# rcedgar/urmap

Measured on AMD Instinct MI355X. Metric: reads/s mapped, 150 bp SE vs hg38, at 1/2/4/8 MI355X; SAM bit-identical, higher is better.
Workload: dtype u8/u64 (fp32 DP cells as the reference)

## Files before the change

urmap_amd/csrc/kernels.h:

```cpp
#pragma once
#include <hip/hip_runtime.h>
#include <stdint.h>

#include "../../include/urmapx.h"

namespace urx {

struct DevIndex {
	const uint8_t *blob;
	const uint8_t *seq;
	const uint4 *seqp;
	uint64_t slotCount;
	uint64_t slotMagic;
	uint64_t shiftMask;
	uint32_t W;
	uint32_t maxIx;
	uint32_t seqDataSize;
	uint32_t seqCount;
	const uint32_t *seqLengths;
	const uint32_t *seqOffsets;
	const uint2 *rowinfo;
	const uint64_t *rowbase;
	const uint32_t *rows;
	const uint4 *slot16;
};

struct ProbeOut {
	uint64_t *slots;
	uint8_t *tallies;
	uint32_t *positions;
};

hipError_t launch_gather_bench(const DevIndex &X, uint32_t blocks, uint32_t iters, uint32_t *d_sink, hipStream_t s);

hipError_t launch_seed_probe(const DevIndex &X, const uint8_t *d_bases, const uint64_t *d_offs, uint32_t n,
                             uint32_t max_read_len, ProbeOut out, hipStream_t s);

struct DpJob {
	uint32_t read;
	uint32_t startdb, pk;
	int32_t maxpen;
	uint32_t combined_tlo;
	int16_t left_score, right_score;
	uint8_t nops;
	uint8_t flags;
	uint8_t vst_l, vst_r;
	uint16_t k;
	uint8_t pad[2];
};
static_assert(sizeof(DpJob) == 32, "DpJob layout");
static constexpr uint8_t DPJ_LEFT_FAIL = 1, DPJ_RIGHT_FAIL = 2, DPJ_RIGHT_SKIPPED = 4, DPJ_PATH_LONG = 8, DPJ_GATED = 16, DPJ_RIGHT_ABORTED = 32;
static constexpr int DP_ROUNDS = 4;
struct DpBounds {
	int rounds;
	uint32_t lo[DP_ROUNDS + 1];
};
inline DpBounds dp_bounds_default(bool long_reads) {
	DpBounds b;
	if (long_reads) { b.rounds = 4; b.lo[0] = 0; b.lo[1] = 2; b.lo[2] = 8; b.lo[3] = 32; b.lo[4] = 0xFFFFFFFFu; }
	else { b.rounds = 3; b.lo[0] = 0; b.lo[1] = 2; b.lo[2] = 16; b.lo[3] = 0xFFFFFFFFu; b.lo[4] = 0xFFFFFFFFu; }
	return b;
}
static constexpr int DP_TICKET_WORDS = 16;
static_assert(DP_ROUNDS <= 8, "DP_TICKET_WORDS");
static constexpr int DP_JOB_OPS = URMAPX_MAX_PATH_OPS;
static constexpr int STAGE_LAST = 3 + 4 * DP_ROUNDS;
static constexpr int STAGE_P3_MAIN = STAGE_LAST + 1, STAGE_P3_DP = STAGE_LAST + 2;
static constexpr int STAGE_EVENTS = STAGE_LAST + 3;

struct DpWork {
	DpJob *jobs = nullptr;
	uint16_t *ops = nullptr;
	uint16_t *kidx = nullptr;
	uint32_t jobs_cap = 0;
	uint32_t *tickets = nullptr;
	uint32_t *round_list = nullptr;
	uint32_t *counters = nullptr;
	uint32_t *fin_list = nullptr;
	uint32_t *state = nullptr;
	uint32_t fin_cap = 0;
};
size_t dp_state_words(bool ovf);
size_t p3_state_words(uint32_t max_read_len);

struct SearchWork {
	uint32_t *stats;
	uint8_t *scratch;
	size_t scratch_stride;
	int blocks;
	uint32_t *ticket;
	uint32_t *ticket3 = nullptr;
	int hsp_lds_cap = 0;
	uint32_t *ovf_list = nullptr;
	DpWork dp[2];
	DpWork dp3;
	uint8_t *dp_scratch = nullptr;
	size_t dp_scratch_stride = 0;
	int dp_blocks = 0;
	int fin_blocks = 0;
	DpBounds dp_bounds = dp_bounds_default(false);
	hipEvent_t *stage_events = nullptr;
};
size_t dp_scratch_stride(uint32_t max_read_len);
int dp_block_count(uint32_t max_read_len, int device);
int fin_block_count(uint32_t max_read_len, int device);
size_t search_scratch_stride(uint32_t max_read_len);
size_t search_scratch_tail(int blocks);
size_t search_pe_scratch_tail(int blocks);
int search_block_count(uint32_t max_read_len, int device);
size_t viterbi_batch_scratch_stride();

hipError_t launch_search_se(const DevIndex &X, const urmapx_params &P, const uint8_t *d_bases, const uint64_t *d_offs,
                            uint32_t n, uint32_t max_read_len, urmapx_result *d_results,
                            urmapx_path_op *d_path_ops, uint32_t *d_path_used, const SearchWork &wk, hipStream_t s);

size_t slow_scratch_stride(uint32_t qcap);
hipError_t launch_search_se_slow(const DevIndex &X, const urmapx_params &P, const uint8_t *d_bases, const uint64_t *d_offs, uint32_t n,
                                 uint32_t qcap, urmapx_result *d_results, urmapx_path_op *d_path_ops, uint32_t *d_path_used,
                                 uint32_t path_cap, uint8_t *scratch, int blocks, uint32_t *list, uint32_t *ticket, hipStream_t s);

size_t packed_seq_blocks(uint32_t seq_data_size);
hipError_t launch_pack_seq(const uint8_t *d_seq, uint32_t seq_data_size, uint4 *d_out, hipStream_t s);

size_t search_pe_scratch_stride(uint32_t max_read_len);
int search_pe_block_count(uint32_t max_read_len, int device);
hipError_t launch_search_pe(const DevIndex &X, const urmapx_params &P, const uint8_t *d_bases, const uint64_t *d_offs,
                            uint32_t npairs, uint32_t max_read_len, urmapx_result *d_results,
                            urmapx_path_op *d_path_ops, uint32_t *d_path_used, const SearchWork &wk, int veryfast,
                            urmapx_pair_info *pair_info, hipStream_t s);

size_t pe_slow_scratch_stride();
hipError_t launch_search_pe_slow(const DevIndex &X, const urmapx_params &P, const uint8_t *d_bases, const uint64_t *d_offs, uint32_t npairs,
                                 urmapx_result *d_results, urmapx_path_op *d_path_ops, uint32_t *d_path_used, uint32_t path_cap,
                                 uint8_t *scratch, int blocks, uint32_t *list, uint32_t *ticket, int veryfast, urmapx_pair_info *pair_info,
                                 int all_pairs, hipStream_t s);

hipError_t build_slot16_direct(const uint8_t *d_blob, uint64_t slot_count, uint32_t max_ix, uint4 **d_slot16, uint32_t **d_rows, uint64_t *total_rows);
hipError_t build_slot16(const uint8_t *d_blob, uint64_t slot_count, const uint2 *d_info, const uint64_t *d_base, const uint32_t *d_rows, uint4 **d_slot16);
hipError_t build_chain_rows(const uint8_t *d_blob, uint64_t slot_count, uint32_t max_ix, uint2 **d_info, uint64_t **d_base, uint32_t **d_rows,
                            uint64_t *total_rows);

hipError_t validate_index(const DevIndex &X, uint64_t out[9], float *ms);

static constexpr int UFI_STATS_COUNTERS = 17;
hipError_t ufi_stats_device(const DevIndex &X, uint64_t counters[UFI_STATS_COUNTERS], uint64_t hist[512], uint64_t *first_bad_slot, float ms[2]);
hipError_t ufi_slot_counts_device(const DevIndex &X, int minus, uint8_t *host_out);

hipError_t checksum_device(const void *d_ptr, uint64_t nbytes, uint64_t *out);

hipError_t launch_viterbi_batch(const urmapx_params &P, const uint8_t *d_a, const uint32_t *d_aoffs,
                                const uint8_t *d_b, const uint32_t *d_boffs, const uint8_t *d_flags, uint32_t n,
                                float *d_scores, uint8_t *d_status, urmapx_path_op *d_ops, uint16_t *d_nops,
                                uint8_t *d_scratch, hipStream_t s);

}
```

urmap_amd/csrc/kernels.hip:

```cpp
#include <algorithm>
#include <cstdlib>

#include "kernels.h"

#include "dev_common.h"
#include "probe_dev.h"
#include "viterbi_dev.h"

namespace urx {

template <int NCH>
__global__ __launch_bounds__(256) void seed_probe_kernel(DevIndex X, const uint8_t *__restrict__ bases,
                                                         const uint64_t *__restrict__ offs, uint32_t n, ProbeOut out) {
	const int lane = threadIdx.x & 63;
	const uint32_t r = blockIdx.x * (blockDim.x >> 6) + (threadIdx.x >> 6);
	if (r >= n) return;
	const uint64_t off = offs[r];
	const uint32_t QL = (uint32_t)(offs[r + 1] - off);
	const uint32_t W = X.W;
	if (QL < W || QL > 64u * NCH) return;
	const uint8_t *q = bases + off;
	probe_read<NCH>(X, q, QL, off, lane, out);
}


static constexpr int VB_MAXL = 448;
static constexpr int VB_WIDE_LA = 320, VB_WIDE_LB = 1800;

__global__ __launch_bounds__(64) void viterbi_batch_kernel(urmapx_params P, const uint8_t *__restrict__ a,
                                                           const uint32_t *__restrict__ aoffs,
                                                           const uint8_t *__restrict__ b,
                                                           const uint32_t *__restrict__ boffs,
                                                           const uint8_t *__restrict__ flags, uint32_t n,
                                                           float *scores, uint8_t *status_out, urmapx_path_op *ops_out,
                                                           uint16_t *nops_out, uint8_t *scratch, size_t scratch_stride) {
	__shared__ uint8_t sA[VB_MAXL];
	__shared__ uint32_t tb[(VB_MAXL / 8 + 2) * 64];
	__shared__ uint16_t rops[OPS_CAP];
	const int lane = threadIdx.x;
	const uint32_t k = blockIdx.x;
	if (k >= n) return;
	const int LA = (int)(aoffs[k + 1] - aoffs[k]), LB = (int)(boffs[k + 1] - boffs[k]);
	uint32_t status = 0;
	float score = 0.0f;
	RevOps R;
	R.ops = rops;
	R.begin();
	if (LA > VB_MAXL)
		status = URMAPX_ST_BAND_TOO_WIDE;
	else {
		for (int i = lane; i < LA; i += 64) sA[i] = a[aoffs[k] + i];
		URX_SYNC();
		WideScratch ws;
		ws.carve(scratch + (size_t)k * scratch_stride, VB_WIDE_LA, VB_WIDE_LB);
		score = viterbi_wave(VPar(P), sA, LA, b + boffs[k], LB, flags[k] & 1, (flags[k] >> 1) & 1, tb, VB_MAXL / 8 + 2, ws, R,
		                     status, lane);
	}
	int nout = R.n;
	if (nout > URMAPX_MAX_PATH_OPS) { status |= URMAPX_ST_PATH_OVERFLOW; nout = 0; }
	if (status) nout = 0;
	for (int t = lane; t < nout; t += 64) ops_out[(size_t)k * URMAPX_MAX_PATH_OPS + t] = rops[nout - 1 - t];
	if (lane == 0) { scores[k] = score; status_out[k] = (uint8_t)status; nops_out[k] = (uint16_t)nout; }
}

__global__ __launch_bounds__(64) void viterbi_batch_pair_kernel(urmapx_params P, const uint8_t *__restrict__ a,
                                                                const uint32_t *__restrict__ aoffs, const uint8_t *__restrict__ b,
                                                                const uint32_t *__restrict__ boffs, const uint8_t *__restrict__ flags,
                                                                uint32_t n, float *scores, uint8_t *status_out, urmapx_path_op *ops_out,
                                                                uint16_t *nops_out, uint8_t *scratch, size_t scratch_stride) {
	constexpr int TBR = VB_MAXL / 8 + 2;
	__shared__ uint8_t sA[2][VB_MAXL];
	__shared__ uint8_t sB[2][VB_MAXL + 96];
	__shared__ uint32_t tb[2][TBR * 64];
	__shared__ uint16_t rops[2][OPS_CAP];
	const int lane = threadIdx.x;
	const VPar VP(P);
	VFlank F[2];
	bool narrow[2] = {false, false};
	int LA[2] = {0, 0}, LB[2] = {0, 0};
	uint32_t kk[2];
	for (int h = 0; h < 2; ++h) {
		kk[h] = 2 * blockIdx.x + h;
		if (kk[h] >= n) continue;
		const uint32_t k = kk[h];
		LA[h] = (int)(aoffs[k + 1] - aoffs[k]); LB[h] = (int)(boffs[k + 1] - boffs[k]);
		if (LA[h] <= VB_MAXL)
			for (int i = lane; i < LA[h]; i += 64) sA[h][i] = a[aoffs[k] + i];
		if (LB[h] <= VB_MAXL + 64)
			for (int i = lane; i < LB[h]; i += 64) sB[h][16 + i] = b[boffs[k] + i];
	}
	URX_SYNC();
	for (int h = 0; h < 2; ++h)
		if (kk[h] < n && LA[h] <= VB_MAXL && LB[h] <= VB_MAXL + 64)
			narrow[h] = F[h].setup(VP, sA[h], LA[h], sB[h] + 16, LB[h], flags[kk[h]] & 1, (flags[kk[h]] >> 1) & 1, tb[h], TBR, -3.0e38f, false);
	if (!narrow[0]) F[0].active = false;
	if (!narrow[1]) F[1].active = false;
	viterbi_pair_rows(F[0], F[1]);
	for (int h = 0; h < 2; ++h) {
		if (kk[h] >= n) continue;
		const uint32_t k = kk[h];
		uint32_t status = 0;
		float score = 0.0f;
		RevOps R;
		R.ops = rops[h];
		R.begin();
		if (narrow[h]) score = F[h].finish(R, status);
		else if (LA[h] > VB_MAXL) status = URMAPX_ST_BAND_TOO_WIDE;
		else {
			WideScratch ws;
			ws.carve(scratch + (size_t)k * scratch_stride, VB_WIDE_LA, VB_WIDE_LB);
			score = viterbi_wave(VP, sA[h], LA[h], b + boffs[k], LB[h], flags[k] & 1, (flags[k] >> 1) & 1, tb[h], TBR, ws, R, status, lane);
		}
		int nout = R.n;
		if (nout > URMAPX_MAX_PATH_OPS) { status |= URMAPX_ST_PATH_OVERFLOW; nout = 0; }
		if (status) nout = 0;
		URX_SYNC();
		for (int t = lane; t < nout; t += 64) ops_out[(size_t)k * URMAPX_MAX_PATH_OPS + t] = rops[h][nout - 1 - t];
		if (lane == 0) { scores[k] = score; status_out[k] = (uint8_t)status; nops_out[k] = (uint16_t)nout; }
		URX_SYNC();
	}
}

static constexpr uint32_t PK_MASK = 1023u, PK_LEN_SH = 10, PK_SCORE_SH = 20, PK_ALIGNED = 1u << 30, PK_PLUS_SH = 31;
static constexpr int HSP_CAP = 256;
static constexpr int SEARCH_OVF_BLOCKS = 2048;
static constexpr int HSP_TOTAL_CAP = 8192;
static constexpr int TICKET_CHUNK = 4;
static constexpr int ROW_CAP = 32;

__host__ __device__ inline size_t search_tb_offset(int nch) {
	const int qmax = 64 * nch;
	size_t b = (size_t)2 * nch * ROW_CAP * 64 * 4 + WideScratch::bytes(qmax, qmax + 64);
	return (b + 255) & ~(size_t)255;
}
static constexpr int SE_HIT_TAIL = 64;
__host__ __device__ inline size_t search_tail_offset(int nch) {
	return (search_tb_offset(nch) + (size_t)((64 * nch - 24) / 8 + 2) * 64 * 4 + 255) & ~(size_t)255;
}
__host__ __device__ inline size_t search_scratch_bytes(int nch) { return search_tail_offset(nch) + (size_t)SE_HIT_TAIL * 4; }

__device__ __noinline__ int hsp_overflow_add(uint2 *ovf, int n, int cap, uint32_t diag, uint32_t startdb, uint32_t npk, int score) {
	const int lane = (int)__builtin_amdgcn_mbcnt_hi(~0u, __builtin_amdgcn_mbcnt_lo(~0u, 0u));
	for (int base = 0; base < n; base += 64) {
		const int i = base + lane;
		bool eq = false;
		uint2 e = make_uint2(0u, 0u);
		if (i < n) { e = ovf[i]; eq = (e.x - (e.y & PK_MASK)) == diag; }
		const uint64_t m = __ballot(eq);
		if (m) {
			const int l = __builtin_ctzll(m);
			const int old = (int)((rdlane(e.y, l) >> PK_SCORE_SH) & PK_MASK);
			if (score > old && lane == 0) ovf[base + l] = make_uint2(startdb, npk);
			URX_SYNC();
			return 0;
		}
	}
	if (n >= cap) return 2;
	if (lane == 0) ovf[n] = make_uint2(startdb, npk);
	return 1;
}

static constexpr int SE_HITW1 = 1;
template <int NCH, bool OVF, int LAYOUT = 0, int KCH = NCH>
struct SearchWave {
	static_assert(KCH >= 1 && KCH <= NCH, "k-mer chunks");
	static constexpr int QMAX = 64 * NCH;
	static constexpr int TB_ROWS8 = (QMAX - 24) / 8 + 2;
	static constexpr int WIDE_LB = QMAX + 64;
	static constexpr int NSEG = 2 * KCH;

	const DevIndex &X;
	const urmapx_params &P;
	int lane;
	const uint8_t *__restrict__ gseq;
	const uint8_t *__restrict__ gblob;
	int QL, W, nwords;
	uint8_t *sQ[2];
	uint8_t *sT;
	uint32_t *tb;
	uint16_t *ropsL, *ropsR, *cand, *top;
	uint16_t *pre;
	uint32_t *hsp_db;
	uint32_t *hsp_pk;
	uint2 *hsp_ovf;
	int hsp_lds;
	int hit_cap;
	uint32_t *rowstore;
	WideScratch ws;
	static constexpr int HITW = OVF ? 8 : SE_HITW1;
	uint32_t hit_db[HITW];
	static constexpr int TAIL = OVF ? 0 : SE_HIT_TAIL;
	uint32_t *hit_tail;
	__device__ __forceinline__ bool has_tail() const { return !OVF && hitCount > 64 * SE_HITW1; }
	int hit_wsh;
	__device__ __forceinline__ int wsh() const { return OVF ? hit_wsh : 6; }
	__device__ __forceinline__ int wl() const { return 1 << wsh(); }
	int hitCount, hspCount;
	int maxPen, best, second, bestHSP;
	bool haveTop; uint32_t top_db; bool top_plus; int top_nops;
	uint32_t status;

	__device__ SearchWave(const DevIndex &X_, const urmapx_params &P_, int lane_) : X(X_), P(P_), lane(lane_) {}

	__device__ __forceinline__ bool overlaps_hit(uint32_t db) const {
		bool eq = false;
#pragma unroll
		for (int w = 0; w < HITW; ++w) eq |= lane < wl() && (w << wsh()) + lane < hitCount && (hit_db[w] >> 6) == (db >> 6);
		if (has_tail()) eq |= lane < hitCount - 64 * SE_HITW1 && (hit_tail[lane] >> 6) == (db >> 6);
		return __ballot(eq) != 0;
	}

	__device__ __forceinline__ bool overlaps_any_hit(uint32_t db) const {
		bool ov = false;
#pragma unroll
		for (int w = 0; w < HITW; ++w)
			for (int k = 0; k < wl() && (w << wsh()) + k < hitCount; ++k) ov |= (rdlane(hit_db[w], k) >> 6) == (db >> 6);
		if (has_tail()) {
			const int nt = hitCount - 64 * SE_HITW1;
			const uint32_t t = lane < nt ? hit_tail[lane] : 0u;
			for (int k = 0; k < nt; ++k) ov |= (rdlane(t, k) >> 6) == (db >> 6);
		}
		return ov;
	}

	__device__ __forceinline__ void add_hit(uint32_t db, bool plus, int score, int cand_nops) {
		if (score < 10) return;
		const int lane = fresh_lane(this->lane);
		if (overlaps_hit(db)) return;
		int mp = (QL - score) - 2 * P.mismatch_score;
		if (mp < maxPen) maxPen = mp;
		bool newTop = false;
		if (score > best) { second = best; best = score; newTop = true; }
		else if (score == best) second = score;
		else {
			if (score < best - SECONDARY_HIT_MAX_DELTA) return;
			if (score > second) second = score;
		}
		if (hitCount >= (OVF ? HITW << wsh() : (hit_cap == 64 * SE_HITW1 ? hit_cap + TAIL : hit_cap))) { status |= URMAPX_ST_HIT_OVERFLOW; return; }
		if (!OVF && hitCount >= 64 * SE_HITW1) {
			if (lane == 0) hit_tail[hitCount - 64 * SE_HITW1] = db;
			URX_SYNC();
		} else {
#pragma unroll
			for (int w = 0; w < HITW; ++w)
				if (lane < wl() && (w << wsh()) + lane == hitCount) hit_db[w] = db;
		}
		++hitCount;
		if (newTop) {
			haveTop = true; top_db = db; top_plus = plus; top_nops = cand_nops;
			if (cand_nops) {
				for (int t = lane; t < cand_nops; t += 64) top[t] = cand[t];
				URX_SYNC();
			}
		}
	}

	__device__ __forceinline__ void add_hsp(uint32_t startq, uint32_t startdb, bool plus, uint32_t len, int score) {
		if (score < best - 4) return;
		const int lane = fresh_lane(this->lane);
		const uint32_t diag = startdb - startq;
		const uint32_t npk = startq | (len << PK_LEN_SH) | ((uint32_t)score << PK_SCORE_SH) | (plus ? 1u << PK_PLUS_SH : 0u);
		const int nlds = hspCount < hsp_lds ? hspCount : hsp_lds;
		for (int base = 0; base < nlds; base += 64) {
			const int i = base + lane;
			bool eq = false;
			if (i < nlds) eq = (hsp_db[i] - (hsp_pk[i] & PK_MASK)) == diag;
			uint64_t m = __ballot(eq);
			if (m) {
				const int k = base + __builtin_ctzll(m);
				const int old = (int)((hsp_pk[k] >> PK_SCORE_SH) & PK_MASK);
				if (score > old && lane == 0) { hsp_db[k] = startdb; hsp_pk[k] = npk; }
				URX_SYNC();
				return;
			}
		}
		if (hspCount >= hsp_lds) {
			const int rc = hsp_overflow_add(hsp_ovf, hspCount - hsp_lds, HSP_TOTAL_CAP - HSP_CAP, diag, startdb, npk, score);
			if (rc == 0) return;
			if (rc == 2) { status |= URMAPX_ST_HSP_OVERFLOW; return; }
		} else if (lane == 0) {
			hsp_db[hspCount] = startdb; hsp_pk[hspCount] = npk;
		}
		URX_SYNC();
		++hspCount;
		if (score > bestHSP) bestHSP = score;
	}

	__device__ __forceinline__ bool load_window(uint32_t tlo, int tl) {
		bool gap = false;
		for (int i = lane; i < tl; i += 64) {
			uint8_t c = gseq[tlo + i];
			sT[i] = c;
			gap |= (c == '-');
		}
		URX_SYNC();
		return __ballot(gap) != 0;
	}

	__device__ void align_hsp(int k) {
		uint32_t startdb, pk;
		if (k < hsp_lds) { startdb = hsp_db[k]; pk = hsp_pk[k]; }
		else { const uint2 e = hsp_ovf[k - hsp_lds]; startdb = e.x; pk = e.y; }
		if (pk & PK_ALIGNED) return;
		URX_SYNC();
		if (lane == 0) {
			if (k < hsp_lds) hsp_pk[k] = pk | PK_ALIGNED;
			else hsp_ovf[k - hsp_lds].y = pk | PK_ALIGNED;
		}
		const int startq = (int)(pk & PK_MASK), len = (int)((pk >> PK_LEN_SH) & PK_MASK);
		const int hscore = (int)((pk >> PK_SCORE_SH) & PK_MASK);
		const bool plus = (pk >> PK_PLUS_SH) & 1u;
		URX_SYNC();
		int totalPen = len - hscore;
		int totalScore = hscore;
		if (totalPen > maxPen) return;
		const int BR = 2 * (int)P.band_radius;
		const uint32_t TL = X.seqDataSize;
		uint32_t combinedTLo = startdb;
		const uint8_t *Q = plus ? sQ[0] : sQ[1];
		RevOps RL, RR;
		RL.ops = ropsL; RR.ops = ropsR;
		RL.begin(); RR.begin();
		int rtrim = 0;
		const VPar VP(P);
		const WideScratch wsv = ws;
		uint32_t vst = 0;

		const int rightQLo = startq + len;
#pragma unroll 1
		for (int side = 0; side < 2; ++side) {
			const bool left = side == 0;
			int fql;
			uint32_t tlo, tl;
			const uint8_t *fq;
			if (left) {
				if (startq <= 0) continue;
				if (startdb < (uint32_t)startq) return;
				fql = startq;
				const uint32_t leftTHi = startdb - 1;
				tl = (uint32_t)(fql + BR);
				if (tl >= leftTHi) return;
				tlo = leftTHi - tl + 1;
				fq = Q;
			} else {
				if (rightQLo >= QL) continue;
				fql = QL - rightQLo;
				tlo = startdb + (uint32_t)len;
				uint32_t thi = tlo + (uint32_t)fql + (uint32_t)BR;
				if (thi >= TL) thi = TL - 1;
				tl = thi - tlo + 1;
				fq = Q + rightQLo;
			}
			if (load_window(tlo, (int)tl)) return;
			const int allGap = P.gap_open_score + (fql - 1) * P.gap_ext_score;
			const int need = fql - (maxPen - totalPen);
			bool aborted = false;
			RevOps R;
			R.ops = left ? ropsL : ropsR;
			int score = (int)viterbi_wave<true>(VP, fq, fql, sT, (int)tl, left, !left, tb, TB_ROWS8, wsv, R, vst, lane, (float)need,
			                                    allGap < need ? &aborted : nullptr);
			if (aborted) return;
			status |= vst;
			if (left) {
				RL.n = R.n;
				int nTrimI = 0;
				if (RL.n > 0) {
					uint32_t lastop = ropsL[RL.n - 1];
					if ((lastop & 3u) == OP_I) { nTrimI = (int)(lastop >> 2); --RL.n; }
				}
				combinedTLo = tlo + (uint32_t)nTrimI;
			} else {
				RR.n = R.n;
				if (RR.n > 1 && (ropsR[0] & 3u) == OP_I) rtrim = 1;
			}
			if (allGap > score) score = allGap;
			totalScore += score;
			totalPen += fql - score;
			if (totalPen > maxPen) return;
		}
		if (vst & (URMAPX_ST_BAND_TOO_WIDE | URMAPX_ST_PATH_OVERFLOW)) return;
		int nc = 0, cop = -1, clen = 0;
		bool ovf = false;
		auto put = [&](int op, int l) {
			if (l <= 0) return;
			if (op == cop) { clen += l; return; }
			if (clen) { if (nc < URMAPX_MAX_PATH_OPS) { if (lane == 0) cand[nc] = (uint16_t)((clen << 2) | cop); ++nc; } else ovf = true; }
			cop = op; clen = l;
		};
		for (int t = RL.n - 1; t >= 0; --t) { uint32_t o = ropsL[t]; put((int)(o & 3u), (int)(o >> 2)); }
		put(OP_M, len);
		for (int t = RR.n - 1; t >= rtrim; --t) { uint32_t o = ropsR[t]; put((int)(o & 3u), (int)(o >> 2)); }
		put(-2, 1);
		if (ovf) { status |= URMAPX_ST_PATH_OVERFLOW; return; }
		URX_SYNC();
		add_hit(combinedTLo, plus, totalScore, nc);
	}

	static constexpr int STATE_WORDS = HITW * 64 + TAIL + 16 + URMAPX_MAX_PATH_OPS / 2;

	__device__ __forceinline__ bool hsp_get(int k, uint32_t &startdb, uint32_t &pk) const {
		startdb = 0; pk = 0;
		if (k >= hspCount) return false;
		if (k < hsp_lds) { startdb = hsp_db[k]; pk = hsp_pk[k]; }
		else { const uint2 e = hsp_ovf[k - hsp_lds]; startdb = e.x; pk = e.y; }
		return true;
	}
	__device__ __forceinline__ bool hsp_wants_dp(int k, uint32_t &startdb, uint32_t &pk) const {
		if (!hsp_get(k, startdb, pk)) return false;
		if (pk & PK_ALIGNED) return false;
		const int len = (int)((pk >> PK_LEN_SH) & PK_MASK), hscore = (int)((pk >> PK_SCORE_SH) & PK_MASK);
		return len - hscore <= maxPen;
	}

	static constexpr int P3_HSP = 128;
	static constexpr int P3_WORDS = STATE_WORDS + 2 * P3_HSP + 3 * NSEG * 64 + 2 * NSEG;

	template <bool P3 = false>
	__device__ int park_for_dp(const DpWork &dp, uint32_t r, int phase) {
		const int lane = fresh_lane(this->lane);
		int njobs = 0;
		bool clipped = false;
		for (int base = 0; base < hspCount; base += 64) {
			uint32_t sdb, pk;
			const bool want = hsp_wants_dp(base + lane, sdb, pk);
			njobs += __builtin_popcountll(__ballot(want));
			clipped |= want && (uint64_t)(sdb - (pk & PK_MASK)) + (uint64_t)QL + 2ull * P.band_radius >= (uint64_t)X.seqDataSize;
		}
		(void)clipped;
		if (njobs == 0) return 0;
		if (P3 && (hspCount > hsp_lds || hspCount > P3_HSP)) return -1;
		uint32_t jb = 0, slot = 0;
		if (lane == 0) jb = atomicAdd(dp.counters, (uint32_t)njobs);
		jb = uni(jb);
		bool room = jb < dp.jobs_cap && (uint32_t)njobs <= dp.jobs_cap - jb;
		if (room) {
			if (lane == 0) slot = atomicAdd(dp.counters + 1, 1u);
			slot = uni(slot);
			room = slot < dp.fin_cap;
		}
		if (!room) {
			for (uint32_t i = jb + lane; i < dp.jobs_cap && i - jb < (uint32_t)njobs; i += 64) { dp.jobs[i].read = 0xFFFFFFFFu; dp.kidx[i] = 0xFFFFu; }
			return -1;
		}
		int w = 0;
		for (int base = 0; base < hspCount; base += 64) {
			uint32_t sdb, pk;
			const bool ok = hsp_wants_dp(base + lane, sdb, pk);
			const uint64_t m = __ballot(ok);
			if (ok) {
				const uint32_t rank = __builtin_amdgcn_mbcnt_hi((uint32_t)(m >> 32), __builtin_amdgcn_mbcnt_lo((uint32_t)m, 0u));
				DpJob J;
				J.read = r; J.startdb = sdb; J.pk = pk; J.maxpen = maxPen;
				J.combined_tlo = 0; J.left_score = 0; J.right_score = 0; J.nops = 0; J.flags = 0; J.vst_l = 0; J.vst_r = 0;
				J.k = (uint16_t)((uint32_t)w + rank); J.pad[0] = J.pad[1] = 0;
				dp.jobs[jb + (uint32_t)w + rank] = J;
				dp.kidx[jb + (uint32_t)w + rank] = J.k;
			}
			w += __builtin_popcountll(m);
		}
		if (njobs > 0xFFFF) status |= URMAPX_ST_HSP_OVERFLOW;
		if (lane == 0) *reinterpret_cast<uint4 *>(dp.fin_list + 4 * (size_t)slot) = make_uint4(r, jb, (uint32_t)njobs, (uint32_t)QL);
		uint32_t *const st = dp.state + (size_t)slot * (P3 ? P3_WORDS : STATE_WORDS);
		park_state(st, phase);
		if constexpr (P3) {
			uint32_t *const hx = st + STATE_WORDS;
			for (int i = lane; i < hspCount; i += 64) { hx[i] = hsp_db[i]; hx[P3_HSP + i] = hsp_pk[i] | PK_ALIGNED; }
			uint32_t *const px = hx + 2 * P3_HSP;
#pragma unroll
			for (int g = 0; g < NSEG; ++g)
				if (64 * (g % KCH) < nwords) {
					px[g * 64 + lane] = pr_lo[g * 64 + lane];
					px[(NSEG + g) * 64 + lane] = pr_hi[g * 64 + lane];
					px[(2 * NSEG + g) * 64 + lane] = pr_sl[g * 64 + lane];
				}
			if (lane < NSEG) reinterpret_cast<uint64_t *>(px + 3 * NSEG * 64)[lane] = pr_hb[lane];
		}
		return 1;
	}

	__device__ __forceinline__ void mark_all_aligned() {
		const int nl = hspCount < hsp_lds ? hspCount : hsp_lds;
		for (int i = lane; i < nl; i += 64) hsp_pk[i] |= PK_ALIGNED;
		for (int i = hsp_lds + lane; i < hspCount; i += 64) hsp_ovf[i - hsp_lds].y |= PK_ALIGNED;
		URX_SYNC();
	}

	__device__ int resume3(uint32_t *st) {
		const int lane = fresh_lane(this->lane);
		const uint32_t *const hx = st + STATE_WORDS;
		const uint32_t *const px = hx + 2 * P3_HSP;
		wait_lgkm0();
#pragma unroll
		for (int g = 0; g < NSEG; ++g)
			if (64 * (g % KCH) < nwords) {
				glds_dword(px + g * 64 + lane, lds_addr(pr_lo + g * 64));
				glds_dword(px + (NSEG + g) * 64 + lane, lds_addr(pr_hi + g * 64));
				glds_dword(px + (2 * NSEG + g) * 64 + lane, lds_addr(pr_sl + g * 64));
			}
		uint64_t hb = 0;
		if (lane < NSEG) hb = reinterpret_cast<const uint64_t *>(px + 3 * NSEG * 64)[lane];
		const int phase = restore_state(st);
		for (int i = lane; i < hspCount; i += 64) { hsp_db[i] = hx[i]; hsp_pk[i] = hx[P3_HSP + i]; }
		if (lane < NSEG) pr_hb[lane] = hb;
		wait_vm0();
		URX_SYNC();
		return phase;
	}

	__device__ void park_state(uint32_t *st, int phase) {
#pragma unroll
		for (int wd = 0; wd < HITW; ++wd) st[wd * 64 + lane] = hit_db[wd];
		if (has_tail() && hit_tail != st + HITW * 64 && lane < hitCount - 64 * SE_HITW1) st[HITW * 64 + lane] = hit_tail[lane];
		uint32_t *sc = st + HITW * 64 + TAIL;
		if (lane == 0) {
			sc[0] = (uint32_t)hitCount; sc[1] = (uint32_t)maxPen; sc[2] = (uint32_t)best; sc[3] = (uint32_t)second;
			sc[4] = top_db; sc[5] = (haveTop ? 1u : 0u) | (top_plus ? 2u : 0u) | ((uint32_t)phase << 8);
			sc[6] = (uint32_t)top_nops; sc[7] = status; sc[8] = (uint32_t)hspCount;
		}
		uint16_t *tops = reinterpret_cast<uint16_t *>(sc + 16);
		for (int t = lane; t < top_nops; t += 64) tops[t] = top[t];
	}

	__device__ int restore_state(uint32_t *st) {
#pragma unroll
		for (int wd = 0; wd < HITW; ++wd) hit_db[wd] = st[wd * 64 + lane];
		hit_tail = st + HITW * 64;
		const uint32_t *sc = st + HITW * 64 + TAIL;
		static_assert(URMAPX_MAX_PATH_OPS <= 128, "two path ops per lane");
		const uint16_t *tops = reinterpret_cast<const uint16_t *>(sc + 16);
		const uint16_t t0 = tops[lane];
		const uint16_t t1 = lane + 64 < URMAPX_MAX_PATH_OPS ? tops[lane + 64] : (uint16_t)0;
		hitCount = (int)uni(sc[0]); maxPen = (int)uni(sc[1]); best = (int)uni(sc[2]); second = (int)uni(sc[3]);
		top_db = uni(sc[4]);
		const uint32_t f = uni(sc[5]);
		haveTop = (f & 1u) != 0; top_plus = (f & 2u) != 0;
		top_nops = (int)uni(sc[6]); status = uni(sc[7]); hspCount = (int)uni(sc[8]); bestHSP = 0;
		top[lane] = t0;
		if (lane + 64 < URMAPX_MAX_PATH_OPS) top[lane + 64] = t1;
		URX_SYNC();
		return (int)(f >> 8);
	}

	__device__ bool consume_job(const DpJob &J, const uint16_t *jops) {
		const uint32_t pk = J.pk;
		const int startq = (int)(pk & PK_MASK), len = (int)((pk >> PK_LEN_SH) & PK_MASK);
		const int hscore = (int)((pk >> PK_SCORE_SH) & PK_MASK);
		const bool plus = (pk >> PK_PLUS_SH) & 1u;
		int totalPen = len - hscore;
		int totalScore = hscore;
		if (totalPen > maxPen) return false;
		if (J.flags & DPJ_GATED) { status |= URMAPX_ST_BAND_TOO_WIDE; return false; }
		uint32_t vst = 0;
		if (startq > 0) {
			if (J.flags & DPJ_LEFT_FAIL) return true;
			vst |= J.vst_l;
			status |= J.vst_l;
			totalScore += J.left_score;
			totalPen += startq - J.left_score;
			if (totalPen > maxPen) return true;
		}
		const int rightQLo = startq + len;
		if (rightQLo < QL) {
			if (J.flags & (DPJ_RIGHT_FAIL | DPJ_RIGHT_SKIPPED)) return true;
			vst |= J.vst_r;
			status |= J.vst_r;
			totalScore += J.right_score;
			totalPen += (QL - rightQLo) - J.right_score;
			if (totalPen > maxPen) return true;
		}
		if (vst & (URMAPX_ST_BAND_TOO_WIDE | URMAPX_ST_PATH_OVERFLOW)) return true;
		if (J.flags & DPJ_PATH_LONG) { status |= URMAPX_ST_PATH_OVERFLOW; return true; }
		const int nc = (int)J.nops;
		URX_SYNC();
		for (int t = lane; t < nc; t += 64) cand[t] = jops[t];
		URX_SYNC();
		add_hit(J.combined_tlo, plus, totalScore, nc);
		return true;
	}

	__device__ void fill_result(urmapx_result &res, int phase, urmapx_path_op *__restrict__ path_ops, uint32_t *path_used) {
		const int lane = fresh_lane(this->lane);
		if (fill_result_core(res, phase)) {
			uint32_t po = 0;
			if (lane == 0) po = atomicAdd(path_used, (uint32_t)top_nops);
			po = uni(po);
			for (int t = lane; t < top_nops; t += 64) path_ops[po + t] = top[t];
			res.path_off = po; res.path_nops = (uint16_t)top_nops;
		}
	}
	__device__ bool fill_result_core(urmapx_result &res, int phase) {
		res.mapq = (uint8_t)calc_mapq();
		res.score = (int16_t)best; res.second = (int16_t)second;
		res.hit_count = (uint16_t)hitCount; res.exit_phase = (uint8_t)phase; res.status = (uint8_t)status;
		if (haveTop) {
			uint32_t lo = 0, hi = X.seqCount - 1;
			uint32_t found = 0xFFFFFFFFu, coord = 0xFFFFFFFFu, tl = 0;
			if (X.seqCount <= 64u) {
				const int lane = fresh_lane(this->lane);
				const bool mine = (uint32_t)lane < X.seqCount;
				const uint32_t o = mine ? X.seqOffsets[lane] : 0u, sl = mine ? X.seqLengths[lane] : 0u;
				const uint64_t m = __ballot(mine && top_db >= o && top_db < o + sl);
				if (m) {
					const int k = __builtin_ctzll(m);
					found = (uint32_t)k; coord = top_db - rdlane(o, k); tl = rdlane(sl, k);
				}
				hi = 0xFFFFFFFFu;
			}
			while (lo <= hi && hi != 0xFFFFFFFFu) {
				uint32_t k = (lo + hi) / 2;
				uint32_t o = X.seqOffsets[k], sl = X.seqLengths[k];
				if (top_db >= o && top_db < o + sl) { found = k; coord = top_db - o; tl = sl; break; }
				if (top_db > o) lo = k + 1;
				else hi = k - 1;
			}
			if (found != 0xFFFFFFFFu && coord + (uint32_t)QL <= tl) {
				res.dbpos = top_db; res.seq_index = found; res.coord = coord; res.plus = top_plus ? 1 : 0;
				return top_nops > 0;
			}
		}
		return false;
	}

	__device__ __forceinline__ uint32_t calc_mapq() const {
		if (hitCount == 0) return 0;
		if (best <= 0) return 0;
		double bp = (double)QL;
		double sec = (double)second;
		if (sec < bp / 2.0) {
			sec = bp / 2.0;
			if ((double)best <= sec) return 0;
		}
		double fract = (double)best / bp;
		double drop = (double)best - sec;
		if (drop > 40) drop = 40;
		double x = drop * fract;
		x = x * fract;
		uint32_t mapq = (uint32_t)x;
		if (mapq > 40) mapq = 40;
		return mapq;
	}

	uint32_t *pr_lo, *pr_hi, *pr_sl;
	uint64_t *pr_hb;
	uint32_t reserved = 0;
	__device__ __forceinline__ void probe_get(int s, int q, uint32_t &tally, uint32_t &pos) const {
		const int e = s * KCH * 64 + (s ? nwords - 1 - q : q);
		if constexpr (LAYOUT == 1) {
			pos = pr_lo[e];
			tally = pr_hi[e] & 0xFFu;
			return;
		}
		const uint32_t lo = pr_lo[e], hi = pr_hi[e], sl = pr_sl[e];
		const uint64_t v = (((uint64_t)hi << 32) | lo) >> (8u * (sl & 3u));
		tally = (uint32_t)(v & 0xFFu);
		pos = (uint32_t)(v >> 8);
	}

	__device__ __forceinline__ void probe_hash(const uint8_t *nq, int QLn, uint32_t *stage_sl, uint64_t *stage_b) {
		const int lane = fresh_lane(this->lane);
		QLn = fresh_uniform(QLn);
		const uint32_t nwn = (uint32_t)(QLn - (W - 1));
		auto planes = [&](int c, uint64_t &lo, uint64_t &hi, uint64_t &inv, uint64_t &invm) {
			const int p = 64 * c + lane;
			const uint32_t ch = p < QLn ? nq[p] : 0u;
			const uint32_t L = p < QLn ? letter_of(ch) : 4u;
			lo = __ballot(L & 1u);
			hi = __ballot((L >> 1) & 1u);
			inv = __ballot(L > 3u);
			invm = __ballot(L > 3u || ch == 'u');
		};
		uint64_t lo0, hi0, inv0, invm0;
		planes(0, lo0, hi0, inv0, invm0);
#pragma unroll
		for (int c = 0; c < KCH; ++c) {
			if (64u * c < nwn) {
				uint64_t lo1 = 0, hi1 = 0, inv1 = ~0ull, invm1 = ~0ull;
				if (c + 1 < NCH && 64 * (c + 1) < QLn) planes(c + 1, lo1, hi1, inv1, invm1);
				uint64_t sp, sm;
				bool vp, vm;
				kmer_slots(X, lo0, hi0, inv0, invm0, lo1, hi1, inv1, invm1, lane, 64u * c + lane, nwn, sp, sm, vp, vm);
				stage_sl[c * 64 + lane] = (uint32_t)sp;
				stage_sl[(KCH + c) * 64 + lane] = (uint32_t)sm;
				const uint64_t hbp = __ballot(vp && ((sp >> 32) & 1ull)), hbm = __ballot(vm && ((sm >> 32) & 1ull));
				const uint64_t okp = __ballot(vp), okm = __ballot(vm);
				if (lane == 0) {
					stage_b[2 * c] = hbp; stage_b[2 * c + 1] = okp;
					stage_b[2 * (KCH + c)] = hbm; stage_b[2 * (KCH + c) + 1] = okm;
				}
				lo0 = lo1; hi0 = hi1; inv0 = inv1; invm0 = invm1;
			}
		}
	}
	__device__ __forceinline__ void probe_gather(int QLn, const uint32_t *stage_sl, const uint64_t *stage_b) {
		const int lane = fresh_lane(this->lane);
		QLn = fresh_uniform(QLn);
		const uint32_t nwn = (uint32_t)(QLn - (W - 1));
		wait_lgkm0();
#pragma unroll
		for (int g = 0; g < NSEG; ++g) {
			if (64u * (g % KCH) < nwn) {
				const uint64_t hb = stage_b[2 * g], ok = stage_b[2 * g + 1];
				const bool v = (ok >> lane) & 1ull;
				const uint32_t sl = stage_sl[g * 64 + lane];
				if constexpr (LAYOUT == 1) {
					const uint64_t slot16 = (uint64_t)sl | (((hb >> lane) & 1ull) << 32);
					const uint8_t *ap = v ? reinterpret_cast<const uint8_t *>(X.slot16) + 16ull * slot16 : reinterpret_cast<const uint8_t *>(g_zero16);
					glds_dword(ap, lds_addr(pr_lo + g * 64));
					glds_dword(ap + 4, lds_addr(pr_hi + g * 64));
					glds_dword(ap + 8, lds_addr(pr_sl + g * 64));
					continue;
				}
#ifdef URX_FAULT_SLOT32
				const uint64_t slot = (uint64_t)sl; (void)hb;
#else
				const uint64_t slot = (uint64_t)sl | (((hb >> lane) & 1ull) << 32);
#endif
				pr_sl[g * 64 + lane] = v ? sl : 0u;
				if (lane == 0) pr_hb[g] = hb;
				const uint8_t *ap = v ? gblob + ((5ull * slot) & ~3ull) : reinterpret_cast<const uint8_t *>(g_zero16);
				glds_dword(ap, lds_addr(pr_lo + g * 64));
				glds_dword(ap + 4, lds_addr(pr_hi + g * 64));
			}
		}
	}

	__device__ __forceinline__ void walk_heads(uint64_t (&sl)[NSEG], uint32_t (&T)[NSEG], uint32_t (&ps)[NSEG], bool (&act)[NSEG]) const {
		const int lane = fresh_lane(this->lane);
#pragma unroll
		for (int g = 0; g < NSEG; ++g) {
			const int s2 = g / KCH, c = g % KCH;
			const int p = 64 * c + lane;
			T[g] = 0; ps[g] = 0; sl[g] = 0;
			if constexpr (LAYOUT == 1) {
				if (p < nwords) {
					const int e = s2 * KCH * 64 + (s2 ? nwords - 1 - p : p);
					const uint32_t hi = pr_hi[e];
					ps[g] = pr_lo[e];
					T[g] = hi & 0xFFu;
					sl[g] = (uint64_t)((hi >> 8) & 0xFFu) | ((uint64_t)pr_sl[e] << 32);
				}
				act[g] = (T[g] & TALLY_MY_BIT) != 0 && T[g] != TALLY_BOTH1;
				continue;
			}
			if (p < nwords) probe_get(s2, p, T[g], ps[g]);
			act[g] = (T[g] & TALLY_MY_BIT) != 0 && T[g] != TALLY_BOTH1;
			if (act[g]) {
				const int i = s2 ? nwords - 1 - p : p;
				sl[g] = (uint64_t)pr_sl[s2 * KCH * 64 + i] | (((pr_hb[s2 * KCH + (i >> 6)] >> (i & 63)) & 1ull) << 32);
			}
		}
	}
	__device__ __forceinline__ void walk_run(uint64_t (&sl)[NSEG], uint32_t (&T)[NSEG], uint32_t (&ps)[NSEG], bool (&act)[NSEG], int (&rl)[NSEG]) {
		const uint64_t N = X.slotCount;
		const int maxIx = (int)X.maxIx;
		bool any = false;
#pragma unroll
		for (int g = 0; g < NSEG; ++g) { rl[g] = 0; any |= act[g]; }
		while (any) {
			const int lane = fresh_lane(this->lane);
#pragma unroll
			for (int g = 0; g < NSEG; ++g) {
				if (!act[g]) continue;
				uint32_t *rs = rowstore + (size_t)g * ROW_CAP * 64 + lane;
				rs[rl[g] * 64] = ps[g];
				++rl[g];
				const uint32_t t = T[g];
				if (rl[g] == maxIx || rl[g] >= ROW_CAP) act[g] = false;
				else if (t == TALLY_PLUS1 || t == TALLY_BOTH1) { rl[g] = 1; act[g] = false; }
				else if (t == TALLY_END) act[g] = false;
				else if (t == TALLY_LONG_MINE || t == TALLY_LONG_OTHER) {
					const uint64_t slotA = addmod(sl[g], ps[g] & 0xFFFFu, N);
					sl[g] = addmod(slotA, ps[g] >> 16, N);
					uint32_t tA, pA;
					load_slot(gblob, slotA, tA, pA);
					rs[(rl[g] - 1) * 64] = pA;
				} else
					sl[g] = addmod(sl[g], t & TALLY_NEXT_MASK, N);
			}
			any = false;
#pragma unroll
			for (int g = 0; g < NSEG; ++g) {
				if (act[g]) load_slot(gblob, sl[g], T[g], ps[g]);
				any |= act[g];
			}
		}
	}

	__device__ __forceinline__ void rows_fetch(uint64_t (&sl)[NSEG], uint32_t (&T)[NSEG], uint32_t (&ps)[NSEG], bool (&act)[NSEG], int (&rl)[NSEG]) {
		const int lane = fresh_lane(this->lane);
		if constexpr (LAYOUT == 1) {
#pragma unroll
			for (int g = 0; g < NSEG; ++g) {
				rl[g] = act[g] ? (int)(sl[g] & 0xFFu) : 0;
				if (act[g]) {
					rowstore[(size_t)g * 64 + lane] = (uint32_t)(sl[g] >> 32);
					rowstore[(size_t)(NSEG + g) * 64 + lane] = ps[g];
				}
			}
			return;
		}
		uint2 info[NSEG];
		bool longhead = false;
#pragma unroll
		for (int g = 0; g < NSEG; ++g) {
			info[g] = make_uint2(0u, 0u);
			if (act[g] && T[g] != TALLY_PLUS1) info[g] = X.rowinfo[sl[g]];
			longhead |= act[g] && T[g] == TALLY_LONG_MINE;
		}
		const bool any_long = __ballot(longhead) != 0;
#pragma unroll
		for (int g = 0; g < NSEG; ++g) {
			rl[g] = 0;
			if (act[g]) {
				uint32_t p0 = ps[g];
				if (T[g] == TALLY_PLUS1) rl[g] = 1;
				else {
					rl[g] = (int)(info[g].x & 0xFFu);
					uint32_t at = 0;
					if (rl[g] > 2 || (any_long && T[g] == TALLY_LONG_MINE)) at = (uint32_t)(X.rowbase[sl[g] >> 10] + (info[g].x >> 8));
					if (any_long && T[g] == TALLY_LONG_MINE) p0 = X.rows[at];
					rowstore[(size_t)g * 64 + lane] = at;
					rowstore[(size_t)(2 * NSEG + g) * 64 + lane] = info[g].y;
				}
				rowstore[(size_t)(NSEG + g) * 64 + lane] = p0;
			}
		}
	}
	__device__ __forceinline__ uint32_t row_entry(int seg, int k, int l, bool short_row) const {
		if constexpr (LAYOUT == 1) {
			if (k == 0) return rowstore[(size_t)(NSEG + seg) * 64 + l];
			const uint32_t x = rowstore[(size_t)seg * 64 + l];
			return short_row ? x : X.rows[(size_t)x + (uint32_t)k];
		}
		if (k < 2) return rowstore[(size_t)((k + 1) * NSEG + seg) * 64 + l];
		return X.rows[(size_t)rowstore[(size_t)seg * 64 + l] + (uint32_t)k];
	}

	template <int NS>
	__device__ __forceinline__ int scan_counts(const int (&cnt)[NS]) {
		int carry = 0;
#pragma unroll
		for (int sgm = 0; sgm < NS; ++sgm) {
			int inc = wave_prefix_sum(cnt[sgm]);
			pre[sgm * 64 + lane] = (uint16_t)(carry + inc - cnt[sgm]);
			carry += rdlane(inc, 63);
		}
		if (lane == 0) pre[NS * 64] = (uint16_t)carry;
		if (carry > 0xFFFF) status |= URMAPX_ST_HSP_OVERFLOW;
		URX_SYNC();
		return carry;
	}

	__device__ __forceinline__ void locate(int g, int nrows, int &r, int &k) const {
		int lo = 0, hi = nrows;
		while (lo < hi) {
			int mid = (lo + hi + 1) >> 1;
			if ((int)pre[mid] <= g) lo = mid;
			else hi = mid - 1;
		}
		r = lo;
		k = g - (int)pre[lo];
	}
};

#define SEARCH_WAVES_PER_EU(NCH) ((NCH) <= 3 ? 4 : (NCH) == 4 ? 3 : (NCH) == 5 ? 2 : 1)
template <int NCH, bool OVF, bool DBG, int ROWS = 0, int PART = 0, int KCH = NCH>
__global__ __launch_bounds__(64, SEARCH_WAVES_PER_EU(NCH)) void search_se_kernel(DevIndex X, urmapx_params P, const uint8_t *__restrict__ bases,
                                                       const uint64_t *__restrict__ offs, uint32_t n,
                                                       urmapx_result *__restrict__ results,
                                                       urmapx_path_op *__restrict__ path_ops, uint32_t *path_used,
                                                       uint32_t *stats, uint8_t *scratch, size_t scratch_stride,
                                                       const uint8_t *__restrict__ g_seq, const uint8_t *__restrict__ g_blob,
                                                       const uint4 *__restrict__ g_seqp,
                                                       uint32_t *ticket, int hsp_lds_cap, uint32_t *ovf_list, uint2 *hsp_ovf_base,
                                                       DpWork dp, DpWork dp3) {
	static_assert(PART == 0 || (!OVF && !DBG && ROWS == 1), "phase 3 is parked by the production first pass only");
	static_assert(KCH == NCH || (ROWS == 2 && PART == 0 && !OVF && !DBG), "fewer k-mer chunks: the production first pass on the slot16 layout");
// ... 157 lines not shown
					if (64 * c < QL) {
						const int p = 64 * c + lane;
						uint64_t b0, b1, b2 = 0, b3 = 0;
						if (acgt) {
							const uint32_t code = p < QL ? seq_code_acgt(sQ2[s * SW::QMAX + p]) : 0u;
							b0 = __ballot(code & 1u); b1 = __ballot(code & 2u);
						} else {
							const uint32_t code = p < QL ? seq_code(sQ2[s * SW::QMAX + p], SEQ_CODE_QOTHER) : 0u;
							b0 = __ballot(code & 1u); b1 = __ballot(code & 2u); b2 = __ballot(code & 4u); b3 = __ballot(code & 8u);
							oth |= __ballot(code == SEQ_CODE_QOTHER);
						}
						if (lane < 2) {
							const int shh = 32 * lane;
							qpl[s * 2 * NCH + 2 * c + lane] = make_uint4((uint32_t)(b0 >> shh), (uint32_t)(b1 >> shh), (uint32_t)(b2 >> shh), (uint32_t)(b3 >> shh));
						}
					}
				}
			}
			q_other = oth != 0;
			URX_SYNC();
			if (next_ok) { wait_lgkm0(); fetch_bytes(noff, nQL); fetched = true; }
			lapc(0);
		}
		int nwords = QL - (W - 1);
		if constexpr (PART == 2) {
			if (cur_ok) {
				phase = S.resume3(dp3.state + (size_t)p3_e * SW::P3_WORDS);
				for (uint32_t k0 = 0; k0 < p3_nj; k0 += 64) {
					const uint32_t k = k0 + (uint32_t)lane;
					uint32_t jpk = 0;
					uint4 jw = make_uint4(0u, 0u, 0u, 0u);
					if (k < p3_nj) {
						const uint32_t *jp = reinterpret_cast<const uint32_t *>(dp3.jobs + p3_jb + k);
						jpk = jp[2];
						jw = *reinterpret_cast<const uint4 *>(jp + 4);
					}
					const int nt = (int)(p3_nj - k0 < 64u ? p3_nj - k0 : 64u);
					for (int t = 0; t < nt; ++t) {
						DpJob J;
						J.read = r; J.startdb = 0; J.maxpen = 0; J.k = 0; J.pad[0] = J.pad[1] = 0;
						J.pk = rdlane(jpk, t);
						J.combined_tlo = rdlane(jw.x, t);
						const uint32_t sc = rdlane(jw.y, t), fl = rdlane(jw.z, t);
						J.left_score = (int16_t)(sc & 0xFFFFu); J.right_score = (int16_t)(sc >> 16);
						J.nops = (uint8_t)(fl & 0xFFu); J.flags = (uint8_t)((fl >> 8) & 0xFFu); J.vst_l = (uint8_t)((fl >> 16) & 0xFFu); J.vst_r = (uint8_t)(fl >> 24);
						S.consume_job(J, dp3.ops + (size_t)(p3_jb + k0 + (uint32_t)t) * DP_JOB_OPS);
					}
				}
				if (S.best >= QL + P.xphase1 * P.mismatch_score) done = true;
			}
		}
		const int minScore1 = QL + P.xphase1 * P.mismatch_score;
		const int minScore3 = QL + P.xphase3 * P.mismatch_score;
		const int minScore4 = QL + P.xphase4 * P.mismatch_score;
		const int termHSP3 = (QL * P.term_hsp_score_pct_phase3) / 100;
		const int minhsp = (int)((uint32_t)P.min_hsp_score_pct * (uint32_t)(QL > 0 ? QL : 0) / 100.0);

		int rl[SW::NSEG];
#pragma unroll
		for (int g = 0; g < SW::NSEG; ++g) rl[g] = 0;
		for (int step = (cur_ok && PART != 2) ? 1 : 5;;) {
			QL = fresh_uniform(QL);
			S.QL = QL; nwords = QL - (W - 1); S.nwords = nwords;
			lane = fresh_lane(lane); S.lane = lane;
			if (DBG && dbg_stop && step != 5 && (dbg_stop == 100 || (dbg_stop < 100 && step > dbg_stop))) {
				done = true;
				if (step == 4 || step == 6) break;
				step = 5;
			}
			if (step == 5) {
				const bool go = !done;
				uint64_t wsl[SW::NSEG];
				uint32_t wT[SW::NSEG], wps[SW::NSEG];
				bool wact[SW::NSEG];
				if (PART != 2 && next_ok) {
					if (!fetched) fetch_bytes(noff, nQL);
					wait_vm0();
					URX_SYNC();
					S.probe_hash(nextQ + nmis, nQL, stage_sl, stage_b);
					URX_SYNC();
				}
				if (go) S.walk_heads(wsl, wT, wps, wact);
				if (PART != 2 && next_ok) S.probe_gather(nQL, stage_sl, stage_b);
				if (PART == 2 && next_ok && !fetched) { fetch_bytes(noff, nQL); fetched = true; }
				if (!go) break;
				if constexpr (ROWS != 0) S.rows_fetch(wsl, wT, wps, wact, rl);
				else S.walk_run(wsl, wT, wps, wact, rl);
				URX_SYNC();
				lapc(3);
				if (DBG && dbg_stop == 104) { done = true; break; }
				step = 4;
				continue;
			}
			phase = step;
			if (step == 3 || step == 6) {
				if constexpr (PART != 0) {
					if (S.status & (URMAPX_ST_HSP_OVERFLOW | URMAPX_ST_HIT_OVERFLOW)) {
						if (step == 6) break;
						done = true;
					} else if (step == 6) {
						const int rc = S.template park_for_dp<false>(dp, r, 6);
						if (rc > 0) parked = true;
						else if (rc < 0) S.status |= URMAPX_ST_HSP_OVERFLOW;
						break;
					} else if (S.bestHSP > termHSP3) {
						const int rc = S.template park_for_dp<true>(dp3, r, 3);
						if (rc > 0) { parked = true; done = true; }
						else if (rc < 0) { S.status |= URMAPX_ST_HSP_OVERFLOW; done = true; }
						else S.mark_all_aligned();
					}
					step = 5;
					continue;
				} else {
				if (step == 6 && !OVF && (S.status & (URMAPX_ST_HSP_OVERFLOW | URMAPX_ST_HIT_OVERFLOW))) break;
				if (step == 6 && dp.jobs != nullptr && S.park_for_dp(dp, r, 6) > 0) { parked = true; break; }
				if (step == 6 || S.bestHSP > termHSP3) {
					for (int k = 0; k < S.hspCount; ++k) S.align_hsp(k);
					if (step == 3 && S.best >= minScore1) done = true;
				}
				lapc(step == 3 ? 2 : 6);
				if (step == 6) break;
				step = 5;
				continue;
				}
			}
			int cnt[2 * SW::NSEG];
#pragma unroll
			for (int g = 0; g < 2 * SW::NSEG; ++g) cnt[g] = 0;
			if (step == 1) {
#pragma unroll
				for (int c = 0; c < KCH; ++c) {
					const int p = 64 * c + lane;
					int nb1 = 0;
					if (p < nwords) {
						uint32_t t0, p0, t1, p1;
						S.probe_get(0, p, t0, p0);
						S.probe_get(1, p, t1, p1);
						nb1 = (t0 == TALLY_BOTH1 ? 1 : 0) + (t1 == TALLY_BOTH1 ? 1 : 0);
					}
					const bool onStride = (p % W) == 0;
					cnt[c] = onStride ? nb1 : 0;
					cnt[KCH + c] = onStride ? 0 : nb1;
				}
			} else {
#pragma unroll
				for (int g = 0; g < SW::NSEG; ++g) {
					cnt[g] = rl[g] <= 2 ? rl[g] : 0;
					cnt[SW::NSEG + g] = rl[g] > 2 ? rl[g] : 0;
				}
			}
			const int used = 2 * SW::NSEG;
			const int total = S.template scan_counts<2 * SW::NSEG>(cnt);
			const int totalFirst = (int)S.pre[(step == 1 ? KCH : SW::NSEG) * 64];
			bool crossed = false;
			int scanned = 0, qhead = 0, qcount = 0;
			while (!done && (scanned < total || qcount > 0)) {
				QL = fresh_uniform(QL);
				S.QL = QL; nwords = QL - (W - 1); S.nwords = nwords;
				lane = fresh_lane(lane); S.lane = lane;
				uint64_t tsub = timing ? __builtin_amdgcn_s_memtime() : 0;
				auto laps = [&](int slot) {
					if (!timing) return;
					uint64_t now = __builtin_amdgcn_s_memtime();
					if (lane == 0) atomicAdd(reinterpret_cast<unsigned long long *>(stats) + 1 + slot, (unsigned long long)(now - tsub));
					tsub = now;
				};
				while (qcount < 64 && scanned < total) {
					const int g = scanned + lane;
					uint32_t s_qpos = 0, s_db = 0;
					bool s_plus = true, ok = false;
					if (g < total) {
						int row, k;
						S.locate(g, used * 64, row, k);
						if (step == 1) {
							if (row >= KCH * 64) row -= KCH * 64;
							s_qpos = (uint32_t)row;
							uint32_t tp, pp, tm, pm;
							S.probe_get(0, row, tp, pp);
							S.probe_get(1, row, tm, pm);
							if (k == 0 && tp == TALLY_BOTH1) { s_plus = true; s_db = pp; }
							else { s_plus = false; s_db = pm; }
						} else {
							int seg = row >> 6;
							const int l = row & 63;
							const bool short_row = seg < SW::NSEG;
							if (seg >= SW::NSEG) seg -= SW::NSEG;
							s_plus = seg < KCH;
							s_qpos = (uint32_t)((seg - (s_plus ? 0 : KCH)) * 64 + l);
							if constexpr (ROWS != 0) s_db = S.row_entry(seg, k, l, short_row);
							else s_db = S.rowstore[((size_t)seg * ROW_CAP + k) * 64 + l];
						}
						ok = s_db >= s_qpos;
					}
					ok = ok && !S.overlaps_any_hit(s_db - s_qpos);
					const uint64_t m = __ballot(ok);
					if (ok) {
						const int pos = (qhead + qcount + (int)__builtin_amdgcn_mbcnt_hi((uint32_t)(m >> 32), __builtin_amdgcn_mbcnt_lo((uint32_t)m, 0u))) & 127;
						cq_db[pos] = s_db;
						cq_qp[pos] = (uint16_t)(s_qpos | (s_plus ? 0x4000u : 0u) | (g >= totalFirst ? 0x8000u : 0u));
					}
					qcount += __builtin_popcountll(m);
					scanned += 64;
				}
				URX_SYNC();
				const int nb = qcount < 64 ? qcount : 64;
				if (nb == 0) break;
				uint32_t c_qpos = 0, c_db = 0;
				bool c_plus = true, c_second = false;
				const bool c_ok = lane < nb;
				if (c_ok) {
					const int pos = (qhead + lane) & 127;
					c_db = cq_db[pos];
					const uint32_t qp = cq_qp[pos];
					c_qpos = qp & 0x3FFFu; c_plus = (qp & 0x4000u) != 0; c_second = (qp & 0x8000u) != 0;
				}
				qhead = (qhead + nb) & 127; qcount -= nb;
				URX_SYNC();
				bool c_live = c_ok;
				laps(8);
				uint64_t mm[NCH];
#pragma unroll
				for (int c = 0; c < NCH; ++c) mm[c] = 0;
				if (q_other) {
					if (c_live) lane_mismatch_mask<NCH>(g_seq, c_db - c_qpos, sQ2 + (c_plus ? 0 : SW::QMAX), QL, mm);
				} else {
					if (c_live) lane_mismatch_planes<NCH>(g_seqp, c_db - c_qpos, qpl + (c_plus ? 0 : 2 * NCH), QL, mm);
				}
				laps(9);
				int e_kind = 0, e_bst = 0, e_start = 0, e_end = 0, e_pen = 0;
				bool worth = false;
				if (c_live) {
					const int nmis = mismatches_outside_seed<NCH>(mm, (int)c_qpos, W);
					const int floor2 = minhsp > S.best - 4 ? minhsp : S.best - 4;
					worth = -P.mismatch_score * nmis <= S.maxPen || QL - nmis >= floor2;
				}
				if (worth) {
					xdrop_walk_lane<NCH>(mm, (int)c_qpos, W, QL, P.mismatch_score, P.xdrop, S.maxPen, e_bst, e_start, e_end, e_pen);
					if (e_start == 0 && e_end == QL - 1) e_kind = 1;
					else if (e_bst >= minhsp) e_kind = 2;
				}
				laps(10);
				const uint32_t my_dblo = c_db - c_qpos;
				uint64_t todo = __ballot(e_kind != 0 && e_pen <= S.maxPen && !(e_kind == 2 && e_bst < S.best - 4) &&
				                         !S.overlaps_any_hit(my_dblo));
				while (todo) {
					lane = fresh_lane(lane); S.lane = lane;
					const int t = __builtin_ctzll(todo);
					todo &= todo - 1;
					if (rdlane((uint32_t)c_second, t) != 0 && !crossed) {
						crossed = true;
						if (step == 4 && S.best >= minScore3) { done = true; break; }
					}
					const uint32_t dblo = rdlane(my_dblo, t);
					if (S.overlaps_hit(dblo)) continue;
					if (rdlane(e_pen, t) > S.maxPen) continue;
					const bool pl = rdlane((uint32_t)c_plus, t) != 0;
					const int bst = rdlane(e_bst, t);
					const int hc0 = S.hitCount, mp0 = S.maxPen, b0 = S.best;
					if (rdlane(e_kind, t) == 1) {
						S.add_hit(dblo, pl, bst, 0);
						if (step == 1 && bst >= minScore1) { done = true; phase = crossed ? 2 : 1; break; }
					} else {
						const int sp = rdlane(e_start, t), ep = rdlane(e_end, t);
						S.add_hsp((uint32_t)sp, dblo + (uint32_t)sp, pl, (uint32_t)(ep - sp + 1), bst);
						todo &= ~__ballot(e_kind == 2 && my_dblo == dblo && e_bst <= bst);
					}
					if (S.hitCount != hc0 || S.maxPen != mp0 || S.best != b0)
						todo &= __ballot(e_pen <= S.maxPen && !(e_kind == 2 && e_bst < S.best - 4) &&
						                 !(S.hitCount != hc0 && (my_dblo >> 6) == (dblo >> 6)));
				}
				laps(11);
			}

			if (step == 1) {
				lapc(1);
				if (!done) phase = 2;
				step = done ? 5 : 3;
				continue;
			}
			lapc(4);
			if (!done && !crossed && S.best >= minScore3) done = true;
			if (!done) { phase = 5; if (S.best >= minScore4) done = true; }
			if (done) break;
			step = 6;
		}
		lapc(6);
		if (cur_ok && !parked) S.fill_result(res, phase, path_ops, path_used);
		lapc(7);
		if (have_cur && !parked) {
			if constexpr (!OVF) {
				if (res.status & (URMAPX_ST_HSP_OVERFLOW | URMAPX_ST_HIT_OVERFLOW)) {
					if (lane == 0) ovf_list[1 + atomicAdd(ovf_list, 1u)] = r;
				}
			}
			if (lane == 0) results[r] = res;
			if (timing && lane == 0) stats[64 + r] = (uint32_t)((__builtin_amdgcn_s_memtime() - t_read0) >> 4);
		}
		if (!have_next) break;
		have_cur = true; r = rn; off = noff; QL = nQL;
		p3_e = n_e; p3_jb = n_jb; p3_nj = n_nj;
	}
}

__global__ __launch_bounds__(256) void dp_round_lists_kernel(DpWork dp, DpBounds bounds) {
	const uint32_t *const DP_ROUND_LO = bounds.lo;
	constexpr int PER = 16;
	__shared__ uint32_t cnt[DP_ROUNDS], base[DP_ROUNDS];
	const uint32_t made = dp.counters[0];
	const uint32_t njobs = made < dp.jobs_cap ? made : dp.jobs_cap;
	for (uint32_t c0 = blockIdx.x * 256u * PER; c0 < njobs; c0 += gridDim.x * 256u * PER) {
		if (threadIdx.x < DP_ROUNDS) cnt[threadIdx.x] = 0;
		__syncthreads();
		const uint32_t j0 = c0 + threadIdx.x * PER;
		uint16_t kk[PER];
		if (j0 + PER <= njobs) {
			const uint4 a = *reinterpret_cast<const uint4 *>(dp.kidx + j0), b = *reinterpret_cast<const uint4 *>(dp.kidx + j0 + 8);
			const uint32_t w[8] = {a.x, a.y, a.z, a.w, b.x, b.y, b.z, b.w};
#pragma unroll
			for (int i = 0; i < PER; ++i) kk[i] = (uint16_t)(w[i >> 1] >> (16 * (i & 1)));
		} else {
#pragma unroll
			for (int i = 0; i < PER; ++i) kk[i] = j0 + i < njobs ? dp.kidx[j0 + i] : (uint16_t)0xFFFFu;
		}
		uint32_t my[DP_ROUNDS], pos[DP_ROUNDS];
#pragma unroll
		for (int rd = 0; rd < DP_ROUNDS; ++rd) {
			my[rd] = 0;
#pragma unroll
			for (int i = 0; i < PER; ++i) my[rd] += (kk[i] != 0xFFFFu && kk[i] >= DP_ROUND_LO[rd] && kk[i] < DP_ROUND_LO[rd + 1]) ? 1u : 0u;
			pos[rd] = my[rd] ? atomicAdd(&cnt[rd], my[rd]) : 0u;
		}
		__syncthreads();
		if (threadIdx.x < DP_ROUNDS) base[threadIdx.x] = cnt[threadIdx.x] ? atomicAdd(dp.tickets + 8 + threadIdx.x, cnt[threadIdx.x]) : 0u;
		__syncthreads();
#pragma unroll
		for (int rd = 0; rd < DP_ROUNDS; ++rd) {
			uint32_t *out = dp.round_list + (size_t)rd * dp.jobs_cap + base[rd] + pos[rd];
#pragma unroll
			for (int i = 0; i < PER; ++i)
				if (kk[i] != 0xFFFFu && kk[i] >= DP_ROUND_LO[rd] && kk[i] < DP_ROUND_LO[rd + 1]) *out++ = j0 + (uint32_t)i;
		}
		__syncthreads();
	}
}

template <int NCH>
__global__ __launch_bounds__(64) void dp_kernel(DevIndex X, urmapx_params P, const uint8_t *__restrict__ bases,
                                                const uint64_t *__restrict__ offs, DpWork dp, uint8_t *scratch,
                                                size_t scratch_stride, const uint8_t *__restrict__ g_seq, uint32_t klo, uint32_t khi,
                                                uint32_t *ticket, const uint32_t *__restrict__ list, const uint32_t *list_count) {
	constexpr int QMAX = 64 * NCH;
	constexpr int TB_ROWS8 = (QMAX - 24) / 8 + 2;
	__shared__ __attribute__((aligned(16))) uint8_t sQT[QMAX + QMAX + 64];
	uint8_t *const sQ = sQT, *const sT = sQT + QMAX;
	static_assert(QMAX >= 64, "the window lies band_radius + 1 bytes or more inside sQT (viterbi_dev.h: B_LDS)");
	uint32_t *const tb = reinterpret_cast<uint32_t *>(scratch + (size_t)blockIdx.x * scratch_stride +
	                                                  ((WideScratch::bytes(QMAX, QMAX + 64) + 255) & ~(size_t)255));
	__shared__ uint32_t wlds[3 * QMAX];
	__shared__ uint16_t ropsL[OPS_CAP], ropsR[OPS_CAP], cand[URMAPX_MAX_PATH_OPS];
	const int lane = threadIdx.x;
	WideScratch ws;
	ws.carve(scratch + (size_t)blockIdx.x * scratch_stride, QMAX, QMAX + 64);
	const VPar VP(P);
	const int BR = 2 * (int)P.band_radius;
	const uint32_t made = dp.counters[0];
	const uint32_t njobs = made < dp.jobs_cap ? made : dp.jobs_cap;
	auto load_window = [&](uint32_t tlo, int tl) {
		bool gap = false;
		for (int i = lane; i < tl; i += 64) {
			const uint8_t c = g_seq[tlo + i];
			sT[i] = c;
			gap |= (c == '-');
		}
		URX_SYNC();
		return __ballot(gap) != 0;
	};
	uint32_t n_gated = 0;
	uint32_t q_read = 0xFFFFFFFFu;
	bool q_plus = false;
	uint64_t q_off = 0;
	int q_len = 0;
	constexpr uint32_t DP_TILE = 16;
	(void)klo; (void)khi; (void)njobs;
	const uint32_t nlist = *list_count < dp.jobs_cap ? *list_count : dp.jobs_cap;
	uint32_t tile = blockIdx.x * DP_TILE;
	for (bool first = true;; first = false) {
	if (!first) {
		if (tile + DP_TILE >= nlist && tile >= gridDim.x * DP_TILE) break;
		uint32_t t0 = 0;
		if (lane == 0) t0 = atomicAdd(ticket, DP_TILE);
		tile = gridDim.x * DP_TILE + (uint32_t)__builtin_amdgcn_readfirstlane((int)t0);
	}
	if (tile >= nlist) break;
	uint32_t jl = 0xFFFFFFFFu;
	if (lane < (int)DP_TILE && tile + lane < nlist) jl = list ? list[tile + lane] : tile + (uint32_t)lane;
	uint64_t todo = __ballot(jl != 0xFFFFFFFFu);
	while (todo) {
		const uint32_t j = rdlane(jl, __builtin_ctzll(todo));
		todo &= todo - 1;
		const DpJob J = dp.jobs[j];
		if (J.read == 0xFFFFFFFFu) continue;
		{
			const int glen = (int)((J.pk >> PK_LEN_SH) & PK_MASK), gscore = (int)((J.pk >> PK_SCORE_SH) & PK_MASK);
			if (glen - gscore > J.maxpen) {
				if (lane == 0) dp.jobs[j].flags = DPJ_GATED;
				++n_gated;
				continue;
			}
		}
		const uint32_t pk = J.pk, startdb = J.startdb;
		const int startq = (int)(pk & PK_MASK), len = (int)((pk >> PK_LEN_SH) & PK_MASK), hscore = (int)((pk >> PK_SCORE_SH) & PK_MASK);
		const bool plus = (pk >> PK_PLUS_SH) & 1u;
		URX_SYNC();
		if (J.read != q_read || plus != q_plus) {
			if (J.read != q_read) {
				q_off = offs[J.read];
				q_len = (int)(offs[J.read + 1] - q_off);
			}
			const uint8_t *q = bases + q_off;
#pragma unroll
			for (int c = 0; c < NCH; ++c) {
				const int p = 64 * c + lane;
				if (p < q_len) sQ[p] = plus ? q[p] : (uint8_t)comp_char(q[q_len - 1 - p]);
			}
			q_read = J.read; q_plus = plus;
			URX_SYNC();
		}
		const int QL = q_len;
		uint32_t flags = 0, vst_l = 0, vst_r = 0, combinedTLo = startdb;
		int leftScore = 0, rightScore = 0, rtrim = 0;
		int totalPen = len - hscore;
		RevOps RL, RR;
		RL.ops = ropsL; RR.ops = ropsR;
		RL.begin(); RR.begin();
		if (startq > 0) {
			const int leftQL = startq;
			const uint32_t leftTHi = startdb - 1;
			const uint32_t leftTL = (uint32_t)(leftQL + BR);
			if (startdb < (uint32_t)startq || leftTL >= leftTHi) flags |= DPJ_LEFT_FAIL;
			else {
				const uint32_t leftTLo = leftTHi - leftTL + 1;
				if (load_window(leftTLo, (int)leftTL)) flags |= DPJ_LEFT_FAIL;
				else {
					const int allGap = P.gap_open_score + (leftQL - 1) * P.gap_ext_score;
					const int need = leftQL - (J.maxpen - totalPen);
					bool aborted = false;
					leftScore = (int)viterbi_wave<true>(VP, sQ, leftQL, sT, (int)leftTL, true, false, tb, TB_ROWS8, ws, RL, vst_l, lane,
					                                    (float)need, allGap < need ? &aborted : nullptr, wlds, 3 * QMAX);
					if (aborted) { leftScore = need - 1; RL.begin(); vst_l = 0; }
					int nTrimI = 0;
					if (RL.n > 0) {
						const uint32_t lastop = ropsL[RL.n - 1];
						if ((lastop & 3u) == OP_I) { nTrimI = (int)(lastop >> 2); --RL.n; }
					}
					combinedTLo = leftTLo + (uint32_t)nTrimI;
					if (allGap > leftScore) leftScore = allGap;
					totalPen += leftQL - leftScore;
				}
			}
		}
		const int rightQLo = startq + len;
		if (!(flags & DPJ_LEFT_FAIL) && rightQLo < QL) {
			if (totalPen > J.maxpen) flags |= DPJ_RIGHT_SKIPPED;
			else {
				const int rightQL = QL - rightQLo;
				const uint32_t rightTLo = startdb + (uint32_t)len;
				uint32_t rightTHi = rightTLo + (uint32_t)rightQL + (uint32_t)BR;
				if (rightTHi >= X.seqDataSize) rightTHi = X.seqDataSize - 1;
				const uint32_t rightTL = rightTHi - rightTLo + 1;
				if (load_window(rightTLo, (int)rightTL)) flags |= DPJ_RIGHT_FAIL;
				else {
					const int allGap = P.gap_open_score + (rightQL - 1) * P.gap_ext_score;
					const int need = rightQL - (J.maxpen - totalPen);
					bool aborted = false;
					rightScore = (int)viterbi_wave<true>(VP, sQ + rightQLo, rightQL, sT, (int)rightTL, false, true, tb, TB_ROWS8, ws, RR, vst_r, lane,
					                                     (float)need, allGap < need ? &aborted : nullptr, wlds, 3 * QMAX);
					if (aborted) { rightScore = need - 1; RR.begin(); vst_r = 0; flags |= DPJ_RIGHT_ABORTED; }
					if (RR.n > 1 && (ropsR[0] & 3u) == OP_I) rtrim = 1;
					if (allGap > rightScore) rightScore = allGap;
				}
			}
		}
		int nc = 0;
		if (!(flags & (DPJ_LEFT_FAIL | DPJ_RIGHT_FAIL | DPJ_RIGHT_SKIPPED | DPJ_RIGHT_ABORTED))) {
			int cop = -1, clen = 0;
			bool ovf = false;
			auto put = [&](int op, int l) {
				if (l <= 0) return;
				if (op == cop) { clen += l; return; }
				if (clen) { if (nc < URMAPX_MAX_PATH_OPS) { if (lane == 0) cand[nc] = (uint16_t)((clen << 2) | cop); ++nc; } else ovf = true; }
				cop = op; clen = l;
			};
			for (int t = RL.n - 1; t >= 0; --t) { const uint32_t o = ropsL[t]; put((int)(o & 3u), (int)(o >> 2)); }
			put(OP_M, len);
			for (int t = RR.n - 1; t >= rtrim; --t) { const uint32_t o = ropsR[t]; put((int)(o & 3u), (int)(o >> 2)); }
			put(-2, 1);
			if (ovf) { flags |= DPJ_PATH_LONG; nc = 0; }
			URX_SYNC();
			uint16_t *out = dp.ops + (size_t)j * DP_JOB_OPS;
			for (int t = lane; t < nc; t += 64) out[t] = cand[t];
		}
		if (lane == 0) {
			DpJob *o = dp.jobs + j;
			o->combined_tlo = combinedTLo;
			o->left_score = (int16_t)leftScore; o->right_score = (int16_t)rightScore;
			o->nops = (uint8_t)nc; o->flags = (uint8_t)flags; o->vst_l = (uint8_t)vst_l; o->vst_r = (uint8_t)vst_r;
		}
	}
	}
	if (lane == 0 && n_gated) atomicAdd(dp.counters + 3, n_gated);
}

template <int NCH, bool OVF>
__global__ __launch_bounds__(64) __attribute__((amdgpu_waves_per_eu(8, 8))) void finalize_se_kernel(DevIndex X, urmapx_params P, const uint64_t *__restrict__ offs, DpWork dp,
                                                         urmapx_result *__restrict__ results, urmapx_path_op *__restrict__ path_ops,
                                                         uint32_t *path_used, int hsp_lds_cap, uint32_t *ovf_list, uint32_t klo,
                                                         uint32_t khi) {
	using SW = SearchWave<NCH, OVF>;
	__shared__ uint16_t top[URMAPX_MAX_PATH_OPS], cand[URMAPX_MAX_PATH_OPS];
	constexpr int PBUF_OPS = 1024, PEND = 64;
	__shared__ uint16_t pbuf[PBUF_OPS];
	__shared__ uint32_t pend_r[PEND];
	__shared__ urmapx_result pend_res[PEND];
	int pb_used = 0, pb_n = 0;
	const int lane = threadIdx.x;
	auto flush_paths = [&]() {
		if (pb_n == 0) return;
		URX_SYNC();
		uint32_t po = 0;
		if (lane == 0) po = atomicAdd(path_used, (uint32_t)pb_used);
		po = uni(po);
		for (int t = lane; t < pb_used; t += 64) path_ops[po + t] = pbuf[t];
		if (lane < pb_n) {
			urmapx_result rr = pend_res[lane];
			rr.path_off += po;
			results[pend_r[lane]] = rr;
		}
		URX_SYNC();
		pb_used = 0; pb_n = 0;
	};
	SW S(X, P, lane);
	S.W = (int)X.W;
	S.top = top; S.cand = cand;
	S.hsp_lds = (hsp_lds_cap >= 64 && hsp_lds_cap <= HSP_CAP) ? (hsp_lds_cap & ~63) : HSP_CAP;
	S.hit_cap = (hsp_lds_cap >= 64 && hsp_lds_cap <= HSP_CAP) ? S.hsp_lds / 4 : 64 * SE_HITW1;
	S.hit_wsh = (hsp_lds_cap >= 64 && hsp_lds_cap <= HSP_CAP) ? 4 : 6;
	const uint32_t parked = dp.counters[1] < dp.fin_cap ? dp.counters[1] : dp.fin_cap;
	const uint4 *const fin = reinterpret_cast<const uint4 *>(dp.fin_list);
	uint32_t used_block = 0;
	uint4 ent = make_uint4(0u, 0u, 0u, 0u);
	if (blockIdx.x < parked) ent = fin[blockIdx.x];
	for (uint32_t e = blockIdx.x; e < parked; e += gridDim.x) {
		const uint32_t r = uni(ent.x), jb = uni(ent.y), nj = uni(ent.z);
		S.QL = (int)uni(ent.w);
		if (e + gridDim.x < parked) ent = fin[e + gridDim.x];
		if (nj <= klo) continue;
		S.nwords = S.QL - (S.W - 1);
		const uint32_t kend = nj < khi ? nj : khi;
		uint32_t jpk0 = 0;
		uint4 jw0 = make_uint4(0u, 0u, 0u, 0u);
		if (klo + (uint32_t)lane < kend) {
			const uint32_t *jp = reinterpret_cast<const uint32_t *>(dp.jobs + jb + klo + (uint32_t)lane);
			jpk0 = jp[2];
			jw0 = *reinterpret_cast<const uint4 *>(jp + 4);
		}
		URX_SYNC();
		uint32_t *const st = dp.state + (size_t)e * SW::STATE_WORDS;
		const int phase = S.restore_state(st);
		uint32_t used = 0;
		for (uint32_t k0 = klo; k0 < kend; k0 += 64) {
			const uint32_t k = k0 + (uint32_t)lane;
			const uint32_t jpk = jpk0;
			const uint4 jw = jw0;
			jpk0 = 0; jw0 = make_uint4(0u, 0u, 0u, 0u);
			if (k + 64u < kend) {
				const uint32_t *jp = reinterpret_cast<const uint32_t *>(dp.jobs + jb + k + 64u);
				jpk0 = jp[2];
				jw0 = *reinterpret_cast<const uint4 *>(jp + 4);
			}
			const int jstartq = (int)(jpk & PK_MASK), jlen = (int)((jpk >> PK_LEN_SH) & PK_MASK), jhs = (int)((jpk >> PK_SCORE_SH) & PK_MASK);
			const int jpen = jlen - jhs;
			const int jls = (int)(int16_t)(jw.y & 0xFFFFu), jrs = (int)(int16_t)(jw.y >> 16);
			const uint32_t jfl = (jw.z >> 8) & 0xFFu;
			const bool has_l = jstartq > 0, has_r = jstartq + jlen < S.QL;
			const bool raises = (jw.z >> 16) != 0u || (jfl & (DPJ_GATED | DPJ_PATH_LONG)) != 0u;
			const bool dead = (has_l && (jfl & DPJ_LEFT_FAIL)) || (has_r && (jfl & (DPJ_RIGHT_FAIL | DPJ_RIGHT_SKIPPED)));
			const int pen1 = jpen + (has_l ? jstartq - jls : 0);
			const int pen2 = pen1 + (has_r ? (S.QL - (jstartq + jlen)) - jrs : 0);
			const int jscore = jhs + (has_l ? jls : 0) + (has_r ? jrs : 0);
			auto viable = [&]() {
				return k < kend && jpen <= S.maxPen && (raises || (!dead && pen1 <= S.maxPen && pen2 <= S.maxPen && jscore >= S.best - SECONDARY_HIT_MAX_DELTA && jscore >= 10));
			};
			used += (uint32_t)__builtin_popcountll(__ballot(k < kend && jpen <= S.maxPen));
			uint64_t todo = __ballot(viable());
			while (todo) {
				const int t = __builtin_ctzll(todo);
				todo &= todo - 1;
				DpJob J;
				J.read = r; J.startdb = 0; J.maxpen = 0; J.k = 0; J.pad[0] = J.pad[1] = 0;
				J.pk = rdlane(jpk, t);
				J.combined_tlo = rdlane(jw.x, t);
				const uint32_t sc = rdlane(jw.y, t), fl = rdlane(jw.z, t);
				J.left_score = (int16_t)(sc & 0xFFFFu); J.right_score = (int16_t)(sc >> 16);
				J.nops = (uint8_t)(fl & 0xFFu); J.flags = (uint8_t)((fl >> 8) & 0xFFu); J.vst_l = (uint8_t)((fl >> 16) & 0xFFu); J.vst_r = (uint8_t)(fl >> 24);
				const int mp0 = S.maxPen, b0 = S.best;
				S.consume_job(J, dp.ops + (size_t)(jb + k0 + (uint32_t)t) * DP_JOB_OPS);
				if (S.maxPen != mp0 || S.best != b0) todo &= __ballot(viable());
			}
		}
		used_block += used;
		if (nj > khi) {
			URX_SYNC();
			S.park_state(st, phase);
			for (uint32_t k = khi + lane; k < nj; k += 64) dp.jobs[jb + k].maxpen = S.maxPen;
			continue;
		}
		urmapx_result res;
		res.dbpos = 0xFFFFFFFFu; res.seq_index = 0xFFFFFFFFu; res.coord = 0xFFFFFFFFu;
		res.score = 0; res.second = 0; res.mapq = 0; res.plus = 0; res.exit_phase = 0; res.status = 0;
		res.hit_count = 0; res.path_nops = 0; res.path_off = 0;
		if (S.fill_result_core(res, phase)) {
			if (pb_used + S.top_nops > PBUF_OPS || pb_n == PEND) flush_paths();
			URX_SYNC();
			for (int t = lane; t < S.top_nops; t += 64) pbuf[pb_used + t] = top[t];
			res.path_nops = (uint16_t)S.top_nops;
			res.path_off = (uint32_t)pb_used;
			if (lane == 0) { pend_r[pb_n] = r; pend_res[pb_n] = res; }
			pb_used += S.top_nops; ++pb_n;
		} else if (lane == 0) results[r] = res;
		if constexpr (!OVF) {
			if (res.status & (URMAPX_ST_HSP_OVERFLOW | URMAPX_ST_HIT_OVERFLOW)) {
				if (lane == 0) ovf_list[1 + atomicAdd(ovf_list, 1u)] = r;
			}
		}
	}
	flush_paths();
	if (lane == 0 && used_block) atomicAdd(dp.counters + 2, used_block);
}

size_t dp_state_words(bool ovf) { return ovf ? (size_t)SearchWave<3, true>::STATE_WORDS : (size_t)SearchWave<3, false>::STATE_WORDS; }
size_t p3_state_words(uint32_t max_read_len) {
	return max_read_len <= 128 ? (size_t)SearchWave<2, false>::P3_WORDS : max_read_len <= 192 ? (size_t)SearchWave<3, false>::P3_WORDS :
	       max_read_len <= 256 ? (size_t)SearchWave<4, false>::P3_WORDS : max_read_len <= 320 ? (size_t)SearchWave<5, false>::P3_WORDS : 0;
}
size_t dp_scratch_stride(uint32_t max_read_len) {
	const int qmax = 64 * (max_read_len <= 128 ? 2 : max_read_len <= 192 ? 3 : max_read_len <= 256 ? 4 : max_read_len <= 320 ? 5 : max_read_len <= 512 ? 8 : 16);
	return ((WideScratch::bytes(qmax, qmax + 64) + 255) & ~(size_t)255) + (size_t)((qmax - 24) / 8 + 2) * 256;
}

static int nch_for(uint32_t max_read_len) {
	if (max_read_len <= 128) return 2;
	if (max_read_len <= 192) return 3;
	if (max_read_len <= 256) return 4;
	if (max_read_len <= 320) return 5;
	if (max_read_len <= 512) return 8;
	if (max_read_len <= 1024) return 16;
	return 0;
}

size_t search_scratch_stride(uint32_t max_read_len) {
	const int nch = nch_for(max_read_len);
	return (search_scratch_bytes(nch) + 255) & ~(size_t)255;
}
size_t search_scratch_tail(int blocks) {
	return (size_t)(blocks > SEARCH_OVF_BLOCKS ? blocks : SEARCH_OVF_BLOCKS) * (HSP_TOTAL_CAP - HSP_CAP) * sizeof(uint2);
}

int search_block_count(uint32_t max_read_len, int device) {
	hipDeviceProp_t prop;
	if (hipGetDeviceProperties(&prop, device) != hipSuccess) return 0;
	int per_cu = 0;
	const int nchq = nch_for(max_read_len);
	hipError_t e = nchq == 2   ? hipOccupancyMaxActiveBlocksPerMultiprocessor(&per_cu, search_se_kernel<2, false, false, true>, 64, 0)
	               : nchq == 3 ? hipOccupancyMaxActiveBlocksPerMultiprocessor(&per_cu, search_se_kernel<3, false, false, true>, 64, 0)
	               : nchq == 4 ? hipOccupancyMaxActiveBlocksPerMultiprocessor(&per_cu, search_se_kernel<4, false, false, true>, 64, 0)
	               : nchq == 5 ? hipOccupancyMaxActiveBlocksPerMultiprocessor(&per_cu, search_se_kernel<5, false, false, true>, 64, 0)
	               : nchq == 8 ? hipOccupancyMaxActiveBlocksPerMultiprocessor(&per_cu, search_se_kernel<8, false, false>, 64, 0)
	                           : hipOccupancyMaxActiveBlocksPerMultiprocessor(&per_cu, search_se_kernel<16, false, false>, 64, 0);
	if (e != hipSuccess || per_cu < 1) per_cu = 8;
	if (const char *t = getenv("URMAPX_TEST_BLOCKS_PER_CU")) { const int v = atoi(t); if (v >= 1 && v < per_cu) per_cu = v; }
	if (const char *t = getenv("URMAPX_BLOCKS_PER_CU")) { const int v = atoi(t); if (v >= 1 && v < per_cu) per_cu = v; }
	return per_cu * prop.multiProcessorCount;
}

__global__ __launch_bounds__(256) void pack_seq_kernel(const uint8_t *__restrict__ seq, uint64_t nbytes, uint4 *__restrict__ out,
                                                       uint64_t nblocks) {
	const int lane = threadIdx.x & 63;
	const uint64_t wave = (uint64_t)blockIdx.x * (blockDim.x >> 6) + (threadIdx.x >> 6);
	const uint64_t nwaves = (uint64_t)gridDim.x * (blockDim.x >> 6);
	uint32_t *o32 = reinterpret_cast<uint32_t *>(out);
	for (uint64_t w = wave; 2 * w < nblocks; w += nwaves) {
		const uint64_t i = 64 * w + lane;
		const uint32_t code = i < nbytes ? seq_code(seq[i], SEQ_CODE_TOTHER) : SEQ_CODE_TOTHER;
		const uint64_t b0 = __ballot(code & 1u), b1 = __ballot(code & 2u), b2 = __ballot(code & 4u), b3 = __ballot(code & 8u);
		if (lane < 8 && 2 * w + (lane >> 2) < nblocks) {
			const int k = lane & 3;
			const uint64_t b = k == 0 ? b0 : k == 1 ? b1 : k == 2 ? b2 : b3;
			o32[8 * w + lane] = (uint32_t)(b >> (32 * (lane >> 2)));
		}
	}
}

size_t packed_seq_blocks(uint32_t seq_data_size) { return ((size_t)seq_data_size + 4096 + 31) / 32 + 40; }

hipError_t launch_pack_seq(const uint8_t *d_seq, uint32_t seq_data_size, uint4 *d_out, hipStream_t s) {
	const uint64_t nblocks = packed_seq_blocks(seq_data_size);
	hipLaunchKernelGGL(pack_seq_kernel, dim3(8192), dim3(256), 0, s, d_seq, (uint64_t)seq_data_size, d_out, nblocks);
	return hipGetLastError();
}

template <int MODE>
__global__ __launch_bounds__(256) void gather_bench_kernel(const uint8_t *__restrict__ blob, uint64_t slot_count,
                                                           uint64_t magic, uint32_t iters, uint32_t *sink) {
	__shared__ uint32_t dst[MODE == 2 ? 4 * 8 * 2 * 64 : (MODE == 3 ? 4 * 8 * 3 * 64 : 1)];
	uint64_t x = murmur64(((uint64_t)blockIdx.x << 20) + threadIdx.x + 1);
	uint32_t acc = 0;
	const int wv = threadIdx.x >> 6;
	for (uint32_t i = 0; i < iters; ++i) {
		if constexpr (MODE == 0) {
			uint32_t t[8], p[8];
#pragma unroll
			for (int u = 0; u < 8; ++u) {
				x = murmur64(x + 0x9E3779B97F4A7C15ull);
				load_slot(blob, mod_slots(x, slot_count, magic), t[u], p[u]);
			}
#pragma unroll
			for (int u = 0; u < 8; ++u) acc += t[u] ^ p[u];
		} else if constexpr (MODE == 1) {
			uint32_t lo[8], hi[8];
			const uint32_t *a[8];
#pragma unroll
			for (int u = 0; u < 8; ++u) {
				x = murmur64(x + 0x9E3779B97F4A7C15ull);
				a[u] = reinterpret_cast<const uint32_t *>(blob + ((5ull * mod_slots(x, slot_count, magic)) & ~3ull));
			}
#pragma unroll
			for (int u = 0; u < 8; ++u) {
				asm volatile("global_load_dword %0, %2, off\n\tglobal_load_dword %1, %2, off offset:4" : "=&v"(lo[u]), "=&v"(hi[u]) : "v"(a[u]) : "memory");
			}
			asm volatile("s_waitcnt vmcnt(0)" : "+v"(lo[0]), "+v"(lo[1]), "+v"(lo[2]), "+v"(lo[3]), "+v"(lo[4]), "+v"(lo[5]), "+v"(lo[6]), "+v"(lo[7]),
			             "+v"(hi[0]), "+v"(hi[1]), "+v"(hi[2]), "+v"(hi[3]), "+v"(hi[4]), "+v"(hi[5]), "+v"(hi[6]), "+v"(hi[7])::"memory");
#pragma unroll
			for (int u = 0; u < 8; ++u) acc += lo[u] ^ hi[u];
		} else if constexpr (MODE == 2 || MODE == 3) {
			constexpr int PER = MODE == 2 ? 2 : 3;
#pragma unroll
			for (int u = 0; u < 8; ++u) {
				x = murmur64(x + 0x9E3779B97F4A7C15ull);
				const uint8_t *a = blob + ((5ull * mod_slots(x, slot_count, magic)) & ~3ull);
				if constexpr (MODE == 2) {
					glds_dword(a, lds_addr(dst + ((wv * 8 + u) * PER + 0) * 64));
					glds_dword(a + 4, lds_addr(dst + ((wv * 8 + u) * PER + 1) * 64));
				} else {
					unsigned keep;
					asm volatile("s_mov_b32 %0, m0\n\ts_mov_b32 m0, %2\n\ts_nop 0\n\tglobal_load_lds_dwordx3 %1, off\n\ts_mov_b32 m0, %0"
					             : "=&s"(keep) : "v"(a), "s"(lds_addr(dst + (wv * 8 + u) * PER * 64)) : "memory");
				}
			}
			wait_vm0();
			acc += dst[(wv * 8 * PER) * 64 + (threadIdx.x & 63) + (i & 7) * 64];
		} else {
			uint4 v[8];
#pragma unroll
			for (int u = 0; u < 8; ++u) {
				x = murmur64(x + 0x9E3779B97F4A7C15ull);
				v[u] = *reinterpret_cast<const uint4 *>(blob + ((5ull * mod_slots(x, slot_count, magic)) & ~15ull));
			}
#pragma unroll
			for (int u = 0; u < 8; ++u) acc += v[u].x ^ v[u].w;
		}
	}
	if (acc == 0x12345678u) *sink = acc;
}

hipError_t launch_gather_bench(const DevIndex &X, uint32_t blocks, uint32_t iters, uint32_t *d_sink, hipStream_t s) {
	const char *e = getenv("URMAPX_GATHER_MODE");
	const int mode = e ? atoi(e) : 0;
	if (mode == 1) hipLaunchKernelGGL(gather_bench_kernel<1>, dim3(blocks), dim3(256), 0, s, X.blob, X.slotCount, X.slotMagic, iters, d_sink);
	else if (mode == 2) hipLaunchKernelGGL(gather_bench_kernel<2>, dim3(blocks), dim3(256), 0, s, X.blob, X.slotCount, X.slotMagic, iters, d_sink);
	else if (mode == 3) hipLaunchKernelGGL(gather_bench_kernel<3>, dim3(blocks), dim3(256), 0, s, X.blob, X.slotCount, X.slotMagic, iters, d_sink);
	else if (mode == 4) hipLaunchKernelGGL(gather_bench_kernel<4>, dim3(blocks), dim3(256), 0, s, X.blob, X.slotCount, X.slotMagic, iters, d_sink);
	else hipLaunchKernelGGL(gather_bench_kernel<0>, dim3(blocks), dim3(256), 0, s, X.blob, X.slotCount, X.slotMagic, iters, d_sink);
	return hipGetLastError();
}

size_t viterbi_batch_scratch_stride() { return (WideScratch::bytes(VB_WIDE_LA, VB_WIDE_LB) + 255) & ~(size_t)255; }

hipError_t launch_seed_probe(const DevIndex &X, const uint8_t *d_bases, const uint64_t *d_offs, uint32_t n,
                             uint32_t max_read_len, ProbeOut out, hipStream_t s) {
	if (n == 0) return hipSuccess;
	const int nch = nch_for(max_read_len);
	dim3 block(256), grid((n + 3) / 4);
	if (nch == 2) hipLaunchKernelGGL(seed_probe_kernel<2>, grid, block, 0, s, X, d_bases, d_offs, n, out);
	else if (nch == 3) hipLaunchKernelGGL(seed_probe_kernel<3>, grid, block, 0, s, X, d_bases, d_offs, n, out);
	else if (nch == 4) hipLaunchKernelGGL(seed_probe_kernel<4>, grid, block, 0, s, X, d_bases, d_offs, n, out);
	else if (nch == 5) hipLaunchKernelGGL(seed_probe_kernel<5>, grid, block, 0, s, X, d_bases, d_offs, n, out);
	else if (nch == 8) hipLaunchKernelGGL(seed_probe_kernel<8>, grid, block, 0, s, X, d_bases, d_offs, n, out);
	else hipLaunchKernelGGL(seed_probe_kernel<16>, grid, block, 0, s, X, d_bases, d_offs, n, out);
	return hipGetLastError();
}

hipError_t launch_search_se(const DevIndex &X, const urmapx_params &P, const uint8_t *d_bases, const uint64_t *d_offs,
                            uint32_t n, uint32_t max_read_len, urmapx_result *d_results,
                            urmapx_path_op *d_path_ops, uint32_t *d_path_used, const SearchWork &wk, hipStream_t s) {
	if (n == 0) return hipSuccess;
	const int nch = nch_for(max_read_len);
	{
		hipError_t e = hipMemsetAsync(wk.ticket, 0, 8, s);
		if (e == hipSuccess && wk.ticket3) e = hipMemsetAsync(wk.ticket3, 0, 4, s);
		if (e != hipSuccess) return e;
	}
	if (wk.stats) {
		hipError_t e = hipMemsetAsync(wk.stats + 2, 0, 184, s);
		if (e != hipSuccess) return e;
	}
	{
		hipError_t e = hipMemsetAsync(wk.ovf_list, 0, 4, s);
		if (e != hipSuccess) return e;
	}
	dim3 block(64), grid((unsigned)wk.blocks);
	uint2 *const no_ovf = reinterpret_cast<uint2 *>(wk.scratch + (size_t)wk.blocks * wk.scratch_stride);
	const DpWork no_dp;
	auto stamp = [&](int i) { if (wk.stage_events) (void)hipEventRecord(wk.stage_events[i], s); };
	if (wk.dp[0].jobs && wk.dp[1].jobs && wk.dp[1].counters == wk.dp[0].counters + 4 && wk.dp[0].tickets == wk.dp[0].counters + 16 &&
	    wk.dp[1].tickets == wk.dp[0].tickets + DP_TICKET_WORDS) {
		const bool with3 = wk.dp3.jobs && wk.dp3.counters == wk.dp[0].counters + 8 && wk.dp3.tickets == wk.dp[0].tickets + 2 * DP_TICKET_WORDS;
		hipError_t e = hipMemsetAsync(wk.dp[0].counters, 0, 64 + (with3 ? 3 : 2) * 4 * DP_TICKET_WORDS, s);
		if (e == hipSuccess && wk.dp3.jobs && !with3) {
			e = hipMemsetAsync(wk.dp3.counters, 0, 16, s);
			if (e == hipSuccess) e = hipMemsetAsync(wk.dp3.tickets, 0, 4 * DP_TICKET_WORDS, s);
		}
		if (e != hipSuccess) return e;
	} else
		for (int pass = 0; pass < 2; ++pass)
			if (wk.dp[pass].jobs) {
				hipError_t e = hipMemsetAsync(wk.dp[pass].counters, 0, 16, s);
				if (e == hipSuccess) e = hipMemsetAsync(wk.dp[pass].tickets, 0, 4 * DP_TICKET_WORDS, s);
				if (e != hipSuccess) return e;
			}
#define URX_LAUNCH_SE(NCH_, OVF_, DBG_, GRID_, STATS_, OVFBASE_, DP_)                                                             \
	hipLaunchKernelGGL((search_se_kernel<NCH_, OVF_, DBG_>), GRID_, block, 0, s, X, P, d_bases, d_offs, n, d_results,                \
	                   d_path_ops, d_path_used, STATS_, wk.scratch, wk.scratch_stride, X.seq, X.blob, X.seqp,                    \
	                   wk.ticket + ((OVF_) ? 1 : 0), wk.hsp_lds_cap, wk.ovf_list, OVFBASE_, DP_, no_dp)
#define URX_LAUNCH_SE_ROWS(NCH_, GRID_, STATS_, OVFBASE_, DP_)                                                                      \
	hipLaunchKernelGGL((search_se_kernel<NCH_, false, false, true>), GRID_, block, 0, s, X, P, d_bases, d_offs, n, d_results,          \
	                   d_path_ops, d_path_used, STATS_, wk.scratch, wk.scratch_stride, X.seq, X.blob, X.seqp, wk.ticket,         \
	                   wk.hsp_lds_cap, wk.ovf_list, OVFBASE_, DP_, no_dp)
#define URX_LAUNCH_SE_S16(NCH_, GRID_, OVFBASE_, DP_)                                                                               \
	hipLaunchKernelGGL((search_se_kernel<NCH_, false, false, 2>), GRID_, block, 0, s, X, P, d_bases, d_offs, n, d_results,            \
	                   d_path_ops, d_path_used, no_stats3, wk.scratch, wk.scratch_stride, X.seq, X.blob, X.seqp, wk.ticket,          \
	                   wk.hsp_lds_cap, wk.ovf_list, OVFBASE_, DP_, no_dp)
#define URX_LAUNCH_SE_S16K(NCH_, KCH_, GRID_, OVFBASE_, DP_)                                                                        \
	hipLaunchKernelGGL((search_se_kernel<NCH_, false, false, 2, 0, KCH_>), GRID_, block, 0, s, X, P, d_bases, d_offs, n, d_results,   \
	                   d_path_ops, d_path_used, no_stats3, wk.scratch, wk.scratch_stride, X.seq, X.blob, X.seqp, wk.ticket,          \
	                   wk.hsp_lds_cap, wk.ovf_list, OVFBASE_, DP_, no_dp)
#define URX_LAUNCH_SE_P3(NCH_)                                                                                                      \
	do {                                                                                                                            \
	hipLaunchKernelGGL((search_se_kernel<NCH_, false, false, true, 1>), grid, block, 0, s, X, P, d_bases, d_offs, n, d_results,       \
	                   d_path_ops, d_path_used, no_stats3, wk.scratch, wk.scratch_stride, X.seq, X.blob, X.seqp, wk.ticket,          \
	                   wk.hsp_lds_cap, wk.ovf_list, no_ovf, wk.dp[0], wk.dp3);                                                       \
	stamp(STAGE_P3_MAIN);                                                                                                           \
	hipLaunchKernelGGL((dp_kernel<NCH_>), dim3((unsigned)wk.dp_blocks), block, 0, s, X, P, d_bases, d_offs, wk.dp3,                   \
	                   wk.dp_scratch, wk.dp_scratch_stride, X.seq, 0u, 0xFFFFFFFFu, wk.dp3.tickets, (const uint32_t *)nullptr,       \
	                   wk.dp3.counters);                                                                                             \
	stamp(STAGE_P3_DP);                                                                                                             \
	hipLaunchKernelGGL((search_se_kernel<NCH_, false, false, true, 2>), grid, block, 0, s, X, P, d_bases, d_offs, n, d_results,       \
	                   d_path_ops, d_path_used, no_stats3, wk.scratch, wk.scratch_stride, X.seq, X.blob, X.seqp, wk.ticket3,         \
	                   wk.hsp_lds_cap, wk.ovf_list, no_ovf, wk.dp[0], wk.dp3);                                                       \
	} while (0)
#define URX_LAUNCH_DP(NCH_, OVF_, PASS_)                                                                                          \
	do {  \
	const unsigned dpg = (unsigned)wk.dp_blocks;                                                                                  \
	const unsigned fing = (unsigned)(wk.fin_blocks > 0 ? wk.fin_blocks : wk.blocks), fing2 = PASS_ && fing > 1024u ? 1024u : fing;  \
	const uint32_t *const DP_ROUND_LO = wk.dp_bounds.lo;                                                                          \
	hipLaunchKernelGGL(dp_round_lists_kernel, dim3(PASS_ ? 128 : 2048), dim3(256), 0, s, wk.dp[PASS_], wk.dp_bounds);             \
	for (int rd = 0; rd < DP_ROUNDS; ++rd) {                                                                                      \
		if (rd >= wk.dp_bounds.rounds) { stamp(2 + (2 * DP_ROUNDS + 1) * PASS_ + 2 * rd); stamp(3 + (2 * DP_ROUNDS + 1) * PASS_ + 2 * rd); continue; } \
		hipLaunchKernelGGL((dp_kernel<NCH_>), dim3(dpg), block, 0, s, X, P, d_bases, d_offs, wk.dp[PASS_],                        \
		                   wk.dp_scratch, wk.dp_scratch_stride, X.seq, DP_ROUND_LO[rd], DP_ROUND_LO[rd + 1],                      \
		                   wk.dp[PASS_].tickets + rd, wk.dp[PASS_].round_list + (size_t)rd * wk.dp[PASS_].jobs_cap,               \
		                   wk.dp[PASS_].tickets + 8 + rd);                                                                       \
		stamp(2 + (2 * DP_ROUNDS + 1) * PASS_ + 2 * rd);                                                                            \
		hipLaunchKernelGGL((finalize_se_kernel<NCH_, OVF_>), dim3(fing2), block,                                                  \
		                   0, s, X, P, d_offs, wk.dp[PASS_], d_results, d_path_ops, d_path_used, wk.hsp_lds_cap, wk.ovf_list,        \
		                   DP_ROUND_LO[rd], DP_ROUND_LO[rd + 1]);                                                                  \
		stamp(3 + (2 * DP_ROUNDS + 1) * PASS_ + 2 * rd);                                                                            \
	} } while (0)
	stamp(0);
	const bool diag = wk.stats != nullptr && (nch == 3 || nch == 4);
	uint32_t *const no_stats3 = nullptr;
	const bool k2 = getenv("URMAPX_NO_K2") == nullptr && max_read_len >= X.W && max_read_len - (X.W - 1) <= 128u;
	const bool p3 = !diag && wk.dp3.jobs && wk.dp[0].jobs && wk.dp_blocks > 0 && X.rowinfo && nch <= 5 && wk.stats == nullptr;
	if (p3 && nch == 2) URX_LAUNCH_SE_P3(2);
	else if (p3 && nch == 3) URX_LAUNCH_SE_P3(3);
	else if (p3 && nch == 4) URX_LAUNCH_SE_P3(4);
	else if (p3) URX_LAUNCH_SE_P3(5);
	else if (!diag && X.slot16 && wk.stats == nullptr && nch == 2) URX_LAUNCH_SE_S16(2, grid, no_ovf, wk.dp[0]);
	else if (!diag && X.slot16 && wk.stats == nullptr && nch == 3 && k2) URX_LAUNCH_SE_S16K(3, 2, grid, no_ovf, wk.dp[0]);
	else if (!diag && X.slot16 && wk.stats == nullptr && nch == 3) URX_LAUNCH_SE_S16(3, grid, no_ovf, wk.dp[0]);
	else if (!diag && X.slot16 && wk.stats == nullptr && nch == 4) URX_LAUNCH_SE_S16(4, grid, no_ovf, wk.dp[0]);
	else if (!diag && X.slot16 && wk.stats == nullptr && nch == 5) URX_LAUNCH_SE_S16(5, grid, no_ovf, wk.dp[0]);
	else if (!diag && X.slot16 && wk.stats == nullptr && nch == 8) URX_LAUNCH_SE_S16(8, grid, no_ovf, wk.dp[0]);
	else if (!diag && X.slot16 && wk.stats == nullptr && nch == 16) URX_LAUNCH_SE_S16(16, grid, no_ovf, wk.dp[0]);
	else if (diag && nch == 3) URX_LAUNCH_SE(3, false, true, grid, wk.stats, no_ovf, no_dp);
	else if (diag) URX_LAUNCH_SE(4, false, true, grid, wk.stats, no_ovf, no_dp);
	else if (nch == 2 && X.rowinfo) URX_LAUNCH_SE_ROWS(2, grid, wk.stats, no_ovf, wk.dp[0]);
	else if (nch == 3 && X.rowinfo) URX_LAUNCH_SE_ROWS(3, grid, wk.stats, no_ovf, wk.dp[0]);
	else if (nch == 4 && X.rowinfo) URX_LAUNCH_SE_ROWS(4, grid, wk.stats, no_ovf, wk.dp[0]);
	else if (nch == 5 && X.rowinfo) URX_LAUNCH_SE_ROWS(5, grid, wk.stats, no_ovf, wk.dp[0]);
	else if (nch == 8 && X.rowinfo) URX_LAUNCH_SE_ROWS(8, grid, wk.stats, no_ovf, wk.dp[0]);
	else if (nch == 16 && X.rowinfo) URX_LAUNCH_SE_ROWS(16, grid, wk.stats, no_ovf, wk.dp[0]);
	else if (nch == 2) URX_LAUNCH_SE(2, false, false, grid, wk.stats, no_ovf, wk.dp[0]);
	else if (nch == 3) URX_LAUNCH_SE(3, false, false, grid, wk.stats, no_ovf, wk.dp[0]);
	else if (nch == 4) URX_LAUNCH_SE(4, false, false, grid, wk.stats, no_ovf, wk.dp[0]);
	else if (nch == 5) URX_LAUNCH_SE(5, false, false, grid, wk.stats, no_ovf, wk.dp[0]);
	else if (nch == 8) URX_LAUNCH_SE(8, false, false, grid, wk.stats, no_ovf, wk.dp[0]);
	else URX_LAUNCH_SE(16, false, false, grid, wk.stats, no_ovf, wk.dp[0]);
	if (!p3) { stamp(STAGE_P3_MAIN); stamp(STAGE_P3_DP); }
	stamp(1);
	if (wk.dp[0].jobs && !diag) {
		if (nch == 2) URX_LAUNCH_DP(2, false, 0);
		else if (nch == 3) URX_LAUNCH_DP(3, false, 0);
		else if (nch == 4) URX_LAUNCH_DP(4, false, 0);
		else if (nch == 5) URX_LAUNCH_DP(5, false, 0);
		else if (nch == 8) URX_LAUNCH_DP(8, false, 0);
		else URX_LAUNCH_DP(16, false, 0);
	} else
		for (int i = 0; i < 2 * DP_ROUNDS; ++i) stamp(2 + i);
	{
		hipError_t e = hipGetLastError();
		if (e != hipSuccess) return e;
	}
	dim3 grid2((unsigned)(wk.blocks < SEARCH_OVF_BLOCKS ? wk.blocks : SEARCH_OVF_BLOCKS));
	uint2 *ovf_base = reinterpret_cast<uint2 *>(wk.scratch + (size_t)wk.blocks * wk.scratch_stride);
	uint32_t *const no_stats = nullptr;
	if (nch == 2) URX_LAUNCH_SE(2, true, false, grid2, no_stats, ovf_base, wk.dp[1]);
	else if (nch == 3) URX_LAUNCH_SE(3, true, false, grid2, no_stats, ovf_base, wk.dp[1]);
	else if (nch == 4) URX_LAUNCH_SE(4, true, false, grid2, no_stats, ovf_base, wk.dp[1]);
	else if (nch == 5) URX_LAUNCH_SE(5, true, false, grid2, no_stats, ovf_base, wk.dp[1]);
	else if (nch == 8) URX_LAUNCH_SE(8, true, false, grid2, no_stats, ovf_base, wk.dp[1]);
	else URX_LAUNCH_SE(16, true, false, grid2, no_stats, ovf_base, wk.dp[1]);
	stamp(2 + 2 * DP_ROUNDS);
	if (wk.dp[1].jobs) {
		if (nch == 2) URX_LAUNCH_DP(2, true, 1);
		else if (nch == 3) URX_LAUNCH_DP(3, true, 1);
		else if (nch == 4) URX_LAUNCH_DP(4, true, 1);
		else if (nch == 5) URX_LAUNCH_DP(5, true, 1);
		else if (nch == 8) URX_LAUNCH_DP(8, true, 1);
		else URX_LAUNCH_DP(16, true, 1);
	} else
		for (int i = 0; i < 2 * DP_ROUNDS; ++i) stamp(3 + 2 * DP_ROUNDS + i);
#undef URX_LAUNCH_SE
#undef URX_LAUNCH_SE_ROWS
#undef URX_LAUNCH_SE_P3
#undef URX_LAUNCH_SE_S16
#undef URX_LAUNCH_SE_S16K
#undef URX_LAUNCH_DP
	return hipGetLastError();
}

int dp_block_count(uint32_t max_read_len, int device) {
	hipDeviceProp_t prop;
	if (hipGetDeviceProperties(&prop, device) != hipSuccess) return 0;
	int per_cu = 0;
	const int nchq = nch_for(max_read_len);
	hipError_t e = nchq == 2   ? hipOccupancyMaxActiveBlocksPerMultiprocessor(&per_cu, dp_kernel<2>, 64, 0)
	               : nchq == 3 ? hipOccupancyMaxActiveBlocksPerMultiprocessor(&per_cu, dp_kernel<3>, 64, 0)
	               : nchq == 4 ? hipOccupancyMaxActiveBlocksPerMultiprocessor(&per_cu, dp_kernel<4>, 64, 0)
	               : nchq == 5 ? hipOccupancyMaxActiveBlocksPerMultiprocessor(&per_cu, dp_kernel<5>, 64, 0)
	               : nchq == 8 ? hipOccupancyMaxActiveBlocksPerMultiprocessor(&per_cu, dp_kernel<8>, 64, 0)
	                           : hipOccupancyMaxActiveBlocksPerMultiprocessor(&per_cu, dp_kernel<16>, 64, 0);
	if (e != hipSuccess || per_cu < 1) per_cu = 8;
	return per_cu * prop.multiProcessorCount;
}

int fin_block_count(uint32_t max_read_len, int device) {
	hipDeviceProp_t prop;
	if (hipGetDeviceProperties(&prop, device) != hipSuccess) return 0;
	int per_cu = 0;
	const int nchq = nch_for(max_read_len);
	hipError_t e = nchq == 2   ? hipOccupancyMaxActiveBlocksPerMultiprocessor(&per_cu, finalize_se_kernel<2, false>, 64, 0)
	               : nchq == 3 ? hipOccupancyMaxActiveBlocksPerMultiprocessor(&per_cu, finalize_se_kernel<3, false>, 64, 0)
	               : nchq == 4 ? hipOccupancyMaxActiveBlocksPerMultiprocessor(&per_cu, finalize_se_kernel<4, false>, 64, 0)
	               : nchq == 5 ? hipOccupancyMaxActiveBlocksPerMultiprocessor(&per_cu, finalize_se_kernel<5, false>, 64, 0)
	               : nchq == 8 ? hipOccupancyMaxActiveBlocksPerMultiprocessor(&per_cu, finalize_se_kernel<8, false>, 64, 0)
	                           : hipOccupancyMaxActiveBlocksPerMultiprocessor(&per_cu, finalize_se_kernel<16, false>, 64, 0);
	if (e != hipSuccess || per_cu < 1) per_cu = 16;
	return per_cu * prop.multiProcessorCount;
}

hipError_t launch_viterbi_batch(const urmapx_params &P, const uint8_t *d_a, const uint32_t *d_aoffs,
                                const uint8_t *d_b, const uint32_t *d_boffs, const uint8_t *d_flags, uint32_t n,
                                float *d_scores, uint8_t *d_status, urmapx_path_op *d_ops, uint16_t *d_nops,
                                uint8_t *d_scratch, hipStream_t s) {
	if (n == 0) return hipSuccess;
	const long worst = (long)VB_MAXL * std::max(std::max(std::labs((long)P.mismatch_score), std::labs((long)P.gap_ext_score)), 1L) + std::labs((long)P.gap_open_score);
	if (getenv("URMAPX_VITERBI_PAIR") && worst < 16000)
		hipLaunchKernelGGL(viterbi_batch_pair_kernel, dim3((n + 1) / 2), dim3(64), 0, s, P, d_a, d_aoffs, d_b, d_boffs, d_flags, n, d_scores,
		                   d_status, d_ops, d_nops, d_scratch, viterbi_batch_scratch_stride());
	else
		hipLaunchKernelGGL(viterbi_batch_kernel, dim3(n), dim3(64), 0, s, P, d_a, d_aoffs, d_b, d_boffs, d_flags, n, d_scores,
		                   d_status, d_ops, d_nops, d_scratch, viterbi_batch_scratch_stride());
	return hipGetLastError();
}

}
```

urmap_amd/csrc/urmapx.hip:

```cpp
#include <fcntl.h>
#include <unistd.h>

#include <algorithm>
#include <atomic>
#include <cstdio>
#include <cstdlib>
#include <cstring>
#include <string>
#include <thread>
#include <vector>

#include "internal.h"
#include "kernels.h"

using namespace urx;

namespace {

const uint32_t MAGIC1 = ('U' << 24) | ('F' << 16) | ('I' << 8) | '1';
const uint32_t MAGIC2 = ('U' << 24) | ('F' << 16) | ('I' << 8) | '2';
const uint32_t MAGIC3 = ('U' << 24) | ('F' << 16) | ('I' << 8) | '3';
const uint32_t MAGIC5 = ('U' << 24) | ('F' << 16) | ('I' << 8) | '5';
const size_t SEQ_TAIL_PAD = 4096;
const size_t BLOB_TAIL_PAD = 8;

bool rd(FILE *f, void *p, size_t n) { return fread(p, 1, n, f) == n; }

}

struct urmapx_index {
	uint32_t W = 0, maxIx = 0, seqDataSize = 0;
	uint64_t slotCount = 0;
	std::vector<std::string> labels;
	std::vector<uint32_t> seqLengths, seqOffsets;
	const uint8_t *h_blob = nullptr, *h_seq = nullptr;
	uint8_t *own_blob = nullptr, *own_seq = nullptr;
	int device = -1;
	const uint8_t *d_blob = nullptr, *d_seq = nullptr;
	uint4 *d_seqp = nullptr;
	uint2 *d_rowinfo = nullptr;
	uint32_t *d_rows = nullptr;
	uint4 *d_slot16 = nullptr;
	uint64_t *d_rowbase = nullptr;
	uint64_t n_rows = 0;
	bool own_dev = false;
	uint32_t *d_seqLengths = nullptr, *d_seqOffsets = nullptr;

	DevIndex view() const {
		DevIndex X;
		X.blob = d_blob; X.seq = d_seq; X.seqp = d_seqp; X.slotCount = slotCount;
		X.slotMagic = (uint64_t)((((unsigned __int128)1) << 64) / slotCount);
		X.shiftMask = (W >= 32) ? ~0ull : ((1ull << (2 * W)) - 1ull);
		X.W = W; X.maxIx = maxIx; X.seqDataSize = seqDataSize; X.seqCount = (uint32_t)labels.size();
		X.seqLengths = d_seqLengths; X.seqOffsets = d_seqOffsets;
		X.rowinfo = d_rowinfo; X.rowbase = d_rowbase; X.rows = d_rows; X.slot16 = d_slot16;
		return X;
	}
};

struct urmapx_ctx {
	const urmapx_index *index = nullptr;
	int device = -1;
	hipStream_t stream = nullptr;
	urmapx_params params;
	DevIndex X;
	char arch[64];
	hipEvent_t ev[3] = {nullptr, nullptr, nullptr};
	bool ev_valid = false;
	DevBuf<uint8_t> bases, tallies, vflags, vstatus, va, vb;
	DevBuf<uint64_t> offs, slots;
	DevBuf<uint32_t> positions, used, vaoffs, vboffs;
	DevBuf<urmapx_result> results;
	DevBuf<urmapx_path_op> pathops, vops;
	DevBuf<float> vscores;
	DevBuf<uint16_t> vnops;
	DevBuf<uint8_t> scratch, vscratch;
	DevBuf<uint32_t> statsbuf;
	DevBuf<uint8_t> pe_scratch;
	int pe_veryfast = 0;
	int dp_rounds_used = 3;
	uint32_t dp_bounds_used[DP_ROUNDS + 1] = {0, 2, 16, 0xFFFFFFFFu, 0xFFFFFFFFu};
	int pair_info_on = 0;
	DevBuf<urmapx_pair_info> pairinfo;
	DevBuf<uint32_t> ovflist;
	DevBuf<uint8_t> dpbuf, dpscratch;
	DevBuf<uint8_t> slowscratch;
	DevBuf<uint32_t> slowlist;
	int dp_blocks[6] = {0, 0, 0, 0, 0, 0};
	int fin_blocks[6] = {0, 0, 0, 0, 0, 0};
	hipEvent_t stage_ev[STAGE_EVENTS] = {};
	bool stage_valid = false;
	bool p3_parked = false;
	uint32_t pairinfo_n = 0;
	uint32_t stats_reads = 0;
	int pe_blocks[4] = {0, 0, 0, 0};
	int blocks[6] = {0, 0, 0, 0, 0, 0};
};

namespace urx {
AllocClock &alloc_clock() { static AllocClock c{}; return c; }

__attribute__((constructor)) static void urx_more_hw_queues() { setenv("GPU_MAX_HW_QUEUES", "16", 0); }
hipStream_t ctx_stream(urmapx_ctx *C) { return C->stream; }
int ctx_device(const urmapx_ctx *C) { return C->device; }
const urmapx_index *ctx_index(const urmapx_ctx *C) { return C->index; }
}

extern "C" {

const char *urmapx_strerror(int code) {
	switch (code) {
	case URMAPX_OK: return "ok";
	case URMAPX_E_IO: return "I/O error";
	case URMAPX_E_FORMAT: return "bad .ufi format";
	case URMAPX_E_NOMEM: return "out of memory";
	case URMAPX_E_NODEVICE: return "no usable HIP device / HIP runtime error";
	case URMAPX_E_ARG: return "invalid argument";
	case URMAPX_E_UNSUPPORTED: return "input outside the device path's domain";
	default: return "unknown error";
	}
}

int urmapx_params_for_method(unsigned method, urmapx_params *p) {
	if (!p) return URMAPX_E_ARG;
	if (method == 6 || method == 8) { *p = urmapx_params{-3, -5, -1, 20, 60, 9, 100, 1, 1, 1, 12}; return URMAPX_OK; }
	if (method == 7) { *p = urmapx_params{-4, -6, -2, 35, 35, 12, 75, 8, 6, 5, 8}; return URMAPX_OK; }
	return URMAPX_E_ARG;
}

static int set_directory(urmapx_index *I, uint32_t seq_count, const uint32_t *seq_lengths, const uint32_t *offsets,
                         const char *labels) {
	const char *p = labels;
	for (uint32_t i = 0; i < seq_count; ++i) {
		I->seqLengths.push_back(seq_lengths[i]);
		I->seqOffsets.push_back(offsets[i]);
		I->labels.push_back(std::string(p));
		p += strlen(p) + 1;
	}
	return URMAPX_OK;
}

int urmapx_index_open(const char *path, urmapx_index **out) {
	if (!path || !out) return URMAPX_E_ARG;
	*out = nullptr;
	FILE *f = fopen(path, "rb");
	if (!f) return URMAPX_E_IO;
	urmapx_index *I = new urmapx_index;
	uint32_t u = 0, seqCount = 0;
	bool ok = rd(f, &u, 4) && u == MAGIC1 && rd(f, &I->W, 4) && rd(f, &I->maxIx, 4) && rd(f, &I->seqDataSize, 4) &&
	          rd(f, &I->slotCount, 8) && rd(f, &seqCount, 4);
	for (uint32_t i = 0; ok && i < seqCount; ++i) {
		uint32_t L, off, n;
		ok = rd(f, &L, 4) && rd(f, &off, 4) && rd(f, &n, 4) && n < (1u << 20);
		if (!ok) break;
		std::string s(n, '\0');
		ok = rd(f, &s[0], n);
		I->seqLengths.push_back(L);
		I->seqOffsets.push_back(off);
		I->labels.push_back(std::string(s.c_str()));
	}
	ok = ok && rd(f, &u, 4) && u == MAGIC2 && I->slotCount > 0 && I->W >= 1 && I->W <= 32;
	if (!ok) { fclose(f); delete I; return URMAPX_E_FORMAT; }
	I->own_blob = (uint8_t *)malloc(5 * I->slotCount + BLOB_TAIL_PAD);
	I->own_seq = (uint8_t *)calloc((size_t)I->seqDataSize + SEQ_TAIL_PAD, 1);
	if (!I->own_blob || !I->own_seq) { fclose(f); urmapx_index_close(I); return URMAPX_E_NOMEM; }
	memset(I->own_blob + 5 * I->slotCount, 0, BLOB_TAIL_PAD);
	ok = rd(f, I->own_blob, 5 * I->slotCount) && rd(f, &u, 4) && u == MAGIC3 && rd(f, I->own_seq, I->seqDataSize) &&
	     rd(f, &u, 4) && u == MAGIC5;
	fclose(f);
	if (!ok) { urmapx_index_close(I); return URMAPX_E_FORMAT; }
	I->h_blob = I->own_blob;
	I->h_seq = I->own_seq;
	*out = I;
	return URMAPX_OK;
}

static int upload_directory(urmapx_index *I);

extern "C++" {
int urx::stream_to_device(int fd, uint64_t file_off, size_t nbytes, uint8_t *dev, int threads) {
	constexpr size_t PIECE = 128u << 20;
	constexpr int NS = 3;
	char *stage[NS] = {nullptr, nullptr, nullptr};
	hipEvent_t ev[NS] = {};
	hipStream_t st = nullptr;
	int rc = URMAPX_OK;
	auto cleanup = [&]() {
		if (st) { (void)hipStreamSynchronize(st); (void)hipStreamDestroy(st); }
		for (int k = 0; k < NS; ++k) {
			if (stage[k]) (void)hipHostFree(stage[k]);
			if (ev[k]) (void)hipEventDestroy(ev[k]);
		}
	};
	if (hipStreamCreateWithFlags(&st, hipStreamNonBlocking) != hipSuccess) { st = nullptr; cleanup(); return URMAPX_E_NODEVICE; }
	const size_t stage_bytes = std::min(PIECE, std::max<size_t>(nbytes, 1));
	for (int k = 0; k < NS; ++k)
		if (hipHostMalloc((void **)&stage[k], stage_bytes, hipHostMallocDefault) != hipSuccess ||
		    hipEventCreateWithFlags(&ev[k], hipEventDisableTiming) != hipSuccess) { (void)hipGetLastError(); cleanup(); return URMAPX_E_NOMEM; }
	if (threads < 1) threads = 1;
	size_t piece = 0;
	for (size_t off = 0; off < nbytes && rc == URMAPX_OK; off += PIECE, ++piece) {
		const int k = (int)(piece % NS);
		const size_t n = std::min(PIECE, nbytes - off);
		if (piece >= (size_t)NS && hipEventSynchronize(ev[k]) != hipSuccess) { rc = URMAPX_E_NODEVICE; break; }
		std::atomic<bool> ok{true};
		std::vector<std::thread> th;
		const int T = (int)std::min<size_t>((size_t)threads, (n + (4u << 20) - 1) / (4u << 20));
		for (int t = 0; t < T; ++t)
			th.emplace_back([&, t] {
				const size_t lo = n * (size_t)t / (size_t)T, hi = n * (size_t)(t + 1) / (size_t)T;
				size_t got = lo;
				while (got < hi) {
					const ssize_t r = pread(fd, stage[k] + got, hi - got, (off_t)(file_off + off + got));
					if (r <= 0) { ok.store(false); return; }
					got += (size_t)r;
				}
			});
		for (auto &x : th) x.join();
		if (!ok.load()) { rc = URMAPX_E_FORMAT; break; }
		if (hipMemcpyAsync(dev + off, stage[k], n, hipMemcpyHostToDevice, st) != hipSuccess || hipEventRecord(ev[k], st) != hipSuccess) rc = URMAPX_E_NODEVICE;
	}
	if (st && hipStreamSynchronize(st) != hipSuccess && rc == URMAPX_OK) rc = URMAPX_E_NODEVICE;
	cleanup();
	return rc;
}
}

int urmapx_index_open_device(const char *path, int device, urmapx_index **out) {
	if (!path || !out) return URMAPX_E_ARG;
	*out = nullptr;
	FILE *f = fopen(path, "rb");
	if (!f) return URMAPX_E_IO;
	urmapx_index *I = new urmapx_index;
	uint32_t u = 0, seqCount = 0;
	bool ok = rd(f, &u, 4) && u == MAGIC1 && rd(f, &I->W, 4) && rd(f, &I->maxIx, 4) && rd(f, &I->seqDataSize, 4) &&
	          rd(f, &I->slotCount, 8) && rd(f, &seqCount, 4);
	for (uint32_t i = 0; ok && i < seqCount; ++i) {
		uint32_t L, off, n;
		ok = rd(f, &L, 4) && rd(f, &off, 4) && rd(f, &n, 4) && n < (1u << 20);
		if (!ok) break;
		std::string s(n, '\0');
		ok = rd(f, &s[0], n);
		I->seqLengths.push_back(L);
		I->seqOffsets.push_back(off);
		I->labels.push_back(std::string(s.c_str()));
	}
	ok = ok && rd(f, &u, 4) && u == MAGIC2 && I->slotCount > 0 && I->W >= 1 && I->W <= 32;
	if (!ok) { fclose(f); delete I; return URMAPX_E_FORMAT; }
	const uint64_t blob_off = (uint64_t)ftello(f);
	const size_t nb = 5 * I->slotCount;
	const uint64_t seq_off = blob_off + nb + 4;
	uint32_t m3 = 0, m5 = 0;
	const int fd = fileno(f);
	ok = pread(fd, &m3, 4, (off_t)(blob_off + nb)) == 4 && m3 == MAGIC3 && pread(fd, &m5, 4, (off_t)(seq_off + I->seqDataSize)) == 4 && m5 == MAGIC5;
	if (!ok) { fclose(f); delete I; return URMAPX_E_FORMAT; }
	hipError_t e = hipSetDevice(device);
	uint8_t *db = nullptr, *ds = nullptr;
	if (e == hipSuccess) e = hipMalloc((void **)&db, nb + BLOB_TAIL_PAD);
	if (e == hipSuccess) e = hipMalloc((void **)&ds, (size_t)I->seqDataSize + SEQ_TAIL_PAD);
	if (e != hipSuccess) { (void)hipGetLastError(); if (db) (void)hipFree(db); fclose(f); delete I; return hip_rc(e); }
	I->d_blob = db; I->d_seq = ds; I->own_dev = true; I->device = device;
	int rc = URMAPX_OK;
	if (hipMemset(db + nb, 0, BLOB_TAIL_PAD) != hipSuccess || hipMemset(ds + I->seqDataSize, 0, SEQ_TAIL_PAD) != hipSuccess) rc = URMAPX_E_NODEVICE;
	int threads = (int)std::min(16u, std::max(1u, std::thread::hardware_concurrency()));
	if (const char *e = getenv("URMAPX_LOAD_THREADS")) threads = std::max(1, std::min(256, atoi(e)));
	const auto t0 = std::chrono::steady_clock::now();
	if (!rc) rc = stream_to_device(fd, blob_off, nb, db, threads);
	if (!rc) rc = stream_to_device(fd, seq_off, I->seqDataSize, ds, threads);
	fclose(f);
	const auto t1 = std::chrono::steady_clock::now();
	if (!rc) rc = upload_directory(I);
	if (getenv("URMAPX_VERBOSE"))
		fprintf(stderr, "urmapx: index streamed to device %d: %.2f GB in %.2f s (%d reader threads), resident layouts built in %.2f s\n", device,
		        (double)(nb + I->seqDataSize) / 1e9, std::chrono::duration<double>(t1 - t0).count(), threads,
		        std::chrono::duration<double>(std::chrono::steady_clock::now() - t1).count());
	if (rc) { urmapx_index_close(I); return rc; }
	*out = I;
	return URMAPX_OK;
}

int urmapx_index_wrap_host(uint32_t W, uint32_t max_ix, uint64_t slot_count, const uint8_t *blob, const uint8_t *seqdata,
                           uint32_t seqdata_size, uint32_t seq_count, const uint32_t *seq_lengths,
                           const uint32_t *offsets, const char *labels, urmapx_index **out) {
	if (!out || !blob || !seqdata || slot_count == 0 || W < 1 || W > 32) return URMAPX_E_ARG;
	urmapx_index *I = new urmapx_index;
	I->W = W; I->maxIx = max_ix; I->slotCount = slot_count; I->seqDataSize = seqdata_size;
	I->h_blob = blob; I->h_seq = seqdata;
	set_directory(I, seq_count, seq_lengths, offsets, labels);
	*out = I;
	return URMAPX_OK;
}

static int build_packed_seq(urmapx_index *I) {
	HIP_TRY(hipMalloc((void **)&I->d_seqp, packed_seq_blocks(I->seqDataSize) * sizeof(uint4)));
	HIP_TRY(launch_pack_seq(I->d_seq, I->seqDataSize, I->d_seqp, nullptr));
	HIP_TRY(hipDeviceSynchronize());
	return URMAPX_OK;
}

static int upload_directory(urmapx_index *I) {
	int rc = build_packed_seq(I);
	if (rc) return rc;
	if (!getenv("URMAPX_NO_CHAIN_ROWS") && !getenv("URMAPX_NO_SLOT16") && !getenv("URMAPX_PARK_PHASE3") && !getenv("URMAPX_KEEP_ROWINFO") && !getenv("URMAPX_TWO_STEP_LAYOUT")) {
		const hipError_t e = build_slot16_direct(I->d_blob, I->slotCount, I->maxIx, &I->d_slot16, &I->d_rows, &I->n_rows);
		if (getenv("URMAPX_VERBOSE"))
			fprintf(stderr, "urmapx: slot16 + rows %s in one build: %llu positions in rows, %.2f GB (hip: %s)\n", I->d_slot16 ? "built" : "NOT built",
			        (unsigned long long)I->n_rows, I->d_slot16 ? (16.0 * (double)I->slotCount + 4.0 * (double)I->n_rows) / 1e9 : 0.0, hipGetErrorString(e));
		HIP_TRY(e);
	}
	if (!I->d_slot16 && !getenv("URMAPX_NO_CHAIN_ROWS")) {
		const hipError_t e = build_chain_rows(I->d_blob, I->slotCount, I->maxIx, &I->d_rowinfo, &I->d_rowbase, &I->d_rows, &I->n_rows);
		if (getenv("URMAPX_VERBOSE"))
			fprintf(stderr, "urmapx: chain rows %s: %llu positions in rows, %.2f GB (hip: %s)\n", I->d_rows ? "built" : "NOT built",
			        (unsigned long long)I->n_rows, I->d_rowinfo ? (8.0 * (double)I->slotCount + 4.0 * (double)I->n_rows) / 1e9 : 0.0, hipGetErrorString(e));
		HIP_TRY(e);
		if (I->d_rowinfo && !getenv("URMAPX_NO_SLOT16")) {
			const hipError_t e2 = build_slot16(I->d_blob, I->slotCount, I->d_rowinfo, I->d_rowbase, I->d_rows, &I->d_slot16);
			if (getenv("URMAPX_VERBOSE")) fprintf(stderr, "urmapx: slot16 table %s (%.2f GB)\n", I->d_slot16 ? "built" : "NOT built", 16.0 * (double)I->slotCount / 1e9);
			HIP_TRY(e2);
			if (I->d_slot16 && !getenv("URMAPX_PARK_PHASE3") && !getenv("URMAPX_KEEP_ROWINFO")) {
				(void)hipFree(I->d_rowinfo); I->d_rowinfo = nullptr;
				(void)hipFree(I->d_rowbase); I->d_rowbase = nullptr;
			}
		}
		static bool warned = false;
		if (!I->d_rowinfo && !I->d_slot16 && !warned) {
			warned = true;
			fprintf(stderr, "urmapx: the chain-row layout of the index was not built on device %d (no room for it, or MaxIx over 32): "
			                "collision chains are walked link by link\n", I->device);
		}
	}
	size_t n = I->labels.size();
	HIP_TRY(hipMalloc((void **)&I->d_seqLengths, (n + 1) * 4));
	HIP_TRY(hipMalloc((void **)&I->d_seqOffsets, (n + 1) * 4));
	HIP_TRY(hipMemcpy(I->d_seqLengths, I->seqLengths.data(), n * 4, hipMemcpyHostToDevice));
	HIP_TRY(hipMemcpy(I->d_seqOffsets, I->seqOffsets.data(), n * 4, hipMemcpyHostToDevice));
	return URMAPX_OK;
}

int urmapx_index_wrap_device(int device, uint32_t W, uint32_t max_ix, uint64_t slot_count, const void *d_blob,
                             const void *d_seqdata, uint32_t seqdata_size, uint32_t seq_count,
                             const uint32_t *seq_lengths, const uint32_t *offsets, const char *labels,
                             urmapx_index **out) {
	if (!out || !d_blob || !d_seqdata || slot_count == 0 || W < 1 || W > 32) return URMAPX_E_ARG;
	HIP_TRY(hipSetDevice(device));
	urmapx_index *I = new urmapx_index;
	I->W = W; I->maxIx = max_ix; I->slotCount = slot_count; I->seqDataSize = seqdata_size;
	I->device = device; I->d_blob = (const uint8_t *)d_blob; I->d_seq = (const uint8_t *)d_seqdata; I->own_dev = false;
	set_directory(I, seq_count, seq_lengths, offsets, labels);
	int rc = upload_directory(I);
	if (rc) { urmapx_index_close(I); return rc; }
	*out = I;
	return URMAPX_OK;
}

int urmapx_index_upload(urmapx_index *I, int device) {
	if (!I) return URMAPX_E_ARG;
	if (I->d_blob && I->device == device) return URMAPX_OK;
	if (I->d_blob) return URMAPX_E_ARG;
	if (!I->h_blob || !I->h_seq) return URMAPX_E_ARG;
	HIP_TRY(hipSetDevice(device));
	uint8_t *db = nullptr, *ds = nullptr;
	const size_t nb = 5 * I->slotCount;
	HIP_TRY(hipMalloc((void **)&db, nb + BLOB_TAIL_PAD));
	hipError_t e = hipMalloc((void **)&ds, (size_t)I->seqDataSize + SEQ_TAIL_PAD);
	if (e != hipSuccess) { (void)hipFree(db); return hip_rc(e); }
	I->d_blob = db; I->d_seq = ds; I->own_dev = true; I->device = device;
	HIP_TRY(hipMemset(db + nb, 0, BLOB_TAIL_PAD));
	HIP_TRY(hipMemset(ds + I->seqDataSize, 0, SEQ_TAIL_PAD));
	HIP_TRY(hipMemcpy(db, I->h_blob, nb, hipMemcpyHostToDevice));
	HIP_TRY(hipMemcpy(ds, I->h_seq, I->seqDataSize, hipMemcpyHostToDevice));
	return upload_directory(I);
}

int urmapx_index_replicate(const urmapx_index *src, int device, urmapx_index **out) {
	if (!src || !out || ((!src->h_blob || !src->h_seq) && (!src->d_blob || !src->d_seq))) return URMAPX_E_ARG;
	*out = nullptr;
	urmapx_index *I = new urmapx_index;
	I->W = src->W; I->maxIx = src->maxIx; I->seqDataSize = src->seqDataSize; I->slotCount = src->slotCount;
	I->labels = src->labels; I->seqLengths = src->seqLengths; I->seqOffsets = src->seqOffsets;
	int rc;
	if (src->h_blob && src->h_seq) {
		I->h_blob = src->h_blob; I->h_seq = src->h_seq;
		rc = urmapx_index_upload(I, device);
	} else {
		const size_t nb = 5 * I->slotCount;
		uint8_t *db = nullptr, *ds = nullptr;
		hipError_t e = hipSetDevice(device);
		if (e == hipSuccess) e = hipMalloc((void **)&db, nb + BLOB_TAIL_PAD);
		if (e == hipSuccess) e = hipMalloc((void **)&ds, (size_t)I->seqDataSize + SEQ_TAIL_PAD);
		if (e != hipSuccess) { (void)hipGetLastError(); if (db) (void)hipFree(db); delete I; return hip_rc(e); }
		I->d_blob = db; I->d_seq = ds; I->own_dev = true; I->device = device;
// ... 7 lines not shown
	return URMAPX_OK;
}

void urmapx_index_close(urmapx_index *I) {
	if (!I) return;
	lane_pool_purge(I);
	if (I->own_dev) { (void)hipFree((void *)I->d_blob); (void)hipFree((void *)I->d_seq); }
	if (I->d_seqp) (void)hipFree(I->d_seqp);
	if (I->d_slot16) (void)hipFree(I->d_slot16);
	if (I->d_rowinfo) (void)hipFree(I->d_rowinfo);
	if (I->d_rowbase) (void)hipFree(I->d_rowbase);
	if (I->d_rows) (void)hipFree(I->d_rows);
	if (I->d_seqLengths) (void)hipFree(I->d_seqLengths);
	if (I->d_seqOffsets) (void)hipFree(I->d_seqOffsets);
	free(I->own_blob);
	free(I->own_seq);
	delete I;
}

uint64_t urmapx_index_chain_row_bytes(const urmapx_index *I) {
	if (!I) return 0ull;
	return (I->d_rowinfo ? 8ull * I->slotCount + 8ull * ((I->slotCount + 1023) / 1024) : 0ull) + (I->d_rows ? 4ull * (I->n_rows + 64) : 0ull) +
	       (I->d_slot16 ? 16ull * (I->slotCount + 1) : 0ull);
}
int urmapx_index_validate(const urmapx_index *I, urmapx_validate_report *out) {
	if (!I || !out) return URMAPX_E_ARG;
	memset(out, 0, sizeof *out);
	out->first_bad_slot = ~0ull;
	if (!I->d_blob || !I->d_seq || I->device < 0) return URMAPX_E_ARG;
	HIP_TRY(hipSetDevice(I->device));
	uint64_t v[9];
	float ms = 0.f;
	HIP_TRY(validate_index(I->view(), v, &ms));
	out->slots = I->slotCount;
	out->heads = v[0]; out->positions = v[1]; out->used = v[2]; out->reached = v[3];
	out->bad_hash = v[4]; out->bad_pos = v[5]; out->bad_link = v[6]; out->bad_len = v[7]; out->first_bad_slot = v[8];
	out->seconds = ms * 1e-3;
	const bool ok = !v[4] && !v[5] && !v[6] && !v[7] && v[2] == v[3];
	return ok ? URMAPX_OK : URMAPX_E_FORMAT;
}
int urmapx_index_stats(const urmapx_index *I, urmapx_ufi_stats *out) {
	if (!I || !out) return URMAPX_E_ARG;
	memset(out, 0, sizeof *out);
	out->first_bad_slot = ~0ull;
	if (!I->d_blob || !I->d_seq || I->device < 0) return URMAPX_E_ARG;
	if (I->W < 1 || I->W > 32) return URMAPX_E_UNSUPPORTED;
	HIP_TRY(hipSetDevice(I->device));
	uint64_t c[UFI_STATS_COUNTERS], hist[512], first_bad = ~0ull;
	float ms[2] = {0.f, 0.f};
	HIP_TRY(ufi_stats_device(I->view(), c, hist, &first_bad, ms));
	out->word_length = I->W; out->max_ix = I->maxIx; out->seqdata_size = I->seqDataSize; out->slots = I->slotCount;
	out->indexed = c[0]; out->not_indexed = c[1]; out->wildcard = c[2];
	out->indexed2 = c[3]; out->free = c[4]; out->collision = c[5]; out->single_both = c[6]; out->single_plus = c[7]; out->end = c[8];
	out->mine = c[9]; out->other = c[10]; out->trunc = c[11]; out->trunc2 = c[12]; out->long_mine = c[13]; out->long_other = c[14];
	out->total = c[15]; out->bad_rows = c[16]; out->first_bad_slot = first_bad;
	memcpy(out->count_hist, hist, sizeof out->count_hist);
	memcpy(out->trunc_hist, hist + 256, sizeof out->trunc_hist);
	out->position_seconds = ms[0] * 1e-3;
	out->slot_seconds = ms[1] * 1e-3;
	return out->bad_rows ? URMAPX_E_FORMAT : URMAPX_OK;
}
int urmapx_index_slot_counts(const urmapx_index *I, int minus, uint8_t *host_out, uint64_t n) {
	if (!I || !host_out || n != I->slotCount) return URMAPX_E_ARG;
	if (!I->d_blob || !I->d_seq || I->device < 0) return URMAPX_E_ARG;
	if (I->W < 1 || I->W > 32) return URMAPX_E_UNSUPPORTED;
	HIP_TRY(hipSetDevice(I->device));
	HIP_TRY(ufi_slot_counts_device(I->view(), minus, host_out));
	return URMAPX_OK;
}
int urmapx_ufi_info(const char *path, uint32_t *word_length, uint32_t *max_ix, uint32_t *seqdata_size, uint64_t *slot_count) {
	if (!path) return URMAPX_E_ARG;
	FILE *f = fopen(path, "rb");
	if (!f) return URMAPX_E_IO;
	uint32_t u = 0, w = 0, m = 0, sd = 0;
	uint64_t sc = 0;
	const bool got = rd(f, &u, 4) && (u != MAGIC1 || (rd(f, &w, 4) && rd(f, &m, 4) && rd(f, &sd, 4) && rd(f, &sc, 8)));
	fclose(f);
	if (!got) return URMAPX_E_IO;
	if (u != MAGIC1) return URMAPX_E_FORMAT;
	if (word_length) *word_length = w;
	if (max_ix) *max_ix = m;
	if (seqdata_size) *seqdata_size = sd;
	if (slot_count) *slot_count = sc;
	return URMAPX_OK;
}
int urmapx_checksum_device(int device, const void *d_ptr, uint64_t nbytes, uint64_t *out) {
	if (!d_ptr || !out || ((uintptr_t)d_ptr & 7)) return URMAPX_E_ARG;
	HIP_TRY(hipSetDevice(device));
	HIP_TRY(checksum_device(d_ptr, nbytes, out));
	return URMAPX_OK;
}
int urmapx_index_checksum(const urmapx_index *I, uint64_t out[2]) {
	if (!I || !out) return URMAPX_E_ARG;
	if (!I->d_blob || !I->d_seq || I->device < 0) return URMAPX_E_ARG;
	HIP_TRY(hipSetDevice(I->device));
	HIP_TRY(checksum_device(I->d_blob, 5ull * I->slotCount, &out[0]));
	HIP_TRY(checksum_device(I->d_seq, I->seqDataSize, &out[1]));
	return URMAPX_OK;
}
int urmapx_index_layout_checksum(const urmapx_index *I, uint64_t out[2]) {
	if (!I || !out) return URMAPX_E_ARG;
	if (!I->d_blob || I->device < 0) return URMAPX_E_ARG;
	out[0] = out[1] = 0;
	HIP_TRY(hipSetDevice(I->device));
	if (I->d_slot16) HIP_TRY(checksum_device(I->d_slot16, 16ull * I->slotCount, &out[0]));
	if (I->d_rows) HIP_TRY(checksum_device(I->d_rows, 4ull * I->n_rows, &out[1]));
	return URMAPX_OK;
}
uint32_t urmapx_index_word_length(const urmapx_index *I) { return I->W; }
uint32_t urmapx_index_max_ix(const urmapx_index *I) { return I->maxIx; }
uint64_t urmapx_index_slot_count(const urmapx_index *I) { return I->slotCount; }
uint32_t urmapx_index_seqdata_size(const urmapx_index *I) { return I->seqDataSize; }
uint32_t urmapx_index_seq_count(const urmapx_index *I) { return (uint32_t)I->labels.size(); }
const char *urmapx_index_label(const urmapx_index *I, uint32_t i) { return i < I->labels.size() ? I->labels[i].c_str() : nullptr; }
uint32_t urmapx_index_seq_length(const urmapx_index *I, uint32_t i) { return i < I->seqLengths.size() ? I->seqLengths[i] : 0; }
uint32_t urmapx_index_seq_offset(const urmapx_index *I, uint32_t i) { return i < I->seqOffsets.size() ? I->seqOffsets[i] : 0; }

int urmapx_ctx_create(const urmapx_index *I, int device, const urmapx_params *P, urmapx_ctx **out) {
	if (!I || !P || !out) return URMAPX_E_ARG;
	*out = nullptr;
	if (!I->d_blob || I->device != device) return URMAPX_E_ARG;
	HIP_TRY(hipSetDevice(device));
	urmapx_ctx *C = new urmapx_ctx;
	C->index = I; C->device = device; C->params = *P; C->X = I->view();
	hipDeviceProp_t prop;
	hipError_t e = hipGetDeviceProperties(&prop, device);
	if (e != hipSuccess) { delete C; return hip_rc(e); }
	snprintf(C->arch, sizeof C->arch, "%s", prop.gcnArchName);
	if (char *colon = strchr(C->arch, ':')) *colon = 0;
	e = hipStreamCreateWithFlags(&C->stream, hipStreamNonBlocking);
	if (e != hipSuccess) { delete C; return hip_rc(e); }
	for (int i = 0; i < 3; ++i) {
		e = hipEventCreate(&C->ev[i]);
		if (e != hipSuccess) { urmapx_ctx_destroy(C); return hip_rc(e); }
	}
	for (int i = 0; i < STAGE_EVENTS; ++i) {
		e = hipEventCreate(&C->stage_ev[i]);
		if (e != hipSuccess) { urmapx_ctx_destroy(C); return hip_rc(e); }
	}
	*out = C;
	return URMAPX_OK;
}

void urmapx_ctx_destroy(urmapx_ctx *C) {
	if (!C) return;
	(void)hipSetDevice(C->device);
	if (C->stream) (void)hipStreamSynchronize(C->stream);
	C->bases.release(); C->tallies.release(); C->vflags.release(); C->vstatus.release(); C->va.release(); C->vb.release();
	C->offs.release(); C->slots.release(); C->positions.release(); C->used.release(); C->vaoffs.release(); C->vboffs.release();
	C->results.release(); C->pathops.release(); C->vops.release(); C->vscores.release(); C->vnops.release();
	C->dpbuf.release(); C->dpscratch.release(); C->slowscratch.release(); C->slowlist.release();
	for (int i = 0; i < STAGE_EVENTS; ++i)
		if (C->stage_ev[i]) (void)hipEventDestroy(C->stage_ev[i]);
	C->scratch.release(); C->vscratch.release(); C->statsbuf.release(); C->pe_scratch.release(); C->pairinfo.release(); C->ovflist.release();
	for (int i = 0; i < 3; ++i)
		if (C->ev[i]) (void)hipEventDestroy(C->ev[i]);
	if (C->stream) (void)hipStreamDestroy(C->stream);
	delete C;
}

const char *urmapx_device_arch(urmapx_ctx *C) { return C ? C->arch : nullptr; }

int urmapx_ctx_phase_cycles(urmapx_ctx *C, uint64_t out[12]) {
	if (!C || !out || !C->statsbuf.p) return URMAPX_E_ARG;
	HIP_TRY(hipStreamSynchronize(C->stream));
	uint64_t buf[13];
	HIP_TRY(hipMemcpy(buf, C->statsbuf.p, sizeof buf, hipMemcpyDeviceToHost));
	for (int i = 0; i < 12; ++i) out[i] = buf[i + 1];
	return URMAPX_OK;
}

int urmapx_ctx_stage_ms(urmapx_ctx *C, float ms[7]) {
	if (!C || !ms) return URMAPX_E_ARG;
	if (!C->stage_valid) { for (int i = 0; i < 7; ++i) ms[i] = 0; return URMAPX_OK; }
	HIP_TRY(hipEventSynchronize(C->stage_ev[STAGE_LAST]));
	auto span = [&](int a, int b, float &out) -> hipError_t { float t = 0; hipError_t e = hipEventElapsedTime(&t, C->stage_ev[a], C->stage_ev[b]); out += t; return e; };
	for (int i = 0; i < 7; ++i) ms[i] = 0;
	HIP_TRY(span(0, 1, ms[0]));
	for (int p = 0; p < 2; ++p) {
		const int b = 1 + (2 * DP_ROUNDS + 1) * p;
		for (int rd = 0; rd < DP_ROUNDS; ++rd) {
			HIP_TRY(span(b + 2 * rd, b + 2 * rd + 1, ms[1 + 3 * p]));
			HIP_TRY(span(b + 2 * rd + 1, b + 2 * rd + 2, ms[2 + 3 * p]));
		}
	}
	HIP_TRY(span(1 + 2 * DP_ROUNDS, 2 + 2 * DP_ROUNDS, ms[3]));
	HIP_TRY(span(STAGE_LAST - 1, STAGE_LAST, ms[6]));
	return URMAPX_OK;
}

int urmapx_ctx_phase3(urmapx_ctx *C, float ms[3], uint32_t stats[2]) {
	if (!C || !ms || !stats) return URMAPX_E_ARG;
	ms[0] = ms[1] = ms[2] = 0; stats[0] = stats[1] = 0;
	if (!C->stage_valid || !C->dpbuf.p || !C->p3_parked) return URMAPX_OK;
	HIP_TRY(hipEventSynchronize(C->stage_ev[STAGE_LAST]));
	HIP_TRY(hipEventElapsedTime(&ms[0], C->stage_ev[0], C->stage_ev[STAGE_P3_MAIN]));
	HIP_TRY(hipEventElapsedTime(&ms[1], C->stage_ev[STAGE_P3_MAIN], C->stage_ev[STAGE_P3_DP]));
	HIP_TRY(hipEventElapsedTime(&ms[2], C->stage_ev[STAGE_P3_DP], C->stage_ev[1]));
	uint32_t buf[2];
	HIP_TRY(hipMemcpy(buf, C->dpbuf.p + 32, sizeof buf, hipMemcpyDeviceToHost));
	stats[0] = buf[0]; stats[1] = buf[1];
	return URMAPX_OK;
}

int urmapx_ctx_round_ms(urmapx_ctx *C, float ms[16], int *rounds) {
	if (!C || !ms || !rounds) return URMAPX_E_ARG;
	static_assert(2 * DP_ROUNDS <= 16, "ms[16]");
	for (int i = 0; i < 16; ++i) ms[i] = 0;
	*rounds = C->dp_rounds_used;
	if (!C->stage_valid) return URMAPX_OK;
	HIP_TRY(hipEventSynchronize(C->stage_ev[STAGE_LAST]));
	for (int i = 0; i < 2 * C->dp_rounds_used; ++i) HIP_TRY(hipEventElapsedTime(&ms[i], C->stage_ev[1 + i], C->stage_ev[2 + i]));
	return URMAPX_OK;
}

int urmapx_ctx_dp_rounds(urmapx_ctx *C, uint32_t lo[8], int *rounds) {
	if (!C || !lo || !rounds) return URMAPX_E_ARG;
	*rounds = C->dp_rounds_used;
	for (int i = 0; i < 8; ++i) lo[i] = i <= DP_ROUNDS ? C->dp_bounds_used[i] : 0xFFFFFFFFu;
	return URMAPX_OK;
}

int urmapx_ctx_dp_stats(urmapx_ctx *C, uint32_t out[8]) {
	if (!C || !out || !C->dpbuf.p) return URMAPX_E_ARG;
	HIP_TRY(hipStreamSynchronize(C->stream));
	uint32_t buf[8];
	HIP_TRY(hipMemcpy(buf, C->dpbuf.p, sizeof buf, hipMemcpyDeviceToHost));
	for (int p = 0; p < 2; ++p)
		for (int i = 0; i < 4; ++i) out[4 * p + i] = buf[4 * p + i];
	return URMAPX_OK;
}

int urmapx_ctx_read_cycles(urmapx_ctx *C, uint32_t *out, uint32_t n) {
	if (!C || !out || !C->statsbuf.p || n > C->stats_reads) return URMAPX_E_ARG;
	HIP_TRY(hipStreamSynchronize(C->stream));
	HIP_TRY(hipMemcpy(out, C->statsbuf.p + 64, (size_t)n * 4, hipMemcpyDeviceToHost));
	return URMAPX_OK;
}

int urmapx_ctx_sync(urmapx_ctx *C) {
	if (!C) return URMAPX_E_ARG;
	HIP_TRY(hipStreamSynchronize(C->stream));
	return URMAPX_OK;
}

int urmapx_ctx_last_kernel_ms(urmapx_ctx *C, float ms[2]) {
	if (!C || !ms || !C->ev_valid) return URMAPX_E_ARG;
	HIP_TRY(hipEventSynchronize(C->ev[2]));
	HIP_TRY(hipEventElapsedTime(&ms[0], C->ev[0], C->ev[1]));
	HIP_TRY(hipEventElapsedTime(&ms[1], C->ev[1], C->ev[2]));
	return URMAPX_OK;
}

static constexpr int PE_SLOW_BLOCKS = 32;

static int ensure_probe(urmapx_ctx *C, uint64_t total_bases) {
	int rc;
	if ((rc = C->slots.ensure(2 * total_bases + 64))) return rc;
	if ((rc = C->tallies.ensure(2 * total_bases + 64))) return rc;
	if ((rc = C->positions.ensure(2 * total_bases + 64))) return rc;
	return URMAPX_OK;
}

int urmapx_map_se_device(urmapx_ctx *C, const void *d_bases, const void *d_offs, uint32_t n, uint64_t total_bases,
                         uint32_t max_read_len, void *d_results, void *d_path_ops, void *d_path_used) {
	if (!C || (n && (!d_bases || !d_offs || !d_results || !d_path_ops || !d_path_used))) return URMAPX_E_ARG;
	if (max_read_len > URMAPX_MAX_QL_SLOW) return URMAPX_E_UNSUPPORTED;
	HIP_TRY(hipSetDevice(C->device));
	(void)total_bases;
	int rc;
	const uint32_t slow_qcap = max_read_len < URMAPX_MAX_QL ? URMAPX_MAX_QL : max_read_len;
	if (max_read_len > URMAPX_MAX_QL) max_read_len = URMAPX_MAX_QL;
	const int cls = max_read_len <= 128 ? 3 : max_read_len <= 192 ? 0 : max_read_len <= 256 ? 2 : max_read_len <= 320 ? 1 : max_read_len <= 512 ? 4 : 5;
	if (C->blocks[cls] == 0) {
		C->blocks[cls] = search_block_count(max_read_len, C->device);
		if (getenv("URMAPX_VERBOSE")) fprintf(stderr, "urmapx: search_se_kernel grid = %d persistent blocks (read class %d)\n", C->blocks[cls], cls);
	}
	if (C->blocks[cls] <= 0) return URMAPX_E_NODEVICE;
	SearchWork wk;
	wk.blocks = C->blocks[cls];
	wk.scratch_stride = search_scratch_stride(max_read_len);
	if ((rc = C->scratch.ensure(wk.scratch_stride * (size_t)wk.blocks + search_scratch_tail(wk.blocks)))) return rc;
	if ((rc = C->ovflist.ensure((size_t)n + 1))) return rc;
	wk.ovf_list = C->ovflist.p;
	const char *ds = getenv("URMAPX_DEBUG_STOP");
	const bool diag = getenv("URMAPX_PHASE_STATS") || ds;
	if ((rc = C->statsbuf.ensure(64 + (diag ? (size_t)n : 0)))) return rc;
	C->stats_reads = diag ? n : 0;
	wk.scratch = C->scratch.p;
	wk.ticket = C->statsbuf.p + 62;
	wk.ticket3 = C->statsbuf.p + 58;
	if (const char *e = getenv("URMAPX_TEST_HSP_LDS_CAP")) wk.hsp_lds_cap = atoi(e);
	wk.stats = diag ? C->statsbuf.p : nullptr;
	if (wk.stats) {
		const uint32_t ctl[2] = {ds ? (uint32_t)atoi(ds) : 0u, getenv("URMAPX_PHASE_STATS") ? 0u : 1u};
		HIP_TRY(hipMemcpyAsync(C->statsbuf.p, ctl, 8, hipMemcpyHostToDevice, C->stream));
	}
	if (!getenv("URMAPX_INLINE_PHASE6")) {
		if (C->dp_blocks[cls] == 0) C->dp_blocks[cls] = dp_block_count(max_read_len, C->device);
		if (C->dp_blocks[cls] <= 0) return URMAPX_E_NODEVICE;
		wk.dp_blocks = C->dp_blocks[cls];
		if (C->fin_blocks[cls] == 0) C->fin_blocks[cls] = fin_block_count(max_read_len, C->device);
		wk.fin_blocks = C->fin_blocks[cls] > 0 ? C->fin_blocks[cls] : 0;
		wk.dp_scratch_stride = dp_scratch_stride(max_read_len);
		wk.dp_bounds = dp_bounds_default(max_read_len > 192);
		if (const char *e = getenv("URMAPX_DP_BOUNDS")) {
			DpBounds b;
			b.rounds = 0;
			for (const char *c = e; *c && b.rounds < DP_ROUNDS;) {
				char *end;
				const unsigned long v = strtoul(c, &end, 10);
				if (end == c) break;
				b.lo[b.rounds++] = (uint32_t)v;
				c = *end == ',' ? end + 1 : end;
			}
			bool ok = b.rounds >= 1 && b.lo[0] == 0;
			for (int i = 1; i < b.rounds; ++i) ok = ok && b.lo[i] > b.lo[i - 1];
			if (ok) {
				for (int i = b.rounds; i <= DP_ROUNDS; ++i) b.lo[i] = 0xFFFFFFFFu;
				wk.dp_bounds = b;
			}
		}
		C->dp_rounds_used = wk.dp_bounds.rounds;
		for (int i = 0; i <= DP_ROUNDS; ++i) C->dp_bounds_used[i] = wk.dp_bounds.lo[i];
		if ((rc = C->dpscratch.ensure(wk.dp_scratch_stride * (size_t)wk.dp_blocks))) return rc;
		wk.dp_scratch = C->dpscratch.p;
		const uint64_t jc = (uint64_t)n * 16u;
		const uint32_t jobs_cap[2] = {(uint32_t)(jc < (1ull << 30) ? jc : (1ull << 30)) + 4096u,
		                              (uint32_t)(jc < (1ull << 30) ? jc : (1ull << 30)) + 65536u};
		const uint32_t fin_cap[2] = {n, n / 8u + 1024u};
		size_t need = 256, at[2][7];
		for (int p = 0; p < 2; ++p) {
			at[p][5] = need; need += (((size_t)jobs_cap[p] * 2) + 63) & ~(size_t)63;
			at[p][0] = need; need += (size_t)jobs_cap[p] * sizeof(DpJob);
			at[p][1] = need; need += (((size_t)jobs_cap[p] * DP_JOB_OPS * 2) + 63) & ~(size_t)63;
			at[p][2] = need; need += (((size_t)fin_cap[p] * 16) + 63) & ~(size_t)63;
			at[p][3] = need; need += (size_t)fin_cap[p] * dp_state_words(p == 1) * 4;
			at[p][4] = 16 * (size_t)p;
			at[p][6] = need; need += (((size_t)jobs_cap[p] * 4 * DP_ROUNDS) + 63) & ~(size_t)63;
		}
		const char *park3 = getenv("URMAPX_PARK_PHASE3");
		size_t p3w = (park3 && atoi(park3) > 0) ? p3_state_words(max_read_len) : 0;
		if (p3w && !C->X.rowinfo) {
			static std::atomic<bool> said{false};
			if (!said.exchange(true)) fprintf(stderr, "urmapx: URMAPX_PARK_PHASE3 is set but the index was uploaded without it (its row layout is gone): phase 3 stays inline\n");
			p3w = 0;
		}
		uint32_t jobs_cap3 = (uint32_t)((uint64_t)n * 2u < (1ull << 30) ? (uint64_t)n * 2u : (1ull << 30)) + 4096u;
		uint32_t fin_cap3 = n;
		if (const char *e = getenv("URMAPX_TEST_P3_JOBS_CAP")) jobs_cap3 = (uint32_t)atoi(e) + 1u;
		if (const char *e = getenv("URMAPX_TEST_P3_FIN_CAP")) fin_cap3 = std::min<uint32_t>(n, (uint32_t)atoi(e));
		size_t at3[5] = {0, 0, 0, 0, 0};
		if (p3w) {
			at3[4] = need; need += (((size_t)jobs_cap3 * 2) + 63) & ~(size_t)63;
			at3[0] = need; need += (size_t)jobs_cap3 * sizeof(DpJob);
			at3[1] = need; need += (((size_t)jobs_cap3 * DP_JOB_OPS * 2) + 63) & ~(size_t)63;
			at3[2] = need; need += (((size_t)fin_cap3 * 16) + 63) & ~(size_t)63;
			at3[3] = need; need += (size_t)fin_cap3 * p3w * 4;
		}
		if ((rc = C->dpbuf.ensure(need))) return rc;
		C->p3_parked = p3w != 0;
		if (p3w) {
			DpWork &d = wk.dp3;
			d.jobs = reinterpret_cast<DpJob *>(C->dpbuf.p + at3[0]);
			d.ops = reinterpret_cast<uint16_t *>(C->dpbuf.p + at3[1]);
			d.kidx = reinterpret_cast<uint16_t *>(C->dpbuf.p + at3[4]);
			d.fin_list = reinterpret_cast<uint32_t *>(C->dpbuf.p + at3[2]);
			d.state = reinterpret_cast<uint32_t *>(C->dpbuf.p + at3[3]);
			d.counters = reinterpret_cast<uint32_t *>(C->dpbuf.p + 32);
			d.tickets = reinterpret_cast<uint32_t *>(C->dpbuf.p + 64 + 4 * DP_TICKET_WORDS * (size_t)2);
			d.jobs_cap = jobs_cap3; d.fin_cap = fin_cap3;
		}
		for (int p = 0; p < 2; ++p) {
			DpWork &d = wk.dp[p];
			d.jobs = reinterpret_cast<DpJob *>(C->dpbuf.p + at[p][0]);
			d.ops = reinterpret_cast<uint16_t *>(C->dpbuf.p + at[p][1]);
			d.kidx = reinterpret_cast<uint16_t *>(C->dpbuf.p + at[p][5]);
			d.round_list = reinterpret_cast<uint32_t *>(C->dpbuf.p + at[p][6]);
			d.fin_list = reinterpret_cast<uint32_t *>(C->dpbuf.p + at[p][2]);
			d.state = reinterpret_cast<uint32_t *>(C->dpbuf.p + at[p][3]);
			d.counters = reinterpret_cast<uint32_t *>(C->dpbuf.p + at[p][4]);
			d.tickets = reinterpret_cast<uint32_t *>(C->dpbuf.p + 64 + 4 * DP_TICKET_WORDS * (size_t)p);
			d.jobs_cap = jobs_cap[p]; d.fin_cap = fin_cap[p];
		}
	}
	const bool stamps = getenv("URMAPX_NO_STAGE_STAMPS") == nullptr;
	wk.stage_events = stamps ? C->stage_ev : nullptr;
	HIP_TRY(hipMemsetAsync(d_path_used, 0, 4, C->stream));
	HIP_TRY(hipEventRecord(C->ev[0], C->stream));
	HIP_TRY(hipEventRecord(C->ev[1], C->stream));
	C->stage_valid = stamps && n > 0;
	const int sblocks = slow_qcap <= URMAPX_MAX_QL ? 128 : 64;
	if ((rc = C->slowscratch.ensure(slow_scratch_stride(slow_qcap) * (size_t)sblocks))) return rc;
	if ((rc = C->slowlist.ensure((size_t)n + 2))) return rc;
	HIP_TRY(launch_search_se(C->X, C->params, (const uint8_t *)d_bases, (const uint64_t *)d_offs, n, max_read_len,
	                         (urmapx_result *)d_results, (urmapx_path_op *)d_path_ops, (uint32_t *)d_path_used, wk, C->stream));
	if (!getenv("URMAPX_TEST_NO_GENERAL")) {
		const uint64_t pcap = (uint64_t)n * URMAPX_MAX_PATH_OPS;
		HIP_TRY(launch_search_se_slow(C->X, C->params, (const uint8_t *)d_bases, (const uint64_t *)d_offs, n, slow_qcap,
		                              (urmapx_result *)d_results, (urmapx_path_op *)d_path_ops, (uint32_t *)d_path_used,
		                              (uint32_t)(pcap > 0xFFFFFFFFull ? 0xFFFFFFFFull : pcap), C->slowscratch.p, sblocks, C->slowlist.p + 1,
		                              C->slowlist.p, C->stream));
	}
	if (stamps) HIP_TRY(hipEventRecord(C->stage_ev[STAGE_LAST], C->stream));
	HIP_TRY(hipEventRecord(C->ev[2], C->stream));
	C->ev_valid = true;
	return URMAPX_OK;
}

static uint32_t max_len(const uint64_t *offs, uint32_t n) {
	uint64_t m = 0;
	for (uint32_t i = 0; i < n; ++i) m = offs[i + 1] - offs[i] > m ? offs[i + 1] - offs[i] : m;
	return m > 0xFFFFFFFFull ? 0xFFFFFFFFu : (uint32_t)m;
}

int urmapx_map_se(urmapx_ctx *C, const uint8_t *bases, const uint64_t *offs, uint32_t n, urmapx_result *results,
                  urmapx_path_op *path_ops, size_t path_cap, size_t *path_used) {
	if (!C || (n && (!bases || !offs || !results))) return URMAPX_E_ARG;
	if (path_used) *path_used = 0;
	if (n == 0) return URMAPX_OK;
	HIP_TRY(hipSetDevice(C->device));
	const uint64_t total = offs[n];
	uint32_t mx = max_len(offs, n);
	if (mx > URMAPX_MAX_QL_SLOW) mx = URMAPX_MAX_QL_SLOW;
	int rc;
	if ((rc = C->bases.ensure(total + 64))) return rc;
	if ((rc = C->offs.ensure((size_t)n + 1))) return rc;
	if ((rc = C->results.ensure(n))) return rc;
	if ((rc = C->pathops.ensure((size_t)n * URMAPX_MAX_PATH_OPS))) return rc;
	if ((rc = C->used.ensure(1))) return rc;
	HIP_TRY(hipMemcpyAsync(C->bases.p, bases, total, hipMemcpyHostToDevice, C->stream));
	HIP_TRY(hipMemcpyAsync(C->offs.p, offs, ((size_t)n + 1) * 8, hipMemcpyHostToDevice, C->stream));
	rc = urmapx_map_se_device(C, C->bases.p, C->offs.p, n, total, mx, C->results.p, C->pathops.p, C->used.p);
	if (rc) return rc;
	uint32_t used = 0;
	HIP_TRY(hipMemcpyAsync(results, C->results.p, (size_t)n * sizeof(urmapx_result), hipMemcpyDeviceToHost, C->stream));
	HIP_TRY(hipMemcpyAsync(&used, C->used.p, 4, hipMemcpyDeviceToHost, C->stream));
	HIP_TRY(hipStreamSynchronize(C->stream));
	if (used > path_cap || (used && !path_ops)) return URMAPX_E_ARG;
	if (used) HIP_TRY(hipMemcpy(path_ops, C->pathops.p, (size_t)used * sizeof(urmapx_path_op), hipMemcpyDeviceToHost));
	if (path_used) *path_used = used;
	for (uint32_t i = 0; i < n; ++i)
		if (results[i].status) return URMAPX_E_UNSUPPORTED;
	return URMAPX_OK;
}

int urmapx_ctx_set_pair_info(urmapx_ctx *C, int on) {
	if (!C) return URMAPX_E_ARG;
	C->pair_info_on = on ? 1 : 0;
	return URMAPX_OK;
}

int urmapx_ctx_get_pair_info(urmapx_ctx *C, urmapx_pair_info *out, uint32_t npairs) {
	if (!C || !out || npairs > C->pairinfo_n || !C->pairinfo.p) return URMAPX_E_ARG;
	HIP_TRY(hipSetDevice(C->device));
	HIP_TRY(hipStreamSynchronize(C->stream));
	HIP_TRY(hipMemcpy(out, C->pairinfo.p, (size_t)npairs * sizeof(urmapx_pair_info), hipMemcpyDeviceToHost));
	return URMAPX_OK;
}

int urmapx_ctx_set_pe_veryfast(urmapx_ctx *C, int on) {
	if (!C) return URMAPX_E_ARG;
	C->pe_veryfast = on ? 1 : 0;
	return URMAPX_OK;
}

int urmapx_map_pe_device(urmapx_ctx *C, const void *d_bases, const void *d_offs, uint32_t npairs, uint64_t total_bases,
                         uint32_t max_read_len, void *d_results, void *d_path_ops, void *d_path_used) {
	if (!C || (npairs && (!d_bases || !d_offs || !d_results || !d_path_ops || !d_path_used))) return URMAPX_E_ARG;
	if (max_read_len > MAX_QL_PE || npairs > 0x7FFFFFFFu) return URMAPX_E_UNSUPPORTED;
	HIP_TRY(hipSetDevice(C->device));
	int rc;
	(void)total_bases;
	C->stage_valid = false;
	const int cls = max_read_len <= 128 ? 3 : max_read_len <= 192 ? 0 : (max_read_len <= 256 ? 2 : 1);
	if (C->pe_blocks[cls] == 0) C->pe_blocks[cls] = search_pe_block_count(max_read_len, C->device);
	if (C->pe_blocks[cls] <= 0) return URMAPX_E_NODEVICE;
	SearchWork wk;
	wk.blocks = C->pe_blocks[cls];
	wk.scratch_stride = search_pe_scratch_stride(max_read_len);
	if ((rc = C->pe_scratch.ensure(wk.scratch_stride * (size_t)wk.blocks + search_pe_scratch_tail(wk.blocks)))) return rc;
	if ((rc = C->ovflist.ensure(2 * ((size_t)npairs + 1)))) return rc;
	if ((rc = C->slowscratch.ensure(pe_slow_scratch_stride() * (size_t)PE_SLOW_BLOCKS))) return rc;
	if ((rc = C->slowlist.ensure((size_t)npairs + 2))) return rc;
	wk.ovf_list = C->ovflist.p;
	if (const char *e = getenv("URMAPX_TEST_HSP_LDS_CAP")) wk.hsp_lds_cap = atoi(e);
	wk.scratch = C->pe_scratch.p;
	wk.stats = nullptr;
	if ((rc = C->statsbuf.ensure(64))) return rc;
	wk.ticket = C->statsbuf.p + 62;
	HIP_TRY(hipMemsetAsync(d_path_used, 0, 4, C->stream));
	HIP_TRY(hipEventRecord(C->ev[0], C->stream));
	HIP_TRY(hipEventRecord(C->ev[1], C->stream));
	urmapx_params Ppe = C->params;
	if (C->pe_veryfast) Ppe.band_radius = 4;
	urmapx_pair_info *d_info = nullptr;
	if (C->pair_info_on) {
		if ((rc = C->pairinfo.ensure(npairs))) return rc;
		d_info = C->pairinfo.p;
		C->pairinfo_n = npairs;
	}
	HIP_TRY(launch_search_pe(C->X, Ppe, (const uint8_t *)d_bases, (const uint64_t *)d_offs, npairs, max_read_len,
	                         (urmapx_result *)d_results, (urmapx_path_op *)d_path_ops, (uint32_t *)d_path_used, wk,
	                         C->pe_veryfast | (getenv("URMAPX_DEBUG_STOP_PE") ? atoi(getenv("URMAPX_DEBUG_STOP_PE")) << 8 : 0), d_info, C->stream));
	{
		const uint64_t pcap = (uint64_t)npairs * 2 * URMAPX_MAX_PATH_OPS;
		HIP_TRY(launch_search_pe_slow(C->X, Ppe, (const uint8_t *)d_bases, (const uint64_t *)d_offs, npairs, (urmapx_result *)d_results,
		                              (urmapx_path_op *)d_path_ops, (uint32_t *)d_path_used, (uint32_t)(pcap > 0xFFFFFFFFull ? 0xFFFFFFFFull : pcap),
		                              C->slowscratch.p, PE_SLOW_BLOCKS, C->slowlist.p + 1, C->slowlist.p, C->pe_veryfast, d_info,
		                              getenv("URMAPX_TEST_PE_GENERAL") != nullptr, C->stream));
	}
	HIP_TRY(hipEventRecord(C->ev[2], C->stream));
	C->ev_valid = true;
	return URMAPX_OK;
}

int urmapx_map_pe(urmapx_ctx *C, const uint8_t *bases, const uint64_t *offs, uint32_t npairs, urmapx_result *results,
                  urmapx_path_op *path_ops, size_t path_cap, size_t *path_used) {
	if (!C || (npairs && (!bases || !offs || !results))) return URMAPX_E_ARG;
	if (path_used) *path_used = 0;
	if (npairs == 0) return URMAPX_OK;
	if (npairs > 0x7FFFFFFFu) return URMAPX_E_ARG;
	HIP_TRY(hipSetDevice(C->device));
	const uint32_t n = 2 * npairs;
	const uint64_t total = offs[n];
	uint32_t mx = max_len(offs, n);
	if (mx > MAX_QL_PE) mx = MAX_QL_PE;
	int rc;
	if ((rc = C->bases.ensure(total + 64))) return rc;
	if ((rc = C->offs.ensure((size_t)n + 1))) return rc;
	if ((rc = C->results.ensure(n))) return rc;
	if ((rc = C->pathops.ensure((size_t)n * URMAPX_MAX_PATH_OPS))) return rc;
	if ((rc = C->used.ensure(1))) return rc;
	HIP_TRY(hipMemcpyAsync(C->bases.p, bases, total, hipMemcpyHostToDevice, C->stream));
	HIP_TRY(hipMemcpyAsync(C->offs.p, offs, ((size_t)n + 1) * 8, hipMemcpyHostToDevice, C->stream));
	if ((rc = urmapx_map_pe_device(C, C->bases.p, C->offs.p, npairs, total, mx, C->results.p, C->pathops.p, C->used.p))) return rc;
	uint32_t used = 0;
	HIP_TRY(hipMemcpyAsync(results, C->results.p, (size_t)n * sizeof(urmapx_result), hipMemcpyDeviceToHost, C->stream));
	HIP_TRY(hipMemcpyAsync(&used, C->used.p, 4, hipMemcpyDeviceToHost, C->stream));
	HIP_TRY(hipStreamSynchronize(C->stream));
	if (used > path_cap || (used && !path_ops)) return URMAPX_E_ARG;
	if (used) HIP_TRY(hipMemcpy(path_ops, C->pathops.p, (size_t)used * sizeof(urmapx_path_op), hipMemcpyDeviceToHost));
	if (path_used) *path_used = used;
	for (uint32_t i = 0; i < n; ++i)
		if (results[i].status) return URMAPX_E_UNSUPPORTED;
	return URMAPX_OK;
}

int urmapx_seed_probe(urmapx_ctx *C, const uint8_t *bases, const uint64_t *offs, uint32_t n, uint64_t *slots,
                      uint8_t *tallies, uint32_t *positions) {
	if (!C || (n && (!bases || !offs || !slots || !tallies || !positions))) return URMAPX_E_ARG;
	if (n == 0) return URMAPX_OK;
	HIP_TRY(hipSetDevice(C->device));
	const uint64_t total = offs[n];
	uint32_t mx = max_len(offs, n);
	if (mx > URMAPX_MAX_QL) return URMAPX_E_UNSUPPORTED;
	int rc;
	if ((rc = C->bases.ensure(total + 64))) return rc;
	if ((rc = C->offs.ensure((size_t)n + 1))) return rc;
	if ((rc = ensure_probe(C, total))) return rc;
	HIP_TRY(hipMemcpyAsync(C->bases.p, bases, total, hipMemcpyHostToDevice, C->stream));
	HIP_TRY(hipMemcpyAsync(C->offs.p, offs, ((size_t)n + 1) * 8, hipMemcpyHostToDevice, C->stream));
	HIP_TRY(hipMemsetAsync(C->slots.p, 0xFF, 2 * total * 8, C->stream));
	HIP_TRY(hipMemsetAsync(C->tallies.p, 0, 2 * total, C->stream));
	HIP_TRY(hipMemsetAsync(C->positions.p, 0xFF, 2 * total * 4, C->stream));
	ProbeOut po{C->slots.p, C->tallies.p, C->positions.p};
	HIP_TRY(launch_seed_probe(C->X, C->bases.p, C->offs.p, n, mx, po, C->stream));
	HIP_TRY(hipMemcpyAsync(slots, C->slots.p, 2 * total * 8, hipMemcpyDeviceToHost, C->stream));
	HIP_TRY(hipMemcpyAsync(tallies, C->tallies.p, 2 * total, hipMemcpyDeviceToHost, C->stream));
	HIP_TRY(hipMemcpyAsync(positions, C->positions.p, 2 * total * 4, hipMemcpyDeviceToHost, C->stream));
	HIP_TRY(hipStreamSynchronize(C->stream));
	return URMAPX_OK;
}

int urmapx_seed_probe_device(urmapx_ctx *C, const void *d_bases, const void *d_offs, uint32_t n, uint64_t total_bases, uint32_t max_read_len,
                             float *ms) {
	if (!C || !ms || (n && (!d_bases || !d_offs))) return URMAPX_E_ARG;
	*ms = 0;
	if (n == 0) return URMAPX_OK;
	if (max_read_len > URMAPX_MAX_QL) return URMAPX_E_UNSUPPORTED;
	HIP_TRY(hipSetDevice(C->device));
	int rc;
	if ((rc = ensure_probe(C, total_bases))) return rc;
	ProbeOut po{C->slots.p, C->tallies.p, C->positions.p};
	hipEvent_t e0, e1;
	HIP_TRY(hipEventCreate(&e0));
	HIP_TRY(hipEventCreate(&e1));
	HIP_TRY(hipEventRecord(e0, C->stream));
	hipError_t e = launch_seed_probe(C->X, (const uint8_t *)d_bases, (const uint64_t *)d_offs, n, max_read_len, po, C->stream);
	if (e == hipSuccess) e = hipEventRecord(e1, C->stream);
	if (e == hipSuccess) e = hipEventSynchronize(e1);
	if (e == hipSuccess) e = hipEventElapsedTime(ms, e0, e1);
	(void)hipEventDestroy(e0);
	(void)hipEventDestroy(e1);
	return hip_rc(e);
}

int urmapx_ctx_gather_microbench(urmapx_ctx *C, uint64_t n_loads, double *loads_per_s) {
	if (!C || !loads_per_s || n_loads == 0) return URMAPX_E_ARG;
	HIP_TRY(hipSetDevice(C->device));
	int rc;
	if ((rc = C->statsbuf.ensure(64))) return rc;
	hipDeviceProp_t prop;
	HIP_TRY(hipGetDeviceProperties(&prop, C->device));
	const uint32_t blocks = (uint32_t)prop.multiProcessorCount * 8u;
	uint64_t per_iter = (uint64_t)blocks * 256u * 8u;
	uint32_t iters = (uint32_t)((n_loads + per_iter - 1) / per_iter);
	if (iters == 0) iters = 1;
	hipEvent_t e0, e1;
	HIP_TRY(hipEventCreate(&e0));
	HIP_TRY(hipEventCreate(&e1));
	HIP_TRY(launch_gather_bench(C->X, blocks, 1, C->statsbuf.p + 60, C->stream));
	HIP_TRY(hipEventRecord(e0, C->stream));
	HIP_TRY(launch_gather_bench(C->X, blocks, iters, C->statsbuf.p + 60, C->stream));
	HIP_TRY(hipEventRecord(e1, C->stream));
	HIP_TRY(hipEventSynchronize(e1));
	float ms = 0;
	HIP_TRY(hipEventElapsedTime(&ms, e0, e1));
	(void)hipEventDestroy(e0);
	(void)hipEventDestroy(e1);
	*loads_per_s = ms > 0 ? (double)per_iter * iters / (ms * 1e-3) : 0.0;
	return URMAPX_OK;
}

int urmapx_viterbi_batch(urmapx_ctx *C, const uint8_t *a, const uint32_t *a_offs, const uint8_t *b, const uint32_t *b_offs,
                         const uint8_t *flags, uint32_t n, float *scores, uint8_t *status, urmapx_path_op *ops,
                         uint16_t *nops) {
	if (!C || (n && (!a_offs || !b_offs || !flags || !scores || !status || !ops || !nops))) return URMAPX_E_ARG;
	if (n == 0) return URMAPX_OK;
	HIP_TRY(hipSetDevice(C->device));
	const size_t ta = a_offs[n], tb = b_offs[n];
	int rc;
	if ((rc = C->va.ensure(ta + 64))) return rc;
	if ((rc = C->vb.ensure(tb + 64))) return rc;
	if ((rc = C->vaoffs.ensure((size_t)n + 1))) return rc;
	if ((rc = C->vboffs.ensure((size_t)n + 1))) return rc;
	if ((rc = C->vflags.ensure(n))) return rc;
	if ((rc = C->vstatus.ensure(n))) return rc;
	if ((rc = C->vscores.ensure(n))) return rc;
	if ((rc = C->vnops.ensure(n))) return rc;
	if ((rc = C->vops.ensure((size_t)n * URMAPX_MAX_PATH_OPS))) return rc;
	if ((rc = C->vscratch.ensure((size_t)n * viterbi_batch_scratch_stride()))) return rc;
	if (ta) HIP_TRY(hipMemcpyAsync(C->va.p, a, ta, hipMemcpyHostToDevice, C->stream));
	if (tb) HIP_TRY(hipMemcpyAsync(C->vb.p, b, tb, hipMemcpyHostToDevice, C->stream));
	HIP_TRY(hipMemcpyAsync(C->vaoffs.p, a_offs, ((size_t)n + 1) * 4, hipMemcpyHostToDevice, C->stream));
	HIP_TRY(hipMemcpyAsync(C->vboffs.p, b_offs, ((size_t)n + 1) * 4, hipMemcpyHostToDevice, C->stream));
	HIP_TRY(hipMemcpyAsync(C->vflags.p, flags, n, hipMemcpyHostToDevice, C->stream));
	HIP_TRY(launch_viterbi_batch(C->params, C->va.p, C->vaoffs.p, C->vb.p, C->vboffs.p, C->vflags.p, n, C->vscores.p,
	                             C->vstatus.p, C->vops.p, C->vnops.p, C->vscratch.p, C->stream));
	HIP_TRY(hipMemcpyAsync(scores, C->vscores.p, (size_t)n * 4, hipMemcpyDeviceToHost, C->stream));
	HIP_TRY(hipMemcpyAsync(status, C->vstatus.p, n, hipMemcpyDeviceToHost, C->stream));
	HIP_TRY(hipMemcpyAsync(nops, C->vnops.p, (size_t)n * 2, hipMemcpyDeviceToHost, C->stream));
	HIP_TRY(hipMemcpyAsync(ops, C->vops.p, (size_t)n * URMAPX_MAX_PATH_OPS * 2, hipMemcpyDeviceToHost, C->stream));
	HIP_TRY(hipStreamSynchronize(C->stream));
	return URMAPX_OK;
}

}
```

Baseline: 58.37 million.

## Fuse per-round DP finalize into DP kernel via per-read job countdown

Each DP round now finalizes a read inside the DP kernel once its last job in that round completes. A per-read, per-round counter filled by the round-lists kernel is decremented atomically, and this replaces the separate finalize_se kernel launch after each round. Job results are written with agent-scope relaxed atomics so the finishing wave can read them. The overflow pass is gated on the overflow list and its grid is capped at the CU count. The change aims to cut kernel launches and serialization between DP and finalize, at the cost of extra atomics, LDS use and occupancy pressure in the fused kernel.

```diff
diff --git a/urmap_amd/csrc/kernels.h b/urmap_amd/csrc/kernels.h
--- a/urmap_amd/csrc/kernels.h
+++ b/urmap_amd/csrc/kernels.h
@@ -98,6 +98,8 @@
 	size_t dp_scratch_stride = 0;
 	int dp_blocks = 0;
 	int fin_blocks = 0;
+	uint32_t *dp_fin_cnt[2] = {nullptr, nullptr};
+	int cus = 0;
 	DpBounds dp_bounds = dp_bounds_default(false);
 	hipEvent_t *stage_events = nullptr;
 };
diff --git a/urmap_amd/csrc/kernels.hip b/urmap_amd/csrc/kernels.hip
--- a/urmap_amd/csrc/kernels.hip
+++ b/urmap_amd/csrc/kernels.hip
@@ -1,4 +1,5 @@
 #include <algorithm>
+#include <cstddef>
 #include <cstdlib>
 
 #include "kernels.h"
@@ -8,6 +9,17 @@
 #include "viterbi_dev.h"
 
 namespace urx {
+
+template <bool XW, class T>
+__device__ __forceinline__ void st_xw(T *p, T v) {
+	if constexpr (XW) __hip_atomic_store(p, v, __ATOMIC_RELAXED, __HIP_MEMORY_SCOPE_AGENT);
+	else *p = v;
+}
+template <bool XW, class T>
+__device__ __forceinline__ T ld_xw(const T *p) {
+	if constexpr (XW) return __hip_atomic_load(p, __ATOMIC_RELAXED, __HIP_MEMORY_SCOPE_AGENT);
+	else return *p;
+}
 
 template <int NCH>
 __global__ __launch_bounds__(256) void seed_probe_kernel(DevIndex X, const uint8_t *__restrict__ bases,
@@ -541,6 +553,7 @@
 		return (int)(f >> 8);
 	}
 
+	template <bool XW = false>
 	__device__ bool consume_job(const DpJob &J, const uint16_t *jops) {
 		const uint32_t pk = J.pk;
 		const int startq = (int)(pk & PK_MASK), len = (int)((pk >> PK_LEN_SH) & PK_MASK);
@@ -572,7 +585,7 @@
 		if (J.flags & DPJ_PATH_LONG) { status |= URMAPX_ST_PATH_OVERFLOW; return true; }
 		const int nc = (int)J.nops;
 		URX_SYNC();
-		for (int t = lane; t < nc; t += 64) cand[t] = jops[t];
+		for (int t = lane; t < nc; t += 64) cand[t] = ld_xw<XW>(jops + t);
 		URX_SYNC();
 		add_hit(J.combined_tlo, plus, totalScore, nc);
 		return true;
@@ -1336,10 +1349,32 @@
 	}
 }
 
-__global__ __launch_bounds__(256) void dp_round_lists_kernel(DpWork dp, DpBounds bounds) {
+__global__ __launch_bounds__(256) void dp_round_lists_kernel(DpWork dp, DpBounds bounds, const uint32_t *gate, uint32_t *fin_cnt) {
+	if (gate && *gate == 0) return;
 	const uint32_t *const DP_ROUND_LO = bounds.lo;
 	constexpr int PER = 16;
 	__shared__ uint32_t cnt[DP_ROUNDS], base[DP_ROUNDS];
+	if (fin_cnt) {
+		const uint32_t parked = dp.counters[1] < dp.fin_cap ? dp.counters[1] : dp.fin_cap;
+		const uint4 *const fin = reinterpret_cast<const uint4 *>(dp.fin_list);
+		const uint32_t lane = threadIdx.x & 63u;
+		for (uint32_t e = blockIdx.x * 4u + (threadIdx.x >> 6); e < parked; e += gridDim.x * 4u) {
+			const uint4 ent = fin[e];
+			const uint32_t jb = ent.y, nj = ent.z;
+			if (lane == 0) {
+				uint4 c;
+				uint32_t *const cw = &c.x;
+#pragma unroll
+				for (int rd = 0; rd < DP_ROUNDS; ++rd) {
+					const uint32_t lo = DP_ROUND_LO[rd] < nj ? DP_ROUND_LO[rd] : nj, hi = DP_ROUND_LO[rd + 1] < nj ? DP_ROUND_LO[rd + 1] : nj;
+					cw[rd] = hi > lo ? hi - lo : 0u;
+				}
+				static_assert(DP_ROUNDS == 4, "one 16-byte store per read");
+				*reinterpret_cast<uint4 *>(fin_cnt + (size_t)e * DP_ROUNDS) = c;
+			}
+			for (uint32_t k = lane; k < nj; k += 64u) dp.jobs[jb + k].combined_tlo = e;
+		}
+	}
 	const uint32_t made = dp.counters[0];
 	const uint32_t njobs = made < dp.jobs_cap ? made : dp.jobs_cap;
 	for (uint32_t c0 = blockIdx.x * 256u * PER; c0 < njobs; c0 += gridDim.x * 256u * PER) {
@@ -1378,11 +1413,144 @@
 	}
 }
 
-template <int NCH>
-__global__ __launch_bounds__(64) void dp_kernel(DevIndex X, urmapx_params P, const uint8_t *__restrict__ bases,
-                                                const uint64_t *__restrict__ offs, DpWork dp, uint8_t *scratch,
-                                                size_t scratch_stride, const uint8_t *__restrict__ g_seq, uint32_t klo, uint32_t khi,
-                                                uint32_t *ticket, const uint32_t *__restrict__ list, const uint32_t *list_count) {
+template <int PBUF_OPS, int PEND>
+struct FinPaths {
+	static_assert(PEND <= 64 && PBUF_OPS >= URMAPX_MAX_PATH_OPS, "one pending read per lane; room for the longest path");
+	uint16_t *pbuf;
+	uint32_t *pend_r;
+	urmapx_result *pend_res;
+	int used = 0, n = 0;
+	__device__ __forceinline__ void flush(int lane, urmapx_result *__restrict__ results, urmapx_path_op *__restrict__ path_ops, uint32_t *path_used) {
+		if (n == 0) return;
+		URX_SYNC();
+		uint32_t po = 0;
+		if (lane == 0) po = atomicAdd(path_used, (uint32_t)used);
+		po = uni(po);
+		for (int t = lane; t < used; t += 64) path_ops[po + t] = pbuf[t];
+		if (lane < n) {
+			urmapx_result rr = pend_res[lane];
+			rr.path_off += po;
+			results[pend_r[lane]] = rr;
+		}
+		URX_SYNC();
+		used = 0; n = 0;
+	}
+};
+
+template <bool XW, int NCH, bool OVF, int PBUF_OPS, int PEND>
+__device__ __forceinline__ uint32_t finalize_read_round(SearchWave<NCH, OVF> &S, FinPaths<PBUF_OPS, PEND> &pb, const DpWork &dp, uint32_t e, uint4 ent,
+                                                        uint32_t klo, uint32_t khi, urmapx_result *__restrict__ results,
+                                                        urmapx_path_op *__restrict__ path_ops, uint32_t *path_used, uint32_t *ovf_list, int lane) {
+	using SW = SearchWave<NCH, OVF>;
+	const uint32_t r = uni(ent.x), jb = uni(ent.y), nj = uni(ent.z);
+	S.QL = (int)uni(ent.w);
+	if (nj <= klo) return 0;
+	S.nwords = S.QL - (S.W - 1);
+	const uint32_t kend = nj < khi ? nj : khi;
+	uint32_t jpk0 = 0;
+	uint4 jw0 = make_uint4(0u, 0u, 0u, 0u);
+	auto job_words = [&](const uint32_t *jp) {
+		if constexpr (XW) return make_uint4(ld_xw<true>(jp + 4), ld_xw<true>(jp + 5), ld_xw<true>(jp + 6), 0u);
+		else return *reinterpret_cast<const uint4 *>(jp + 4);
+	};
+	if (klo + (uint32_t)lane < kend) {
+		const uint32_t *jp = reinterpret_cast<const uint32_t *>(dp.jobs + jb + klo + (uint32_t)lane);
+		jpk0 = jp[2];
+		jw0 = job_words(jp);
+	}
+	URX_SYNC();
+	uint32_t *const st = dp.state + (size_t)e * SW::STATE_WORDS;
+	const int phase = S.restore_state(st);
+	uint32_t used = 0;
+	for (uint32_t k0 = klo; k0 < kend; k0 += 64) {
+		const uint32_t k = k0 + (uint32_t)lane;
+		const uint32_t jpk = jpk0;
+		const uint4 jw = jw0;
+		jpk0 = 0; jw0 = make_uint4(0u, 0u, 0u, 0u);
+		if (k + 64u < kend) {
+			const uint32_t *jp = reinterpret_cast<const uint32_t *>(dp.jobs + jb + k + 64u);
+			jpk0 = jp[2];
+			jw0 = job_words(jp);
+		}
+		const int jstartq = (int)(jpk & PK_MASK), jlen = (int)((jpk >> PK_LEN_SH) & PK_MASK), jhs = (int)((jpk >> PK_SCORE_SH) & PK_MASK);
+		const int jpen = jlen - jhs;
+		const int jls = (int)(int16_t)(jw.y & 0xFFFFu), jrs = (int)(int16_t)(jw.y >> 16);
+		const uint32_t jfl = (jw.z >> 8) & 0xFFu;
+		const bool has_l = jstartq > 0, has_r = jstartq + jlen < S.QL;
+		const bool raises = (jw.z >> 16) != 0u || (jfl & (DPJ_GATED | DPJ_PATH_LONG)) != 0u;
+		const bool dead = (has_l && (jfl & DPJ_LEFT_FAIL)) || (has_r && (jfl & (DPJ_RIGHT_FAIL | DPJ_RIGHT_SKIPPED)));
+		const int pen1 = jpen + (has_l ? jstartq - jls : 0);
+		const int pen2 = pen1 + (has_r ? (S.QL - (jstartq + jlen)) - jrs : 0);
+		const int jscore = jhs + (has_l ? jls : 0) + (has_r ? jrs : 0);
+		auto viable = [&]() {
+			return k < kend && jpen <= S.maxPen && (raises || (!dead && pen1 <= S.maxPen && pen2 <= S.maxPen && jscore >= S.best - SECONDARY_HIT_MAX_DELTA && jscore >= 10));
+		};
+		used += (uint32_t)__builtin_popcountll(__ballot(k < kend && jpen <= S.maxPen));
+		uint64_t todo = __ballot(viable());
+		while (todo) {
+			const int t = __builtin_ctzll(todo);
+			todo &= todo - 1;
+			DpJob J;
+			J.read = r; J.startdb = 0; J.maxpen = 0; J.k = 0; J.pad[0] = J.pad[1] = 0;
+			J.pk = rdlane(jpk, t);
+			J.combined_tlo = rdlane(jw.x, t);
+			const uint32_t sc = rdlane(jw.y, t), fl = rdlane(jw.z, t);
+			J.left_score = (int16_t)(sc & 0xFFFFu); J.right_score = (int16_t)(sc >> 16);
+			J.nops = (uint8_t)(fl & 0xFFu); J.flags = (uint8_t)((fl >> 8) & 0xFFu); J.vst_l = (uint8_t)((fl >> 16) & 0xFFu); J.vst_r = (uint8_t)(fl >> 24);
+			const int mp0 = S.maxPen, b0 = S.best;
+			S.template consume_job<XW>(J, dp.ops + (size_t)(jb + k0 + (uint32_t)t) * DP_JOB_OPS);
+			if (S.maxPen != mp0 || S.best != b0) todo &= __ballot(viable());
+		}
+	}
+	if (nj > khi) {
+		URX_SYNC();
+		S.park_state(st, phase);
+		for (uint32_t k = khi + lane; k < nj; k += 64) dp.jobs[jb + k].maxpen = S.maxPen;
+		return used;
+	}
+	urmapx_result res;
+	res.dbpos = 0xFFFFFFFFu; res.seq_index = 0xFFFFFFFFu; res.coord = 0xFFFFFFFFu;
+	res.score = 0; res.second = 0; res.mapq = 0; res.plus = 0; res.exit_phase = 0; res.status = 0;
+	res.hit_count = 0; res.path_nops = 0; res.path_off = 0;
+	if (S.fill_result_core(res, phase)) {
+		if (pb.used + S.top_nops > PBUF_OPS || pb.n == PEND) pb.flush(lane, results, path_ops, path_used);
+		URX_SYNC();
+		for (int t = lane; t < S.top_nops; t += 64) pb.pbuf[pb.used + t] = S.top[t];
+		res.path_nops = (uint16_t)S.top_nops;
+		res.path_off = (uint32_t)pb.used;
+		if (lane == 0) { pb.pend_r[pb.n] = r; pb.pend_res[pb.n] = res; }
+		pb.used += S.top_nops; ++pb.n;
+	} else if (lane == 0) results[r] = res;
+	if constexpr (!OVF) {
+		if (res.status & (URMAPX_ST_HSP_OVERFLOW | URMAPX_ST_HIT_OVERFLOW)) {
+			if (lane == 0) ovf_list[1 + atomicAdd(ovf_list, 1u)] = r;
+		}
+	}
+	return used;
+}
+
+template <class SW>
+__device__ __forceinline__ void finalize_caps(SW &S, int hsp_lds_cap) {
+	S.hsp_lds = (hsp_lds_cap >= 64 && hsp_lds_cap <= HSP_CAP) ? (hsp_lds_cap & ~63) : HSP_CAP;
+	S.hit_cap = (hsp_lds_cap >= 64 && hsp_lds_cap <= HSP_CAP) ? S.hsp_lds / 4 : 64 * SE_HITW1;
+	S.hit_wsh = (hsp_lds_cap >= 64 && hsp_lds_cap <= HSP_CAP) ? 4 : 6;
+}
+
+struct DpFinArgs {
+	uint32_t *fin_cnt;
+	urmapx_result *results;
+	urmapx_path_op *path_ops;
+	uint32_t *path_used;
+	uint32_t *ovf_list;
+	const uint32_t *gate;
+	int hsp_lds_cap;
+	int rd;
+};
+template <int NCH, int FIN>
+__device__ __forceinline__ void dp_body(const DevIndex &X, const urmapx_params &P, const uint8_t *__restrict__ bases,
+                                        const uint64_t *__restrict__ offs, const DpWork &dp, uint8_t *scratch,
+                                        size_t scratch_stride, const uint8_t *__restrict__ g_seq, uint32_t klo, uint32_t khi,
+                                        uint32_t *ticket, const uint32_t *__restrict__ list, const uint32_t *list_count, const DpFinArgs &fa) {
 	constexpr int QMAX = 64 * NCH;
 	constexpr int TB_ROWS8 = (QMAX - 24) / 8 + 2;
 	__shared__ __attribute__((aligned(16))) uint8_t sQT[QMAX + QMAX + 64];
@@ -1393,6 +1561,35 @@
 	__shared__ uint32_t wlds[3 * QMAX];
 	__shared__ uint16_t ropsL[OPS_CAP], ropsR[OPS_CAP], cand[URMAPX_MAX_PATH_OPS];
 	const int lane = threadIdx.x;
+	constexpr int FIN_PBUF = 256, FIN_PEND = 16;
+	uint16_t *fin_top = nullptr;
+	FinPaths<FIN_PBUF, FIN_PEND> fin_pb;
+	if constexpr (FIN != 0) {
+		__shared__ uint16_t s_top[URMAPX_MAX_PATH_OPS], s_pbuf[FIN_PBUF];
+		__shared__ uint32_t s_pend_r[FIN_PEND];
+		__shared__ urmapx_result s_pend_res[FIN_PEND];
+		fin_top = s_top;
+		fin_pb.pbuf = s_pbuf; fin_pb.pend_r = s_pend_r; fin_pb.pend_res = s_pend_res;
+	}
+	uint32_t fin_used = 0;
+	uint32_t pend_slot = 0, pend_n = 0;
+	auto count_off = [&]() {
+		if constexpr (FIN != 0) {
+			const uint32_t slot = pend_slot, n = pend_n;
+			pend_n = 0;
+			wait_vm0();
+			const uint32_t left = uni(atomicSub(fa.fin_cnt + (size_t)slot * DP_ROUNDS + fa.rd, lane == 0 ? n : 0u));
+			if (left != n) return;
+			using SW = SearchWave<NCH, FIN == 2>;
+			SW S(X, P, lane);
+			S.W = (int)X.W;
+			S.top = fin_top; S.cand = cand;
+			finalize_caps(S, fa.hsp_lds_cap);
+			const uint4 ent = reinterpret_cast<const uint4 *>(dp.fin_list)[slot];
+			fin_used += finalize_read_round<true>(S, fin_pb, dp, slot, ent, klo, khi, fa.results, fa.path_ops, fa.path_used, fa.ovf_list, lane);
+			URX_SYNC();
+		}
+	};
 	WideScratch ws;
 	ws.carve(scratch + (size_t)blockIdx.x * scratch_stride, QMAX, QMAX + 64);
 	const VPar VP(P);
@@ -1429,16 +1626,27 @@
 	uint32_t jl = 0xFFFFFFFFu;
 	if (lane < (int)DP_TILE && tile + lane < nlist) jl = list ? list[tile + lane] : tile + (uint32_t)lane;
 	uint64_t todo = __ballot(jl != 0xFFFFFFFFu);
-	while (todo) {
-		const uint32_t j = rdlane(jl, __builtin_ctzll(todo));
-		todo &= todo - 1;
-		const DpJob J = dp.jobs[j];
-		if (J.read == 0xFFFFFFFFu) continue;
+	while (todo || (FIN != 0 && pend_n)) {
+		const bool have = todo != 0;
+		uint32_t j = 0;
+		DpJob J{};
+		if (have) {
+			j = rdlane(jl, __builtin_ctzll(todo));
+			todo &= todo - 1;
+			J = dp.jobs[j];
+			if (J.read == 0xFFFFFFFFu) continue;
+		}
+		if constexpr (FIN != 0) {
+			if (pend_n && (!have || J.combined_tlo != pend_slot)) count_off();
+			if (!have) break;
+			pend_slot = J.combined_tlo;
+		}
 		{
 			const int glen = (int)((J.pk >> PK_LEN_SH) & PK_MASK), gscore = (int)((J.pk >> PK_SCORE_SH) & PK_MASK);
 			if (glen - gscore > J.maxpen) {
-				if (lane == 0) dp.jobs[j].flags = DPJ_GATED;
+				if (lane == 0) st_xw<FIN != 0>(&dp.jobs[j].flags, DPJ_GATED);
 				++n_gated;
+				++pend_n;
 				continue;
 			}
 		}
@@ -1532,17 +1740,46 @@
 			if (ovf) { flags |= DPJ_PATH_LONG; nc = 0; }
 			URX_SYNC();
 			uint16_t *out = dp.ops + (size_t)j * DP_JOB_OPS;
-			for (int t = lane; t < nc; t += 64) out[t] = cand[t];
+			for (int t = lane; t < nc; t += 64) st_xw<FIN != 0>(out + t, cand[t]);
 		}
 		if (lane == 0) {
 			DpJob *o = dp.jobs + j;
-			o->combined_tlo = combinedTLo;
-			o->left_score = (int16_t)leftScore; o->right_score = (int16_t)rightScore;
-			o->nops = (uint8_t)nc; o->flags = (uint8_t)flags; o->vst_l = (uint8_t)vst_l; o->vst_r = (uint8_t)vst_r;
-		}
-	}
+			if constexpr (FIN != 0) {
+				static_assert(offsetof(DpJob, combined_tlo) == 16 && offsetof(DpJob, left_score) == 20 && offsetof(DpJob, nops) == 24, "DpJob layout");
+				uint32_t *ow = reinterpret_cast<uint32_t *>(o);
+				st_xw<true>(ow + 4, combinedTLo);
+				st_xw<true>(ow + 5, (uint32_t)(uint16_t)(int16_t)leftScore | ((uint32_t)(uint16_t)(int16_t)rightScore << 16));
+				st_xw<true>(ow + 6, (uint32_t)(uint8_t)nc | ((uint32_t)(uint8_t)flags << 8) | ((uint32_t)(uint8_t)vst_l << 16) | ((uint32_t)(uint8_t)vst_r << 24));
+			} else {
+				o->combined_tlo = combinedTLo;
+				o->left_score = (int16_t)leftScore; o->right_score = (int16_t)rightScore;
+				o->nops = (uint8_t)nc; o->flags = (uint8_t)flags; o->vst_l = (uint8_t)vst_l; o->vst_r = (uint8_t)vst_r;
+			}
+		}
+		++pend_n;
+	}
+	}
+	if constexpr (FIN != 0) {
+		fin_pb.flush(lane, fa.results, fa.path_ops, fa.path_used);
+		if (lane == 0 && fin_used) atomicAdd(dp.counters + 2, fin_used);
 	}
 	if (lane == 0 && n_gated) atomicAdd(dp.counters + 3, n_gated);
+}
+template <int NCH>
+__global__ __launch_bounds__(64) void dp_kernel(DevIndex X, urmapx_params P, const uint8_t *__restrict__ bases,
+                                                const uint64_t *__restrict__ offs, DpWork dp, uint8_t *scratch,
+                                                size_t scratch_stride, const uint8_t *__restrict__ g_seq, uint32_t klo, uint32_t khi,
+                                                uint32_t *ticket, const uint32_t *__restrict__ list, const uint32_t *list_count, const uint32_t *gate) {
+	if (gate && *gate == 0) return;
+	dp_body<NCH, 0>(X, P, bases, offs, dp, scratch, scratch_stride, g_seq, klo, khi, ticket, list, list_count, DpFinArgs{});
+}
+template <int NCH, bool OVF>
+__global__ __launch_bounds__(64) __attribute__((amdgpu_waves_per_eu(NCH <= 5 ? 6 : 1))) void dp_fin_kernel(DevIndex X, urmapx_params P, const uint8_t *__restrict__ bases,
+                                                const uint64_t *__restrict__ offs, DpWork dp, uint8_t *scratch,
+                                                size_t scratch_stride, const uint8_t *__restrict__ g_seq, uint32_t klo, uint32_t khi,
+                                                uint32_t *ticket, const uint32_t *__restrict__ list, const uint32_t *list_count, DpFinArgs fa) {
+	if (fa.gate && *fa.gate == 0) return;
+	dp_body<NCH, OVF ? 2 : 1>(X, P, bases, offs, dp, scratch, scratch_stride, g_seq, klo, khi, ticket, list, list_count, fa);
 }
 
 template <int NCH, bool OVF>
@@ -1556,119 +1793,24 @@
 	__shared__ uint16_t pbuf[PBUF_OPS];
 	__shared__ uint32_t pend_r[PEND];
 	__shared__ urmapx_result pend_res[PEND];
-	int pb_used = 0, pb_n = 0;
 	const int lane = threadIdx.x;
-	auto flush_paths = [&]() {
-		if (pb_n == 0) return;
-		URX_SYNC();
-		uint32_t po = 0;
-		if (lane == 0) po = atomicAdd(path_used, (uint32_t)pb_used);
-		po = uni(po);
-		for (int t = lane; t < pb_used; t += 64) path_ops[po + t] = pbuf[t];
-		if (lane < pb_n) {
-			urmapx_result rr = pend_res[lane];
-			rr.path_off += po;
-			results[pend_r[lane]] = rr;
-		}
-		URX_SYNC();
-		pb_used = 0; pb_n = 0;
-	};
+	FinPaths<PBUF_OPS, PEND> pb;
+	pb.pbuf = pbuf; pb.pend_r = pend_r; pb.pend_res = pend_res;
 	SW S(X, P, lane);
 	S.W = (int)X.W;
 	S.top = top; S.cand = cand;
-	S.hsp_lds = (hsp_lds_cap >= 64 && hsp_lds_cap <= HSP_CAP) ? (hsp_lds_cap & ~63) : HSP_CAP;
-	S.hit_cap = (hsp_lds_cap >= 64 && hsp_lds_cap <= HSP_CAP) ? S.hsp_lds / 4 : 64 * SE_HITW1;
-	S.hit_wsh = (hsp_lds_cap >= 64 && hsp_lds_cap <= HSP_CAP) ? 4 : 6;
+	finalize_caps(S, hsp_lds_cap);
 	const uint32_t parked = dp.counters[1] < dp.fin_cap ? dp.counters[1] : dp.fin_cap;
 	const uint4 *const fin = reinterpret_cast<const uint4 *>(dp.fin_list);
 	uint32_t used_block = 0;
 	uint4 ent = make_uint4(0u, 0u, 0u, 0u);
 	if (blockIdx.x < parked) ent = fin[blockIdx.x];
 	for (uint32_t e = blockIdx.x; e < parked; e += gridDim.x) {
-		const uint32_t r = uni(ent.x), jb = uni(ent.y), nj = uni(ent.z);
-		S.QL = (int)uni(ent.w);
+		const uint4 cur = ent;
 		if (e + gridDim.x < parked) ent = fin[e + gridDim.x];
-		if (nj <= klo) continue;
-		S.nwords = S.QL - (S.W - 1);
-		const uint32_t kend = nj < khi ? nj : khi;
-		uint32_t jpk0 = 0;
-		uint4 jw0 = make_uint4(0u, 0u, 0u, 0u);
-		if (klo + (uint32_t)lane < kend) {
-			const uint32_t *jp = reinterpret_cast<const uint32_t *>(dp.jobs + jb + klo + (uint32_t)lane);
-			jpk0 = jp[2];
-			jw0 = *reinterpret_cast<const uint4 *>(jp + 4);
-		}
-		URX_SYNC();
-		uint32_t *const st = dp.state + (size_t)e * SW::STATE_WORDS;
-		const int phase = S.restore_state(st);
-		uint32_t used = 0;
-		for (uint32_t k0 = klo; k0 < kend; k0 += 64) {
-			const uint32_t k = k0 + (uint32_t)lane;
-			const uint32_t jpk = jpk0;
-			const uint4 jw = jw0;
-			jpk0 = 0; jw0 = make_uint4(0u, 0u, 0u, 0u);
-			if (k + 64u < kend) {
-				const uint32_t *jp = reinterpret_cast<const uint32_t *>(dp.jobs + jb + k + 64u);
-				jpk0 = jp[2];
-				jw0 = *reinterpret_cast<const uint4 *>(jp + 4);
-			}
-			const int jstartq = (int)(jpk & PK_MASK), jlen = (int)((jpk >> PK_LEN_SH) & PK_MASK), jhs = (int)((jpk >> PK_SCORE_SH) & PK_MASK);
-			const int jpen = jlen - jhs;
-			const int jls = (int)(int16_t)(jw.y & 0xFFFFu), jrs = (int)(int16_t)(jw.y >> 16);
-			const uint32_t jfl = (jw.z >> 8) & 0xFFu;
-			const bool has_l = jstartq > 0, has_r = jstartq + jlen < S.QL;
-			const bool raises = (jw.z >> 16) != 0u || (jfl & (DPJ_GATED | DPJ_PATH_LONG)) != 0u;
-			const bool dead = (has_l && (jfl & DPJ_LEFT_FAIL)) || (has_r && (jfl & (DPJ_RIGHT_FAIL | DPJ_RIGHT_SKIPPED)));
-			const int pen1 = jpen + (has_l ? jstartq - jls : 0);
-			const int pen2 = pen1 + (has_r ? (S.QL - (jstartq + jlen)) - jrs : 0);
-			const int jscore = jhs + (has_l ? jls : 0) + (has_r ? jrs : 0);
-			auto viable = [&]() {
-				return k < kend && jpen <= S.maxPen && (raises || (!dead && pen1 <= S.maxPen && pen2 <= S.maxPen && jscore >= S.best - SECONDARY_HIT_MAX_DELTA && jscore >= 10));
-			};
-			used += (uint32_t)__builtin_popcountll(__ballot(k < kend && jpen <= S.maxPen));
-			uint64_t todo = __ballot(viable());
-			while (todo) {
-				const int t = __builtin_ctzll(todo);
-				todo &= todo - 1;
-				DpJob J;
-				J.read = r; J.startdb = 0; J.maxpen = 0; J.k = 0; J.pad[0] = J.pad[1] = 0;
-				J.pk = rdlane(jpk, t);
-				J.combined_tlo = rdlane(jw.x, t);
-				const uint32_t sc = rdlane(jw.y, t), fl = rdlane(jw.z, t);
-				J.left_score = (int16_t)(sc & 0xFFFFu); J.right_score = (int16_t)(sc >> 16);
-				J.nops = (uint8_t)(fl & 0xFFu); J.flags = (uint8_t)((fl >> 8) & 0xFFu); J.vst_l = (uint8_t)((fl >> 16) & 0xFFu); J.vst_r = (uint8_t)(fl >> 24);
-				const int mp0 = S.maxPen, b0 = S.best;
-				S.consume_job(J, dp.ops + (size_t)(jb + k0 + (uint32_t)t) * DP_JOB_OPS);
-				if (S.maxPen != mp0 || S.best != b0) todo &= __ballot(viable());
-			}
-		}
-		used_block += used;
-		if (nj > khi) {
-			URX_SYNC();
-			S.park_state(st, phase);
-			for (uint32_t k = khi + lane; k < nj; k += 64) dp.jobs[jb + k].maxpen = S.maxPen;
-			continue;
-		}
-		urmapx_result res;
-		res.dbpos = 0xFFFFFFFFu; res.seq_index = 0xFFFFFFFFu; res.coord = 0xFFFFFFFFu;
-		res.score = 0; res.second = 0; res.mapq = 0; res.plus = 0; res.exit_phase = 0; res.status = 0;
-		res.hit_count = 0; res.path_nops = 0; res.path_off = 0;
-		if (S.fill_result_core(res, phase)) {
-			if (pb_used + S.top_nops > PBUF_OPS || pb_n == PEND) flush_paths();
-			URX_SYNC();
-			for (int t = lane; t < S.top_nops; t += 64) pbuf[pb_used + t] = top[t];
-			res.path_nops = (uint16_t)S.top_nops;
-			res.path_off = (uint32_t)pb_used;
-			if (lane == 0) { pend_r[pb_n] = r; pend_res[pb_n] = res; }
-			pb_used += S.top_nops; ++pb_n;
-		} else if (lane == 0) results[r] = res;
-		if constexpr (!OVF) {
-			if (res.status & (URMAPX_ST_HSP_OVERFLOW | URMAPX_ST_HIT_OVERFLOW)) {
-				if (lane == 0) ovf_list[1 + atomicAdd(ovf_list, 1u)] = r;
-			}
-		}
-	}
-	flush_paths();
+		used_block += finalize_read_round<false>(S, pb, dp, e, cur, klo, khi, results, path_ops, path_used, ovf_list, lane);
+	}
+	pb.flush(lane, results, path_ops, path_used);
 	if (lane == 0 && used_block) atomicAdd(dp.counters + 2, used_block);
 }
 
@@ -1896,7 +2038,7 @@
 	stamp(STAGE_P3_MAIN);                                                                                                           \
 	hipLaunchKernelGGL((dp_kernel<NCH_>), dim3((unsigned)wk.dp_blocks), block, 0, s, X, P, d_bases, d_offs, wk.dp3,                   \
 	                   wk.dp_scratch, wk.dp_scratch_stride, X.seq, 0u, 0xFFFFFFFFu, wk.dp3.tickets, (const uint32_t *)nullptr,       \
-	                   wk.dp3.counters);                                                                                             \
+	                   wk.dp3.counters, (const uint32_t *)nullptr);                                                                                        \
 	stamp(STAGE_P3_DP);                                                                                                             \
 	hipLaunchKernelGGL((search_se_kernel<NCH_, false, false, true, 2>), grid, block, 0, s, X, P, d_bases, d_offs, n, d_results,       \
 	                   d_path_ops, d_path_used, no_stats3, wk.scratch, wk.scratch_stride, X.seq, X.blob, X.seqp, wk.ticket3,         \
@@ -1904,22 +2046,33 @@
 	} while (0)
 #define URX_LAUNCH_DP(NCH_, OVF_, PASS_)                                                                                          \
 	do {  \
-	const unsigned dpg = (unsigned)wk.dp_blocks;                                                                                  \
+	const unsigned dpg = PASS_ && wk.cus > 0 && (unsigned)wk.cus < (unsigned)wk.dp_blocks ? (unsigned)wk.cus : (unsigned)wk.dp_blocks;  \
 	const unsigned fing = (unsigned)(wk.fin_blocks > 0 ? wk.fin_blocks : wk.blocks), fing2 = PASS_ && fing > 1024u ? 1024u : fing;  \
 	const uint32_t *const DP_ROUND_LO = wk.dp_bounds.lo;                                                                          \
-	hipLaunchKernelGGL(dp_round_lists_kernel, dim3(PASS_ ? 128 : 2048), dim3(256), 0, s, wk.dp[PASS_], wk.dp_bounds);             \
+	const uint32_t *const gate = PASS_ ? wk.ovf_list : nullptr;                                                                   \
+	const DpWork &dpw = wk.dp[PASS_];                                                                                             \
+	uint32_t *const fin_cnt = fused ? wk.dp_fin_cnt[PASS_] : nullptr;                                                             \
+	hipLaunchKernelGGL(dp_round_lists_kernel, dim3(PASS_ ? 128 : 2048), dim3(256), 0, s, dpw, wk.dp_bounds, gate, fin_cnt);       \
 	for (int rd = 0; rd < DP_ROUNDS; ++rd) {                                                                                      \
 		if (rd >= wk.dp_bounds.rounds) { stamp(2 + (2 * DP_ROUNDS + 1) * PASS_ + 2 * rd); stamp(3 + (2 * DP_ROUNDS + 1) * PASS_ + 2 * rd); continue; } \
-		hipLaunchKernelGGL((dp_kernel<NCH_>), dim3(dpg), block, 0, s, X, P, d_bases, d_offs, wk.dp[PASS_],                        \
-		                   wk.dp_scratch, wk.dp_scratch_stride, X.seq, DP_ROUND_LO[rd], DP_ROUND_LO[rd + 1],                      \
-		                   wk.dp[PASS_].tickets + rd, wk.dp[PASS_].round_list + (size_t)rd * wk.dp[PASS_].jobs_cap,               \
-		                   wk.dp[PASS_].tickets + 8 + rd);                                                                       \
+		const DpFinArgs fa{fin_cnt, d_results, d_path_ops, d_path_used, wk.ovf_list, gate, wk.hsp_lds_cap, rd};                              \
+		if (fused)                                                                                                                \
+			hipLaunchKernelGGL((dp_fin_kernel<NCH_, OVF_>), dim3(dpg), block, 0, s, X, P, d_bases, d_offs, dpw,                 \
+			                   wk.dp_scratch, wk.dp_scratch_stride, X.seq, DP_ROUND_LO[rd], DP_ROUND_LO[rd + 1],                      \
+			                   dpw.tickets + rd, dpw.round_list + (size_t)rd * dpw.jobs_cap, dpw.tickets + 8 + rd, fa);               \
+		else                                                                                                                      \
+			hipLaunchKernelGGL((dp_kernel<NCH_>), dim3(dpg), block, 0, s, X, P, d_bases, d_offs, dpw,                                 \
+			                   wk.dp_scratch, wk.dp_scratch_stride, X.seq, DP_ROUND_LO[rd], DP_ROUND_LO[rd + 1],                      \
+			                   dpw.tickets + rd, dpw.round_list + (size_t)rd * dpw.jobs_cap, dpw.tickets + 8 + rd, gate);             \
 		stamp(2 + (2 * DP_ROUNDS + 1) * PASS_ + 2 * rd);                                                                            \
-		hipLaunchKernelGGL((finalize_se_kernel<NCH_, OVF_>), dim3(fing2), block,                                                  \
-		                   0, s, X, P, d_offs, wk.dp[PASS_], d_results, d_path_ops, d_path_used, wk.hsp_lds_cap, wk.ovf_list,        \
-		                   DP_ROUND_LO[rd], DP_ROUND_LO[rd + 1]);                                                                  \
+		if (!fused)                                                                                                               \
+			hipLaunchKernelGGL((finalize_se_kernel<NCH_, OVF_>), dim3(fing2), block,                                                  \
+			                   0, s, X, P, d_offs, dpw, d_results, d_path_ops, d_path_used, wk.hsp_lds_cap, wk.ovf_list,                 \
+			                   DP_ROUND_LO[rd], DP_ROUND_LO[rd + 1]);                                                                  \
 		stamp(3 + (2 * DP_ROUNDS + 1) * PASS_ + 2 * rd);                                                                            \
 	} } while (0)
+	const char *const sepfin = getenv("URMAPX_DP_SEPARATE_FINALIZE");
+	const bool fused = !(sepfin && atoi(sepfin) > 0) && wk.dp_fin_cnt[0] != nullptr && wk.dp_fin_cnt[1] != nullptr;
 	stamp(0);
 	const bool diag = wk.stats != nullptr && (nch == 3 || nch == 4);
 	uint32_t *const no_stats3 = nullptr;
@@ -1998,12 +2151,12 @@
 	if (hipGetDeviceProperties(&prop, device) != hipSuccess) return 0;
 	int per_cu = 0;
 	const int nchq = nch_for(max_read_len);
-	hipError_t e = nchq == 2   ? hipOccupancyMaxActiveBlocksPerMultiprocessor(&per_cu, dp_kernel<2>, 64, 0)
-	               : nchq == 3 ? hipOccupancyMaxActiveBlocksPerMultiprocessor(&per_cu, dp_kernel<3>, 64, 0)
-	               : nchq == 4 ? hipOccupancyMaxActiveBlocksPerMultiprocessor(&per_cu, dp_kernel<4>, 64, 0)
-	               : nchq == 5 ? hipOccupancyMaxActiveBlocksPerMultiprocessor(&per_cu, dp_kernel<5>, 64, 0)
-	               : nchq == 8 ? hipOccupancyMaxActiveBlocksPerMultiprocessor(&per_cu, dp_kernel<8>, 64, 0)
-	                           : hipOccupancyMaxActiveBlocksPerMultiprocessor(&per_cu, dp_kernel<16>, 64, 0);
+	hipError_t e = nchq == 2   ? hipOccupancyMaxActiveBlocksPerMultiprocessor(&per_cu, dp_fin_kernel<2, false>, 64, 0)
+	               : nchq == 3 ? hipOccupancyMaxActiveBlocksPerMultiprocessor(&per_cu, dp_fin_kernel<3, false>, 64, 0)
+	               : nchq == 4 ? hipOccupancyMaxActiveBlocksPerMultiprocessor(&per_cu, dp_fin_kernel<4, false>, 64, 0)
+	               : nchq == 5 ? hipOccupancyMaxActiveBlocksPerMultiprocessor(&per_cu, dp_fin_kernel<5, false>, 64, 0)
+	               : nchq == 8 ? hipOccupancyMaxActiveBlocksPerMultiprocessor(&per_cu, dp_fin_kernel<8, false>, 64, 0)
+	                           : hipOccupancyMaxActiveBlocksPerMultiprocessor(&per_cu, dp_fin_kernel<16, false>, 64, 0);
 	if (e != hipSuccess || per_cu < 1) per_cu = 8;
 	return per_cu * prop.multiProcessorCount;
 }
diff --git a/urmap_amd/csrc/urmapx.hip b/urmap_amd/csrc/urmapx.hip
--- a/urmap_amd/csrc/urmapx.hip
+++ b/urmap_amd/csrc/urmapx.hip
@@ -88,6 +88,7 @@
 	DevBuf<uint32_t> slowlist;
 	int dp_blocks[6] = {0, 0, 0, 0, 0, 0};
 	int fin_blocks[6] = {0, 0, 0, 0, 0, 0};
+	int cus = 0;
 	hipEvent_t stage_ev[STAGE_EVENTS] = {};
 	bool stage_valid = false;
 	bool p3_parked = false;
@@ -701,6 +702,8 @@
 		wk.dp_blocks = C->dp_blocks[cls];
 		if (C->fin_blocks[cls] == 0) C->fin_blocks[cls] = fin_block_count(max_read_len, C->device);
 		wk.fin_blocks = C->fin_blocks[cls] > 0 ? C->fin_blocks[cls] : 0;
+		if (C->cus == 0 && hipDeviceGetAttribute(&C->cus, hipDeviceAttributeMultiprocessorCount, C->device) != hipSuccess) C->cus = 0;
+		wk.cus = C->cus;
 		wk.dp_scratch_stride = dp_scratch_stride(max_read_len);
 		wk.dp_bounds = dp_bounds_default(max_read_len > 192);
 		if (const char *e = getenv("URMAPX_DP_BOUNDS")) {
@@ -728,7 +731,7 @@
 		const uint32_t jobs_cap[2] = {(uint32_t)(jc < (1ull << 30) ? jc : (1ull << 30)) + 4096u,
 		                              (uint32_t)(jc < (1ull << 30) ? jc : (1ull << 30)) + 65536u};
 		const uint32_t fin_cap[2] = {n, n / 8u + 1024u};
-		size_t need = 256, at[2][7];
+		size_t need = 256, at[2][8];
 		for (int p = 0; p < 2; ++p) {
 			at[p][5] = need; need += (((size_t)jobs_cap[p] * 2) + 63) & ~(size_t)63;
 			at[p][0] = need; need += (size_t)jobs_cap[p] * sizeof(DpJob);
@@ -737,6 +740,8 @@
 			at[p][3] = need; need += (size_t)fin_cap[p] * dp_state_words(p == 1) * 4;
 			at[p][4] = 16 * (size_t)p;
 			at[p][6] = need; need += (((size_t)jobs_cap[p] * 4 * DP_ROUNDS) + 63) & ~(size_t)63;
+			need = (need + 63) & ~(size_t)63;
+			at[p][7] = need; need += (((size_t)fin_cap[p] * 4 * DP_ROUNDS) + 63) & ~(size_t)63;
 		}
 		const char *park3 = getenv("URMAPX_PARK_PHASE3");
 		size_t p3w = (park3 && atoi(park3) > 0) ? p3_state_words(max_read_len) : 0;
@@ -777,6 +782,7 @@
 			d.kidx = reinterpret_cast<uint16_t *>(C->dpbuf.p + at[p][5]);
 			d.round_list = reinterpret_cast<uint32_t *>(C->dpbuf.p + at[p][6]);
 			d.fin_list = reinterpret_cast<uint32_t *>(C->dpbuf.p + at[p][2]);
+			wk.dp_fin_cnt[p] = reinterpret_cast<uint32_t *>(C->dpbuf.p + at[p][7]);
 			d.state = reinterpret_cast<uint32_t *>(C->dpbuf.p + at[p][3]);
 			d.counters = reinterpret_cast<uint32_t *>(C->dpbuf.p + at[p][4]);
 			d.tickets = reinterpret_cast<uint32_t *>(C->dpbuf.p + 64 + 4 * DP_TICKET_WORDS * (size_t)p);
```

Result: no change. 58.22 million (-0.3%).
